# myshell-ai/OpenVoice

Measured on AMD Instinct MI355X. Metric: real_time_factor, higher is better.
Workload: dtype f32; 1 GPU; ToneColorConverter.convert path, 32 x 10 s @ 22.05 kHz per GPU (T=861 frames), fp32, calibrated random weights; batch_per_gpu=32, global_batch=32, parallelism=dp1 (utterance sharding, RCCL broadcast of src/tgt se)

## Files before the change

include/openvoice_amd.h:

```cpp
#ifndef OPENVOICE_AMD_H
#define OPENVOICE_AMD_H

#include <stddef.h>
#include <stdint.h>

#ifdef __cplusplus
extern "C" {
#endif

typedef void* ov_stream_t;

enum {
  OV_OK = 0,
  OV_E_BADARG = -1,
  OV_E_UNSUPPORTED = -2,
  OV_E_ALIGN = -3,
  OV_E_LAUNCH = -4
};

enum {
  OV_EPI_LINEAR = 0,
  OV_EPI_GATE = 1,
  OV_EPI_RESSKIP = 2,
  OV_EPI_COUPLE = 3,
  OV_EPI_POSTERIOR = 4,
  OV_EPI_CONVT = 5,
  OV_EPI_MAGNITUDE = 6
};

enum {
  OV_F_MASK_V = 1,
  OV_F_OUT2_INIT = 2,
  OV_F_CONVT_GROUPED = 4,
  OV_F_NO_XCD_MAP = 8
};

typedef struct ov_conv1d_params {
  const float* x;
  const float* w;
  const float* bias;
  const float* bias_b;
  float* out;
  const float* res;
  const float* add;
  float* out2;
  const float* mask;
  int64_t x_bstride;
  int64_t out_bstride;
  int64_t res_bstride;
  int64_t add_bstride;
  int64_t out2_bstride;
  int64_t bias_b_bstride;
  int64_t mask_bstride;
  int32_t B, Cin, L;
  int32_t x_ld;
  int32_t out_ld;
  int32_t M;
  int32_t Cout;
  int32_t K, dil;
  int32_t epi, flags, split, phase_s;
  int32_t tiles_per_wg;
  int32_t tile;
  int32_t loaders;
  int32_t chunk;
  float in_slope;
  float scale;
  const int32_t* col_limit;
  int32_t col_limit_scale;
  int32_t reserved0;
} ov_conv1d_params;


size_t ov_conv1d_pack_size(int Cout, int Cin, int K);
int ov_conv1d_pack_rows(int Cout);
int ov_conv1d_pack_f32(const float* w, int Cout, int Cin, int K, float* dst);


int ov_conv1d_f32(const ov_conv1d_params* p, ov_stream_t stream);

typedef struct ov_respair_params {
  const float* x;
  const float* w1;
  const float* b1;
  const float* w2;
  const float* b2;
  float* out;
  const float* add;
  int64_t x_bstride, out_bstride, add_bstride;
  int32_t B, C, L;
  int32_t ld;
  int32_t K, dil;
  int32_t nwg;
  float slope;
  float scale;
  unsigned long long* dbg;
  const int32_t* col_limit;
  int32_t col_limit_scale;
  int32_t reserved0;
} ov_respair_params;
int ov_resblock_pair_f32(const ov_respair_params* p, ov_stream_t stream);
int ov_resblock_pair_supported(int C, int K, int dil);

typedef struct ov_wn_layer_params {
  const float* x;
  float* out;
  float* skip;
  const float* w_in;
  const float* b_in;
  const float* cond;
  const float* w_rs;
  const float* b_rs;
  const float* mask;
  int64_t bstride;
  int64_t cond_bstride;
  int64_t mask_bstride;
  int32_t B, H, T;
  int32_t ld;
  int32_t K;
  int32_t first;
  int32_t last;
  int32_t width;
  int32_t ntile;
  int32_t row_split;
  unsigned long long* dbg;
  float* acts;
} ov_wn_layer_params;
int ov_wn_layer_f32(const ov_wn_layer_params* p, ov_stream_t stream);
int ov_wn_layer_supported(int H, int K);
size_t ov_wn_pack_size(int rows, int cin, int K);
int ov_wn_pack_f32(const float* w, int rows, int cin, int K, float* dst);
int ov_wn_layer_tile(int B, int T, int width);

int ov_wn_layer_wino_f32(const ov_wn_layer_params* p, ov_stream_t stream);
int ov_wn_layer_wino_tile(void);
size_t ov_wn_wino_pack_size(int rows, int cin, int K);
int ov_wn_wino_pack_f32(const float* w, int rows, int cin, int K, float* dst);

int ov_wn_layer_bf16(const ov_wn_layer_params* p, ov_stream_t stream);
int ov_wn_layer_bf16_supported(int H, int K);
size_t ov_wn_bf16_pack_size(int rows, int cin, int K);
int ov_wn_bf16_pack(const float* w, int rows, int cin, int K, uint16_t* dst);
int ov_wn_layer_bf16_tile(int B, int T, int width);

int ov_frame_hops_f32(const float* wave, float* hops, int B, int N, int hop, int pad, int U, int ld,
                      ov_stream_t stream);

int ov_frame_hops_windows_f32(const float* wave, int64_t n_samples, const int64_t* first_frame, int W, int hop, int pad,
                              int U, int ld, float* hops, ov_stream_t stream);
int ov_frame_hops_multi_f32(const float* pool, int64_t pool_len, const int64_t* records, int W, int hop, int pad, int U,
                            int ld, float* hops, ov_stream_t stream);
int ov_stitch_window_cores_f32(const float* o_hat, const int64_t* windows, int W, int Tw, int spf, float* out,
                               int64_t out_len, int64_t out_frame0, ov_stream_t stream);
int ov_carry_rows_f32(const int64_t* records, int n_records, const float* src_base, int64_t src_elems, float* dst_base,
                      int64_t dst_elems, ov_stream_t stream);
int ov_rows_f32_to_cl_bf16(const float* src, int64_t src_bs, int src_ld, uint16_t* dst, int B, int C, int L,
                           ov_stream_t stream);
int ov_cl_bf16_to_rows_f32(const uint16_t* src, float* dst, int64_t dst_bs, int dst_ld, int B, int C, int L,
                           ov_stream_t stream);

int ov_vad_frame_energy_f32(const float* pool, int64_t pool_len, const int64_t* records, int R, int H, int ldT,
                            float* energy, ov_stream_t stream);
int ov_vad_segments_i32(const float* energy, const int64_t* records, int R, int H, int ldT, float floor_lin,
                        float range_lin, int min_silence_frames, int min_speech_frames, int pad_frames, int32_t* mask,
                        int64_t* offsets, int64_t* n_active, ov_stream_t stream);
int ov_vad_compact_f32(const float* pool, int64_t pool_len, const int64_t* records, int R, int H, int ldT,
                       const int32_t* mask, const int64_t* offsets, const int64_t* out_bases, float* out,
                       int64_t out_len, ov_stream_t stream);

int ov_join_segments_f32(const float* src, int64_t src_elems, const int64_t* records, int R, float* dst,
                         int64_t dst_elems, int64_t max_span, ov_stream_t stream);

int ov_pack_groups_cl_bf16(const float* src, int64_t src_len, const int64_t* records, int n, int C, uint16_t* dst,
                           int64_t dst_len, ov_stream_t stream);
int ov_unpack_groups_f32(const float* src, int64_t src_len, const int64_t* records, int n, float* dst, int64_t dst_len,
                         ov_stream_t stream);

int ov_normal_philox_f32(const int64_t* records, int R, int C, float* dst, int64_t dst_elems, int64_t max_frames,
                         ov_stream_t stream);

int ov_polyphase_fir_f32(const float* x, const double* h, float* y, int64_t n_in, int64_t n_out, int P, int Q, int taps,
                         ov_stream_t stream);

int ov_polyphase_fir_rows_f32(const int64_t* records, int n_records, const float* src_base, int64_t src_elems,
                              const double* h_base, int64_t h_elems, float* dst_base, int64_t dst_elems, int64_t max_out,
                              ov_stream_t stream);

int ov_conv_post_tanh_f32(const float* x, const float* w, float* out, int B, int C, int L, int K,
                          float in_slope, ov_stream_t stream);
int ov_conv_post_tanh_limited_f32(const float* x, const float* w, float* out, int B, int C, int L, int K,
                                  float in_slope, const int32_t* col_limit, int col_limit_scale, ov_stream_t stream);
int ov_frame_limits_i32(const int64_t* lengths, int32_t* limits, int B, int T, int margin, ov_stream_t stream);

int ov_linear_f32(const float* x, const float* w, const float* bias, float* y, int B, int M, int Kdim,
                  ov_stream_t stream);

int ov_sequence_mask_f32(const int64_t* lengths, float* mask, int B, int T, int ld, ov_stream_t stream);
int ov_unpad_rows_f32(const float* src, float* dst, int rows, int T, int ld, ov_stream_t stream);


int ov_layernorm_freq_f32(const float* x, const float* gamma, const float* beta, float* y, int N, int F, int T,
                          float eps, ov_stream_t stream);

int ov_conv2d_s2_relu_f32(const float* x, const float* w, const float* bias, float* y, int N, int Cin, int Cout,
                          int Fi, int Ti, ov_stream_t stream);

int ov_gru_f32(const float* gi, const float* whh_t, const float* bhh, float* h_out, int N, int H, int T,
               ov_stream_t stream);


int ov_layernorm_freq_ragged_f32(const float* x, const float* gamma, const float* beta, const int32_t* lens, float* y,
                                 int N, int F, int ld, float eps, ov_stream_t stream);

int ov_conv2d_s2_relu_ragged_f32(const float* x, const float* w, const float* bias, const int32_t* lens_in, float* y,
                                 int N, int Cin, int Cout, int Fi, int ld_in, int ld_out, ov_stream_t stream);

int ov_gru_ragged_f32(const float* gi, const float* whh_t, const float* bhh, const int32_t* lens, float* h_out, int N,
                      int H, int ld, ov_stream_t stream);


int ov_embed_f32(const int64_t* tokens, const float* emb, const int64_t* lengths, float* out, int B, int T, int H,
                 int V, int ld, float scale, ov_stream_t stream);

enum {
  OV_LN_PRE_RELU = 1,
  OV_LN_POST_GELU = 2
};
int ov_layernorm_ch_f32(const float* x, const float* res, const float* gamma, const float* beta, const float* res2,
                        const float* mask, float* out, int B, int C, int T, int ld, float eps, int flags,
                        ov_stream_t stream);

int ov_rel_attention_f32(const float* q, const float* k, const float* v, const float* emb_k, const float* emb_v,
                         const float* mask, float* out, int64_t qkv_bstride, int64_t out_bstride, int B, int n_heads,
                         int dk, int T, int ld, int window, ov_stream_t stream);

int ov_dwconv1d_f32(const float* x, const float* w, const float* bias, const float* mask, float* out, int B, int C,
                    int T, int ld, int K, int dil, ov_stream_t stream);

int ov_expand1_f32(const float* x0, int64_t x0_bstride, const float* w, const float* bias, const float* g, float* out,
                   int B, int C, int T, int ld, ov_stream_t stream);

int ov_add_bias_mask_f32(const float* x, const float* bias_b, const float* mask, float* out, int B, int C, int T,
                         int ld, ov_stream_t stream);

int ov_rq_spline_inverse_f32(float* z, int64_t z_bstride, int c0, int c1, const float* h, int64_t h_bstride,
                             const float* mask, int B, int T, int ld, int num_bins, int filter_channels,
                             float tail_bound, ov_stream_t stream);

int ov_duration_f32(const float* z_sdp, int64_t z_bstride, float ea_m, float ea_logs, const float* dp,
                    int64_t dp_bstride, const float* mask, float* logw, int32_t* cum, int64_t* y_len, int B, int T,
                    int ld, float sdp_ratio, float length_scale, ov_stream_t stream);

int ov_expand_prior_f32(const float* m_tok, const float* logs_tok, int64_t tok_bstride, int ldx, const int32_t* cum,
                        const int64_t* x_len, const int64_t* y_len, const float* noise, int64_t noise_bstride, int ldn, float* z_p,
                        float* m_p, float* logs_p, float* attn, int B, int C, int Tx, int Ty, int ldy,
                        float noise_scale, ov_stream_t stream);

int ov_duration_items_f32(const float* z_sdp, int64_t z_bstride, float ea_m, float ea_logs, const float* dp,
                          int64_t dp_bstride, const float* mask, float* logw, int32_t* cum, int64_t* y_len, int B,
                          int T, int ld, const float* sdp_ratio_b, const float* length_scale_b, ov_stream_t stream);

int ov_expand_prior_items_f32(const float* m_tok, const float* logs_tok, int64_t tok_bstride, int ldx,
                              const int32_t* cum, const int64_t* x_len, const int64_t* y_len, const float* noise,
                              int64_t noise_bstride, int ldn, float* z_p, float* m_p, float* logs_p, float* attn,
                              int B, int C, int Tx, int Ty, int ldy, const float* noise_scale_b, ov_stream_t stream);

typedef struct ov_conv1d_bf16_params {
  const uint16_t* x;
  const uint16_t* w;
  const float* bias;
  uint16_t* out;
  const uint16_t* res;
  const uint16_t* add;
  int32_t B, L, Cin, Cout, K, dil;
  int32_t phase_s;
  int32_t bias_bstride;
  int32_t layout;
  float in_slope;
  float scale;
  float out_slope;
  unsigned long long* dbg;
} ov_conv1d_bf16_params;

size_t ov_conv1d_bf16_pack_size(int Cout, int Cin, int K);
int ov_conv1d_bf16_pack(const float* w, int Cout, int Cin, int K, uint16_t* dst);
int ov_conv1d_bf16cl(const ov_conv1d_bf16_params* p, ov_stream_t stream);
int ov_conv_post_tanh_bf16(const uint16_t* x, const float* w, float* out, int B, int C, int L, int K, float in_slope,
                           ov_stream_t stream);

typedef struct ov_respair_bf16_params {
  const uint16_t* x;
  const uint16_t* w1;
  const float* b1;
  const uint16_t* w2;
  const float* b2;
  uint16_t* out;
  const uint16_t* add;
  int32_t B, L, C, K, dil;
  int32_t nwg;
  float slope, scale;
  unsigned long long* dbg;
} ov_respair_bf16_params;
int ov_resblock_pair_bf16cl(const ov_respair_bf16_params* p, ov_stream_t stream);
int ov_resblock_pair_bf16_supported(int C, int K, int dil);

typedef struct ov_respair2_bf16_params {
  const uint16_t* x;
  const uint16_t* w1;
  const float* b1;
  const uint16_t* w2;
  const float* b2;
  uint16_t* out;
  const uint16_t* add;
  int32_t B, L, C, K, dil;
  int32_t nwg;
  float slope;
  float scale;
  float out_slope;
  int32_t exp_flags;
  unsigned long long* dbg;
} ov_respair2_bf16_params;
int ov_resblock_pair2_bf16cl(const ov_respair2_bf16_params* p, ov_stream_t stream);
int ov_conv1d_bf16_pack16(const float* w, int Cout, int Cin, int K, uint16_t* dst);
int ov_resblock_pair2_bf16_supported(int C, int K, int dil);

typedef struct ov_conv1d_split3_params {
  const uint16_t* x;
  const uint16_t* w;
  const float* bias;
  uint16_t* out;
  const uint16_t* res;
  int64_t x_plane, out_plane, res_plane;
  int32_t B, L, Cin, Cout, K, dil;
  int32_t nwg;
  int32_t products;
  float res_slope;
  float out_slope;
  float scale;
  int32_t col_limit_scale;
  unsigned long long* dbg;
  const int32_t* col_limit;
} ov_conv1d_split3_params;
int ov_conv1d_split3(const ov_conv1d_split3_params* p, ov_stream_t stream);
size_t ov_conv1d_split3_pack_size(int Cout, int Cin, int K);
int ov_conv1d_split3_pack(const float* w, int Cout, int Cin, int K, uint16_t* dst);
int ov_conv1d_split3_supported(int Cin, int Cout, int K, int dil);
int ov_split3_from_f32(const float* x, uint16_t* planes, int64_t plane_stride, int B, int C, int L, float slope,
                       ov_stream_t stream);
int ov_split3_to_f32(const uint16_t* a, const uint16_t* b, const uint16_t* c, int64_t plane_stride, float* out, int B,
                     int C, int L, float in_slope, float scale, ov_stream_t stream);

typedef struct ov_conv1d_wino_params {
  const float* x;
  const float* w;
  const float* bias;
  float* out;
  const float* res;
  const float* add;
  int64_t x_bstride, out_bstride, res_bstride, add_bstride;
  int32_t B, Cin, Cout, L;
  int32_t x_ld, out_ld;
  int32_t K, dil;
  int32_t nwg;
  int32_t frags;
  float in_slope;
  float scale;
  unsigned long long* dbg;
  const int32_t* col_limit;
  int32_t col_limit_scale;
  float out_slope;
} ov_conv1d_wino_params;
int ov_conv1d_wino_f32(const ov_conv1d_wino_params* p, ov_stream_t stream);
int ov_conv1d_wino_multi_f32(const ov_conv1d_wino_params* convs, int n, ov_stream_t stream);
int ov_conv1d_wino_supported(int Cin, int Cout, int K, int dil);
int ov_conv1d_wino_chunk(int K, int Cout);
size_t ov_conv1d_wino_pack_size(int Cout, int Cin, int K);
int ov_conv1d_wino_pack_f32(const float* w, int Cout, int Cin, int K, float* dst);

int ov_version(void);
#define OV_ABI_VERSION 212
int ov_build_experiment(void);

#ifdef __cplusplus
}
#endif
#endif
```

openvoice_amd/_lib.py:

```python
import ctypes
import os

_HERE = os.path.dirname(os.path.abspath(__file__))
LIB_PATH = os.environ.get("OPENVOICE_AMD_LIB") or os.path.join(_HERE, "libopenvoice_amd.so")

OV_OK = 0
MIN_VERSION = 212
OV_ERRORS = {-1: "OV_E_BADARG", -2: "OV_E_UNSUPPORTED", -3: "OV_E_ALIGN", -4: "OV_E_LAUNCH"}

EPI_LINEAR, EPI_GATE, EPI_RESSKIP, EPI_COUPLE, EPI_POSTERIOR, EPI_CONVT, EPI_MAGNITUDE = range(7)
F_MASK_V = 1
F_OUT2_INIT = 2
F_CONVT_GROUPED = 4
F_NO_XCD_MAP = 8

_fp = ctypes.c_void_p
_i = ctypes.c_int
_i64 = ctypes.c_int64
LN_PRE_RELU, LN_POST_GELU = 1, 2


class ConvParams(ctypes.Structure):
    _fields_ = [
        ("x", _fp), ("w", _fp), ("bias", _fp), ("bias_b", _fp), ("out", _fp), ("res", _fp),
        ("add", _fp), ("out2", _fp), ("mask", _fp),
        ("x_bstride", ctypes.c_int64), ("out_bstride", ctypes.c_int64), ("res_bstride", ctypes.c_int64),
        ("add_bstride", ctypes.c_int64), ("out2_bstride", ctypes.c_int64), ("bias_b_bstride", ctypes.c_int64),
        ("mask_bstride", ctypes.c_int64),
        ("B", ctypes.c_int32), ("Cin", ctypes.c_int32), ("L", ctypes.c_int32),
        ("x_ld", ctypes.c_int32), ("out_ld", ctypes.c_int32), ("M", ctypes.c_int32),
        ("Cout", ctypes.c_int32), ("K", ctypes.c_int32), ("dil", ctypes.c_int32), ("epi", ctypes.c_int32),
        ("flags", ctypes.c_int32), ("split", ctypes.c_int32), ("phase_s", ctypes.c_int32),
        ("tiles_per_wg", ctypes.c_int32), ("tile", ctypes.c_int32), ("loaders", ctypes.c_int32),
        ("chunk", ctypes.c_int32),
        ("in_slope", ctypes.c_float), ("scale", ctypes.c_float),
        ("col_limit", _fp), ("col_limit_scale", ctypes.c_int32), ("reserved0", ctypes.c_int32),
    ]


class ConvBf16Params(ctypes.Structure):
    _fields_ = [("x", _fp), ("w", _fp), ("bias", _fp), ("out", _fp), ("res", _fp), ("add", _fp),
                ("B", ctypes.c_int32), ("L", ctypes.c_int32), ("Cin", ctypes.c_int32), ("Cout", ctypes.c_int32),
                ("K", ctypes.c_int32), ("dil", ctypes.c_int32), ("phase_s", ctypes.c_int32), ("bias_bstride", ctypes.c_int32), ("layout", ctypes.c_int32),
                ("in_slope", ctypes.c_float), ("scale", ctypes.c_float), ("out_slope", ctypes.c_float), ("dbg", _fp)]


class RespairParams(ctypes.Structure):
    _fields_ = [("x", _fp), ("w1", _fp), ("b1", _fp), ("w2", _fp), ("b2", _fp), ("out", _fp), ("add", _fp),
                ("x_bstride", ctypes.c_int64), ("out_bstride", ctypes.c_int64), ("add_bstride", ctypes.c_int64),
                ("B", ctypes.c_int32), ("C", ctypes.c_int32), ("L", ctypes.c_int32), ("ld", ctypes.c_int32),
                ("K", ctypes.c_int32), ("dil", ctypes.c_int32), ("nwg", ctypes.c_int32),
                ("slope", ctypes.c_float), ("scale", ctypes.c_float), ("dbg", _fp),
                ("col_limit", _fp), ("col_limit_scale", ctypes.c_int32), ("reserved0", ctypes.c_int32)]


class RespairBf16Params(ctypes.Structure):
    _fields_ = [("x", _fp), ("w1", _fp), ("b1", _fp), ("w2", _fp), ("b2", _fp), ("out", _fp), ("add", _fp),
                ("B", ctypes.c_int32), ("L", ctypes.c_int32), ("C", ctypes.c_int32), ("K", ctypes.c_int32),
                ("dil", ctypes.c_int32), ("nwg", ctypes.c_int32), ("slope", ctypes.c_float), ("scale", ctypes.c_float),
                ("dbg", _fp)]


class Respair2Bf16Params(ctypes.Structure):
    _fields_ = [("x", _fp), ("w1", _fp), ("b1", _fp), ("w2", _fp), ("b2", _fp), ("out", _fp), ("add", _fp),
                ("B", ctypes.c_int32), ("L", ctypes.c_int32), ("C", ctypes.c_int32), ("K", ctypes.c_int32),
                ("dil", ctypes.c_int32), ("nwg", ctypes.c_int32), ("slope", ctypes.c_float), ("scale", ctypes.c_float),
                ("out_slope", ctypes.c_float), ("exp_flags", ctypes.c_int32), ("dbg", _fp)]


class ConvSplit3Params(ctypes.Structure):
    _fields_ = [("x", _fp), ("w", _fp), ("bias", _fp), ("out", _fp), ("res", _fp),
                ("x_plane", ctypes.c_int64), ("out_plane", ctypes.c_int64), ("res_plane", ctypes.c_int64),
                ("B", ctypes.c_int32), ("L", ctypes.c_int32), ("Cin", ctypes.c_int32), ("Cout", ctypes.c_int32),
                ("K", ctypes.c_int32), ("dil", ctypes.c_int32), ("nwg", ctypes.c_int32), ("products", ctypes.c_int32),
                ("res_slope", ctypes.c_float), ("out_slope", ctypes.c_float), ("scale", ctypes.c_float),
                ("col_limit_scale", ctypes.c_int32), ("dbg", _fp), ("col_limit", _fp)]


class ConvWinoParams(ctypes.Structure):
    _fields_ = [("x", _fp), ("w", _fp), ("bias", _fp), ("out", _fp), ("res", _fp), ("add", _fp),
                ("x_bstride", ctypes.c_int64), ("out_bstride", ctypes.c_int64), ("res_bstride", ctypes.c_int64),
                ("add_bstride", ctypes.c_int64),
                ("B", ctypes.c_int32), ("Cin", ctypes.c_int32), ("Cout", ctypes.c_int32), ("L", ctypes.c_int32),
                ("x_ld", ctypes.c_int32), ("out_ld", ctypes.c_int32), ("K", ctypes.c_int32), ("dil", ctypes.c_int32),
                ("nwg", ctypes.c_int32), ("frags", ctypes.c_int32),
                ("in_slope", ctypes.c_float), ("scale", ctypes.c_float), ("dbg", _fp),
                ("col_limit", _fp), ("col_limit_scale", ctypes.c_int32), ("out_slope", ctypes.c_float)]


class WnLayerParams(ctypes.Structure):
    _fields_ = [("x", _fp), ("out", _fp), ("skip", _fp), ("w_in", _fp), ("b_in", _fp), ("cond", _fp), ("w_rs", _fp),
                ("b_rs", _fp), ("mask", _fp),
                ("bstride", ctypes.c_int64), ("cond_bstride", ctypes.c_int64), ("mask_bstride", ctypes.c_int64),
                ("B", ctypes.c_int32), ("H", ctypes.c_int32), ("T", ctypes.c_int32), ("ld", ctypes.c_int32),
                ("K", ctypes.c_int32), ("first", ctypes.c_int32), ("last", ctypes.c_int32), ("width", ctypes.c_int32),
                ("ntile", ctypes.c_int32), ("row_split", ctypes.c_int32), ("dbg", _fp), ("acts", _fp)]


SIGNATURES = {
    "ov_version": (ctypes.c_int, []),
    "ov_build_experiment": (ctypes.c_int, []),
    "ov_conv1d_pack_size": (ctypes.c_size_t, [ctypes.c_int, ctypes.c_int, ctypes.c_int]),
    "ov_conv1d_pack_rows": (ctypes.c_int, [ctypes.c_int]),
    "ov_conv1d_pack_f32": (ctypes.c_int, [_fp, ctypes.c_int, ctypes.c_int, ctypes.c_int, _fp]),
    "ov_conv1d_f32": (ctypes.c_int, [ctypes.POINTER(ConvParams), _fp]),
    "ov_resblock_pair_f32": (ctypes.c_int, [ctypes.POINTER(RespairParams), _fp]),
    "ov_resblock_pair_supported": (ctypes.c_int, [_i, _i, _i]),
    "ov_wn_layer_f32": (ctypes.c_int, [ctypes.POINTER(WnLayerParams), _fp]),
    "ov_wn_layer_supported": (ctypes.c_int, [_i, _i]),
    "ov_wn_pack_size": (ctypes.c_size_t, [_i, _i, _i]),
    "ov_wn_pack_f32": (ctypes.c_int, [_fp, _i, _i, _i, _fp]),
    "ov_wn_layer_tile": (ctypes.c_int, [_i, _i, _i]),
    "ov_wn_layer_wino_f32": (ctypes.c_int, [ctypes.POINTER(WnLayerParams), _fp]),
    "ov_wn_layer_wino_tile": (ctypes.c_int, []),
    "ov_wn_wino_pack_size": (ctypes.c_size_t, [_i, _i, _i]),
    "ov_wn_wino_pack_f32": (ctypes.c_int, [_fp, _i, _i, _i, _fp]),
    "ov_wn_layer_bf16": (ctypes.c_int, [ctypes.POINTER(WnLayerParams), _fp]),
    "ov_wn_layer_bf16_supported": (ctypes.c_int, [_i, _i]),
    "ov_wn_bf16_pack_size": (ctypes.c_size_t, [_i, _i, _i]),
    "ov_wn_bf16_pack": (ctypes.c_int, [_fp, _i, _i, _i, _fp]),
    "ov_wn_layer_bf16_tile": (ctypes.c_int, [_i, _i, _i]),
    "ov_conv_post_tanh_f32": (ctypes.c_int, [_fp, _fp, _fp, ctypes.c_int, ctypes.c_int, ctypes.c_int,
                                             ctypes.c_int, ctypes.c_float, _fp]),
    "ov_conv_post_tanh_limited_f32": (ctypes.c_int, [_fp, _fp, _fp, ctypes.c_int, ctypes.c_int, ctypes.c_int,
                                                     ctypes.c_int, ctypes.c_float, _fp, ctypes.c_int, _fp]),
    "ov_frame_limits_i32": (ctypes.c_int, [_fp, _fp, _i, _i, _i, _fp]),
    "ov_linear_f32": (ctypes.c_int, [_fp, _fp, _fp, _fp, ctypes.c_int, ctypes.c_int, ctypes.c_int, _fp]),
    "ov_sequence_mask_f32": (ctypes.c_int, [_fp, _fp, ctypes.c_int, ctypes.c_int, ctypes.c_int, _fp]),
    "ov_unpad_rows_f32": (ctypes.c_int, [_fp, _fp, ctypes.c_int, ctypes.c_int, ctypes.c_int, _fp]),
    "ov_polyphase_fir_f32": (ctypes.c_int, [_fp, _fp, _fp, ctypes.c_int64, ctypes.c_int64, _i, _i, _i, _fp]),
    "ov_polyphase_fir_rows_f32": (ctypes.c_int, [_fp, _i, _fp, _i64, _fp, _i64, _fp, _i64, _i64, _fp]),
    "ov_layernorm_freq_f32": (ctypes.c_int, [_fp, _fp, _fp, _fp, ctypes.c_int, ctypes.c_int, ctypes.c_int,
                                             ctypes.c_float, _fp]),
    "ov_conv2d_s2_relu_f32": (ctypes.c_int, [_fp, _fp, _fp, _fp, ctypes.c_int, ctypes.c_int, ctypes.c_int,
                                             ctypes.c_int, ctypes.c_int, _fp]),
    "ov_gru_f32": (ctypes.c_int, [_fp, _fp, _fp, _fp, ctypes.c_int, ctypes.c_int, ctypes.c_int, _fp]),
    "ov_layernorm_freq_ragged_f32": (ctypes.c_int, [_fp, _fp, _fp, _fp, _fp, _i, _i, _i, ctypes.c_float, _fp]),
    "ov_conv2d_s2_relu_ragged_f32": (ctypes.c_int, [_fp, _fp, _fp, _fp, _fp, _i, _i, _i, _i, _i, _i, _fp]),
    "ov_gru_ragged_f32": (ctypes.c_int, [_fp, _fp, _fp, _fp, _fp, _i, _i, _i, _fp]),
    "ov_conv1d_bf16_pack_size": (ctypes.c_size_t, [_i, _i, _i]),
    "ov_conv1d_bf16_pack": (ctypes.c_int, [_fp, _i, _i, _i, _fp]),
    "ov_conv1d_bf16_pack16": (ctypes.c_int, [_fp, _i, _i, _i, _fp]),
    "ov_conv1d_bf16cl": (ctypes.c_int, [ctypes.POINTER(ConvBf16Params), _fp]),
    "ov_resblock_pair_bf16cl": (ctypes.c_int, [ctypes.POINTER(RespairBf16Params), _fp]),
    "ov_resblock_pair_bf16_supported": (ctypes.c_int, [_i, _i, _i]),
    "ov_resblock_pair2_bf16cl": (ctypes.c_int, [ctypes.POINTER(Respair2Bf16Params), _fp]),
    "ov_resblock_pair2_bf16_supported": (ctypes.c_int, [_i, _i, _i]),
    "ov_conv_post_tanh_bf16": (ctypes.c_int, [_fp, _fp, _fp, _i, _i, _i, _i, ctypes.c_float, _fp]),
    "ov_conv1d_split3": (ctypes.c_int, [ctypes.POINTER(ConvSplit3Params), _fp]),
    "ov_conv1d_split3_pack_size": (ctypes.c_size_t, [_i, _i, _i]),
    "ov_conv1d_split3_pack": (ctypes.c_int, [_fp, _i, _i, _i, _fp]),
    "ov_conv1d_split3_supported": (ctypes.c_int, [_i, _i, _i, _i]),
    "ov_split3_from_f32": (ctypes.c_int, [_fp, _fp, _i64, _i, _i, _i, ctypes.c_float, _fp]),
    "ov_split3_to_f32": (ctypes.c_int, [_fp, _fp, _fp, _i64, _fp, _i, _i, _i, ctypes.c_float, ctypes.c_float, _fp]),
    "ov_conv1d_wino_f32": (ctypes.c_int, [ctypes.POINTER(ConvWinoParams), _fp]),
    "ov_conv1d_wino_multi_f32": (ctypes.c_int, [ctypes.POINTER(ConvWinoParams), _i, _fp]),
    "ov_conv1d_wino_supported": (ctypes.c_int, [_i, _i, _i, _i]),
    "ov_conv1d_wino_chunk": (ctypes.c_int, [_i, _i]),
    "ov_conv1d_wino_pack_size": (ctypes.c_size_t, [_i, _i, _i]),
    "ov_conv1d_wino_pack_f32": (ctypes.c_int, [_fp, _i, _i, _i, _fp]),
    "ov_frame_hops_f32": (ctypes.c_int, [_fp, _fp, _i, _i, _i, _i, _i, _i, _fp]),
    "ov_frame_hops_windows_f32": (ctypes.c_int, [_fp, _i64, _fp, _i, _i, _i, _i, _i, _fp, _fp]),
    "ov_frame_hops_multi_f32": (ctypes.c_int, [_fp, _i64, _fp, _i, _i, _i, _i, _i, _fp, _fp]),
    "ov_stitch_window_cores_f32": (ctypes.c_int, [_fp, _fp, _i, _i, _i, _fp, _i64, _i64, _fp]),
    "ov_carry_rows_f32": (ctypes.c_int, [_fp, _i, _fp, _i64, _fp, _i64, _fp]),
    "ov_rows_f32_to_cl_bf16": (ctypes.c_int, [_fp, _i64, _i, _fp, _i, _i, _i, _fp]),
    "ov_cl_bf16_to_rows_f32": (ctypes.c_int, [_fp, _fp, _i64, _i, _i, _i, _i, _fp]),
    "ov_vad_frame_energy_f32": (ctypes.c_int, [_fp, _i64, _fp, _i, _i, _i, _fp, _fp]),
    "ov_vad_segments_i32": (ctypes.c_int, [_fp, _fp, _i, _i, _i, ctypes.c_float, ctypes.c_float, _i, _i, _i, _fp, _fp, _fp,
                                           _fp]),
    "ov_vad_compact_f32": (ctypes.c_int, [_fp, _i64, _fp, _i, _i, _i, _fp, _fp, _fp, _fp, _i64, _fp]),
    "ov_join_segments_f32": (ctypes.c_int, [_fp, _i64, _fp, _i, _fp, _i64, _i64, _fp]),
    "ov_pack_groups_cl_bf16": (ctypes.c_int, [_fp, _i64, _fp, _i, _i, _fp, _i64, _fp]),
    "ov_unpack_groups_f32": (ctypes.c_int, [_fp, _i64, _fp, _i, _fp, _i64, _fp]),
    "ov_normal_philox_f32": (ctypes.c_int, [_fp, _i, _i, _fp, _i64, _i64, _fp]),
    "ov_embed_f32": (ctypes.c_int, [_fp, _fp, _fp, _fp, _i, _i, _i, _i, _i, ctypes.c_float, _fp]),
    "ov_layernorm_ch_f32": (ctypes.c_int, [_fp, _fp, _fp, _fp, _fp, _fp, _fp, _i, _i, _i, _i, ctypes.c_float, _i, _fp]),
    "ov_rel_attention_f32": (ctypes.c_int, [_fp, _fp, _fp, _fp, _fp, _fp, _fp, _i64, _i64, _i, _i, _i, _i, _i, _i,
                                            _fp]),
    "ov_add_bias_mask_f32": (ctypes.c_int, [_fp, _fp, _fp, _fp, _i, _i, _i, _i, _fp]),
    "ov_dwconv1d_f32": (ctypes.c_int, [_fp, _fp, _fp, _fp, _fp, _i, _i, _i, _i, _i, _i, _fp]),
    "ov_expand1_f32": (ctypes.c_int, [_fp, _i64, _fp, _fp, _fp, _fp, _i, _i, _i, _i, _fp]),
    "ov_rq_spline_inverse_f32": (ctypes.c_int, [_fp, _i64, _i, _i, _fp, _i64, _fp, _i, _i, _i, _i, _i,
                                                ctypes.c_float, _fp]),
    "ov_duration_f32": (ctypes.c_int, [_fp, _i64, ctypes.c_float, ctypes.c_float, _fp, _i64, _fp, _fp, _fp, _fp,
                                       _i, _i, _i, ctypes.c_float, ctypes.c_float, _fp]),
    "ov_expand_prior_f32": (ctypes.c_int, [_fp, _fp, _i64, _i, _fp, _fp, _fp, _fp, _i64, _i, _fp, _fp, _fp, _fp,
                                           _i, _i, _i, _i, _i, ctypes.c_float, _fp]),
    "ov_duration_items_f32": (ctypes.c_int, [_fp, _i64, ctypes.c_float, ctypes.c_float, _fp, _i64, _fp, _fp, _fp, _fp,
                                             _i, _i, _i, _fp, _fp, _fp]),
    "ov_expand_prior_items_f32": (ctypes.c_int, [_fp, _fp, _i64, _i, _fp, _fp, _fp, _fp, _i64, _i, _fp, _fp, _fp, _fp,
                                                 _i, _i, _i, _i, _i, _fp, _fp]),
}

_lib = None


class OvError(RuntimeError):
    pass


GENERATORS = ("fp32", "bf16")


def check_generator(generator, optional=False):
    if generator is None and optional:
        return None
    if not isinstance(generator, str) or generator not in GENERATORS:
        raise OvError(f"generator must be 'fp32' or 'bf16'{' (or None)' if optional else ''}, got {generator!r}")
    return generator


def generator_kw(generator):
    return {} if generator is None else {"generator": generator}


WAVENETS = ("fp32", "bf16")


def check_wavenet(wavenet, optional=False):
    if wavenet is None and optional:
        return None
    if not isinstance(wavenet, str) or wavenet not in WAVENETS:
        raise OvError(f"wavenet must be 'fp32' or 'bf16'{' (or None)' if optional else ''}, got {wavenet!r}")
    return wavenet


def wavenet_kw(wavenet):
    return {} if wavenet is None else {"wavenet": wavenet}


def load():
    global _lib
    if _lib is None:
        if not os.path.exists(LIB_PATH):
            raise OvError(f"{LIB_PATH} not found: build the HIP extension first "
                          f"(python -c 'import __graft_entry__ as g; g.build()'); there is no CPU fallback")
        lib = ctypes.CDLL(LIB_PATH)
        lib.ov_version.restype, lib.ov_version.argtypes = ctypes.c_int, []
        if lib.ov_version() < MIN_VERSION:
            raise OvError(f"{LIB_PATH} is version {lib.ov_version()}, this package needs >= {MIN_VERSION}: rebuild it "
                          f"(make -C openvoice_amd/csrc)")
        for name, (restype, argtypes) in SIGNATURES.items():
            try:
                fn = getattr(lib, name)
            except AttributeError:
                raise OvError(f"{LIB_PATH} lacks {name}: it was built from older source, rebuild it "
                              f"(make -C openvoice_amd/csrc)") from None
            fn.restype = restype
            fn.argtypes = argtypes
        exp = lib.ov_build_experiment()
        if exp != 0 and os.environ.get("OPENVOICE_AMD_ALLOW_EXPERIMENT") != "1":
            raise OvError(f"{LIB_PATH} is a measurement build (OV_EXP={exp}: kernels with loads / barriers compiled "
                          f"out, results meaningless); rebuild with `make -C openvoice_amd/csrc clean all`")
        _lib = lib
    return _lib


def torch_op(name, *args):
    try:
        return getattr(torch_ops(), name)(*args)
    except RuntimeError as exc:
        if isinstance(exc, OvError):
            raise
        raise OvError(str(exc).split("\n")[0]) from None


def check(code, what):
    if code != OV_OK:
        raise OvError(f"{what} failed: {OV_ERRORS.get(code, code)}")


SHIM_PATH = os.path.join(_HERE, "libopenvoice_amd_torch.so")
_ops = None
VALUE_FUNCS = {"ov_version", "ov_build_experiment", "ov_conv1d_pack_size", "ov_conv1d_pack_rows", "ov_wn_pack_size",
               "ov_conv1d_bf16_pack_size", "ov_resblock_pair_supported", "ov_wn_layer_supported", "ov_wn_layer_tile",
               "ov_resblock_pair_bf16_supported", "ov_resblock_pair2_bf16_supported", "ov_conv1d_split3_pack_size",
               "ov_conv1d_split3_supported", "ov_conv1d_wino_supported", "ov_conv1d_wino_chunk", "ov_conv1d_wino_pack_size",
               "ov_wn_layer_wino_tile", "ov_wn_wino_pack_size", "ov_wn_layer_bf16_supported", "ov_wn_bf16_pack_size",
               "ov_wn_layer_bf16_tile"}


def binding():
    b = os.environ.get("OPENVOICE_AMD_BINDING", "ctypes" if os.environ.get("OPENVOICE_AMD_LIB") else "torch")
    if b not in ("torch", "ctypes"):
        raise OvError(f"OPENVOICE_AMD_BINDING={b!r}: expected 'torch' or 'ctypes'")
    return b


def use_torch_binding():
    return binding() == "torch"


def torch_ops():
    global _ops
    if _ops is None:
        import torch
        for path in (LIB_PATH, SHIM_PATH):
            if not os.path.exists(path):
                raise OvError(f"{path} not found: build the HIP extension first (python -c 'import __graft_entry__ "
                              f"as g; g.build()'); there is no CPU fallback (OPENVOICE_AMD_BINDING=ctypes needs only "
                              f"libopenvoice_amd.so)")
        torch.ops.load_library(SHIM_PATH)
        ops = torch.ops.openvoice_amd
        if ops.version() < MIN_VERSION:
            raise OvError(f"{LIB_PATH} is version {ops.version()}, this package needs >= {MIN_VERSION}: rebuild it "
                          f"(make -C openvoice_amd/csrc)")
        exp = ops.build_experiment()
        if exp != 0 and os.environ.get("OPENVOICE_AMD_ALLOW_EXPERIMENT") != "1":
            raise OvError(f"{LIB_PATH} is a measurement build (OV_EXP={exp}); rebuild with "
                          f"`make -C openvoice_amd/csrc clean all`")
        _ops = ops
    return _ops


def _flat_view(t, off):
    start = t.storage_offset() + off
    n = t.untyped_storage().nbytes() // t.element_size() - start
    return t.as_strided((n,), (1,), start)


def call(name, *args):
    if use_torch_binding():
        targs = [_flat_view(*a) if type(a) is tuple else a for a in args]
        try:
            return getattr(torch_ops(), name[3:])(*targs)
        except RuntimeError as exc:
            if isinstance(exc, OvError):
                raise
            raise OvError(str(exc).split("\n")[0]) from None
    import torch
    lib = load()
    fn = getattr(lib, name)
    cargs, dev = [], None
    for a in args:
        off = 0
        if type(a) is tuple:
            a, off = a
        if isinstance(a, torch.Tensor):
            if dev is None and a.is_cuda:
                dev = a.device
            a = ctypes.c_void_p(a.data_ptr() + off * a.element_size())
        cargs.append(a)
    if len(fn.argtypes) == len(cargs) + 1:
        if dev is None:
            raise OvError(f"{name}: no device tensor among the arguments")
        cargs.append(ctypes.c_void_p(torch.cuda.current_stream(dev).cuda_stream))
    rc = fn(*cargs)
    if name in VALUE_FUNCS:
        return rc
    check(rc, name)
```

openvoice_amd/csrc/conv1d_mfma.h:

```cpp
#pragma once
#include <hip/hip_runtime.h>

#include <atomic>

#include "openvoice_amd.h"

namespace ovk {

constexpr int EPI_CONVT_S8 = 16;
constexpr int EPI_CONVT_S2 = 17;
constexpr bool is_convt(int epi) { return epi == OV_EPI_CONVT || epi == EPI_CONVT_S8 || epi == EPI_CONVT_S2; }

typedef float f32x16 __attribute__((ext_vector_type(16)));
typedef float f32x4 __attribute__((ext_vector_type(4)));
typedef float f32x2 __attribute__((ext_vector_type(2)));

constexpr int UNIT = 8;
constexpr int REC = 256;
constexpr int LB_MAX = 12;
constexpr int LIMIT_MAX_BATCH = 256;

__host__ __device__ inline int packed_units(int cin) { return ((cin + UNIT - 1) / UNIT + 3) / 4 * 4; }

__device__ __forceinline__ float lrelu(float v, float slope) { return v > 0.f ? v : v * slope; }

template <int EPI, int WM, int WN>
__device__ __forceinline__ void conv_epilogue(const ov_conv1d_params& p, f32x16 (&acc)[WM][WN], int b, int tcol0,
                                              int mtile0, int q, int lane, bool preloaded) {
  const uint32_t L = (uint32_t)p.L;
  const uint32_t LD = (uint32_t)p.out_ld;
  const uint32_t half = (uint32_t)lane >> 5;
  const uint32_t Cout = (uint32_t)p.Cout;
  const float scale = p.scale;
  const float* mrow = p.mask ? p.mask + (int64_t)b * p.mask_bstride : nullptr;
  float* outb = p.out + (int64_t)b * p.out_bstride;
  const uint32_t col0 = (uint32_t)tcol0 + ((uint32_t)lane & 31u);

  if constexpr (EPI == EPI_CONVT_S8 || EPI == EPI_CONVT_S2) {
    static_assert(WM == 2, "grouped ConvTranspose pairs two 32-row tiles per wave");
    const uint32_t Lout = LD;
    if ((uint32_t)q * 64u >= Cout * (uint32_t)p.phase_s) return;
#pragma unroll
    for (int j = 0; j < WN; ++j) {
      const uint32_t col = col0 + 32u * j;
      if (col >= L) continue;
      if constexpr (EPI == EPI_CONVT_S8) {
#pragma unroll
        for (int i = 0; i < 2; ++i) {
          const f32x16 v = acc[i][j];
#pragma unroll
          for (int c = 0; c < 4; ++c) {
            f32x4 o = {v[4 * c], v[4 * c + 1], v[4 * c + 2], v[4 * c + 3]};
            *reinterpret_cast<f32x4*>(outb + (size_t)((uint32_t)q * 8u + 2u * c + half) * Lout +
                                      (8u * col + 4u * i)) = o;
          }
        }
      } else {
        const f32x16 v0 = acc[0][j], v1 = acc[1][j];
#pragma unroll
        for (int r = 0; r < 16; ++r) {
          const uint32_t co = (uint32_t)q * 32u + 4u * half + (r & 3) + 8 * (r >> 2);
          f32x2 o = {v0[r], v1[r]};
          *reinterpret_cast<f32x2*>(outb + (co * Lout + 2u * col)) = o;
        }
      }
    }
    return;
  } else if constexpr (EPI == OV_EPI_MAGNITUDE) {
    static_assert(WM == 2, "magnitude pairs two 32-row tiles per wave");
    if ((uint32_t)q * 32u >= Cout) return;
#pragma unroll
    for (int j = 0; j < WN; ++j) {
      const uint32_t col = col0 + 32u * j;
      if (col >= L) continue;
      const uint32_t rbase = (uint32_t)q * 32u + 4u * half;
      const uint32_t voff = rbase * LD + col;
#pragma unroll
      for (int r = 0; r < 16; ++r) {
        const uint32_t rr = (r & 3) + 8 * (r >> 2);
        const float re = acc[0][j][r], im = acc[1][j][r];
        if (rbase + rr < Cout) (outb + (size_t)rr * LD)[voff] = sqrtf(re * re + im * im + scale);
      }
    }
    return;
  } else if constexpr (EPI == OV_EPI_GATE || EPI == OV_EPI_POSTERIOR) {
    static_assert(WM == 2, "gate/posterior pair two 32-row tiles per wave");
    if ((uint32_t)q * 32u >= Cout) return;
    const float* resb = p.res ? p.res + (int64_t)b * p.res_bstride : nullptr;
#pragma unroll
    for (int j = 0; j < WN; ++j) {
      const uint32_t col = col0 + 32u * j;
      if (col >= L) continue;
      const float mk = mrow ? mrow[col] : 1.f;
      const uint32_t voff = ((uint32_t)q * 32u + 4u * half) * LD + col;
      const uint32_t rbase = (uint32_t)q * 64u + 4u * half;
      const f32x16 v0 = acc[0][j], v1 = acc[1][j];
      if constexpr (EPI == OV_EPI_GATE) {
#pragma unroll
        for (int r = 0; r < 16; ++r) {
          const uint32_t rr = (r & 3) + 8 * (r >> 2);
          (outb + (size_t)rr * LD)[voff] = tanhf(v0[r]) * (1.f / (1.f + expf(-v1[r])));
        }
      } else {
        f32x16 nz;
#pragma unroll
        for (int r = 0; r < 16; ++r) nz[r] = (resb + (size_t)((r & 3) + 8 * (r >> 2)) * LD)[voff];
#pragma unroll
        for (int r = 0; r < 16; ++r) {
          const uint32_t rr = (r & 3) + 8 * (r >> 2);
          (outb + (size_t)rr * LD)[voff] = (v0[r] * mk + nz[r] * scale * expf(v1[r] * mk)) * mk;
        }
      }
    }
    return;
  } else {
    if constexpr (EPI == OV_EPI_LINEAR) {
      if (!mrow && !(p.res && !preloaded) && !p.add) {
#pragma unroll
        for (int i = 0; i < WM; ++i) {
          const uint32_t mt = (uint32_t)(mtile0 + i);
          if (mt * 32u >= Cout) continue;
#pragma unroll
          for (int j = 0; j < WN; ++j) {
            const uint32_t col = col0 + 32u * j;
            if (col >= L) continue;
            const uint32_t voff = (mt * 32u + 4u * half) * LD + col;
#pragma unroll
            for (int r = 0; r < 16; ++r) (outb + (size_t)((r & 3) + 8 * (r >> 2)) * LD)[voff] = acc[i][j][r] * scale;
          }
        }
        return;
      }
    }
#pragma unroll
    for (int i = 0; i < WM; ++i) {
      const uint32_t mt = (uint32_t)(mtile0 + i);
      if (mt * 32u >= (is_convt(EPI) ? Cout * (uint32_t)p.phase_s : Cout)) continue;
#pragma unroll
      for (int j = 0; j < WN; ++j) {
        const uint32_t col = col0 + 32u * j;
        if (col >= L) continue;
        const float mk = mrow ? mrow[col] : 1.f;
        const uint32_t rbase = mt * 32u + 4u * half;
        f32x16 v = acc[i][j];
        if constexpr (is_convt(EPI)) {
          const uint32_t s = (uint32_t)p.phase_s;
          const uint32_t Lout = LD;
          {
#pragma unroll
            for (int r = 0; r < 16; ++r) {
              const uint32_t row = rbase + (r & 3) + 8 * (r >> 2);
              const uint32_t co = row / s, ph = row - co * s;
              outb[co * Lout + s * col + ph] = v[r];
            }
          }
        } else {
          const uint32_t voff = rbase * LD + col;
          if constexpr (EPI == OV_EPI_LINEAR) {
            const float* resb = (p.res && !preloaded) ? p.res + (int64_t)b * p.res_bstride : nullptr;
            const float* addb = p.add ? p.add + (int64_t)b * p.add_bstride : nullptr;
            const float mkv = (p.flags & OV_F_MASK_V) ? mk : 1.f;
#pragma unroll
            for (int r = 0; r < 16; ++r) v[r] *= mkv;
            if (resb) {
#pragma unroll
              for (int r = 0; r < 16; ++r) v[r] += (resb + (size_t)((r & 3) + 8 * (r >> 2)) * LD)[voff];
            }
            if (addb) {
#pragma unroll
              for (int r = 0; r < 16; ++r) v[r] += (addb + (size_t)((r & 3) + 8 * (r >> 2)) * LD)[voff];
            }
#pragma unroll
            for (int r = 0; r < 16; ++r) (outb + (size_t)((r & 3) + 8 * (r >> 2)) * LD)[voff] = v[r] * scale;
          } else if constexpr (EPI == OV_EPI_RESSKIP) {
            if (mt * 32u < (uint32_t)p.split) {
#pragma unroll
              for (int r = 0; r < 16; ++r) (outb + (size_t)((r & 3) + 8 * (r >> 2)) * LD)[voff] = v[r] * mk;
            } else {
              float* o2 = p.out2 + (int64_t)b * p.out2_bstride;
              const uint32_t voff2 = voff - (uint32_t)p.split * LD;
#pragma unroll
              for (int r = 0; r < 16; ++r) (o2 + (size_t)((r & 3) + 8 * (r >> 2)) * LD)[voff2] = v[r];
            }
          } else {
            const float sg = scale > 0.f ? mk : -mk;
#pragma unroll
            for (int r = 0; r < 16; ++r) (outb + (size_t)((r & 3) + 8 * (r >> 2)) * LD)[voff] = v[r] * sg;
          }
        }
      }
    }
  }
}

template <int EPI, int WM, int WN>
__device__ __forceinline__ bool conv_preload(const ov_conv1d_params& p, f32x16 (&acc)[WM][WN], int b, int tcol0,
                                             int mtile0, int lane) {
  const uint32_t half = (uint32_t)lane >> 5;
  const uint32_t L = (uint32_t)p.L, LD = (uint32_t)p.out_ld;
  const uint32_t col0 = (uint32_t)tcol0 + ((uint32_t)lane & 31u);
  constexpr bool kOperands = EPI == OV_EPI_LINEAR || EPI == OV_EPI_RESSKIP || EPI == OV_EPI_COUPLE;
  bool preloaded = false;
  if constexpr (kOperands) {
    const float* src = nullptr;
    int64_t src_bs = 0;
    if constexpr (EPI == OV_EPI_LINEAR) {
      if (p.res && !(p.flags & OV_F_MASK_V)) { src = p.res; src_bs = p.res_bstride; }
    } else if (EPI == OV_EPI_COUPLE && p.res) {
      src = p.res; src_bs = p.res_bstride;
    } else {
      src = p.out; src_bs = p.out_bstride;
    }
    preloaded = src != nullptr;
    if (preloaded) {
      const uint32_t nfrag = (uint32_t)p.Cout / 32u;
      const float* srcb = src + (int64_t)b * src_bs;
#pragma unroll
      for (int i = 0; i < WM; ++i) {
        const uint32_t mt = min((uint32_t)(mtile0 + i), nfrag - 1u);
        const float* rowb = srcb;
        uint32_t mrow = mt * 32u;
        bool zero = false;
        if constexpr (EPI == OV_EPI_RESSKIP) {
          if (mrow >= (uint32_t)p.split) {
            rowb = p.out2 + (int64_t)b * p.out2_bstride;
            mrow -= (uint32_t)p.split;
            zero = (p.flags & OV_F_OUT2_INIT) != 0;
          }
        }
#pragma unroll
        for (int j = 0; j < WN; ++j) {
          const uint32_t col = min(col0 + 32u * j, L - 1u);
          const uint32_t voff = (mrow + 4u * half) * LD + col;
#pragma unroll
          for (int r = 0; r < 16; ++r) acc[i][j][r] = (rowb + (size_t)((r & 3) + 8 * (r >> 2)) * LD)[voff];
          if constexpr (EPI == OV_EPI_RESSKIP) {
            if (zero) {
#pragma unroll
              for (int r = 0; r < 16; ++r) acc[i][j][r] = 0.f;
            }
          }
          if constexpr (EPI == OV_EPI_COUPLE) {
            if (!(p.scale > 0.f)) {
#pragma unroll
              for (int r = 0; r < 16; ++r) acc[i][j][r] = -acc[i][j][r];
            }
          }
        }
      }
    }
  }
  if (!preloaded) {
#pragma unroll
    for (int i = 0; i < WM; ++i)
#pragma unroll
      for (int j = 0; j < WN; ++j)
#pragma unroll
        for (int r = 0; r < 16; ++r) acc[i][j][r] = 0.f;
  }
  {
    const float* __restrict__ bias = p.bias;
    const float* __restrict__ bias_b = p.bias_b ? p.bias_b + (int64_t)b * p.bias_b_bstride : nullptr;
    const uint32_t row_limit = (EPI == OV_EPI_GATE || EPI == OV_EPI_POSTERIOR || EPI == OV_EPI_MAGNITUDE)
                                   ? 2u * (uint32_t)p.Cout
                                   : (is_convt(EPI) ? (uint32_t)p.Cout * (uint32_t)p.phase_s : (uint32_t)p.Cout);
#pragma unroll
    for (int i = 0; i < WM; ++i) {
      const uint32_t rbase = (uint32_t)(mtile0 + i) * 32u + 4u * half;
      if (EPI != OV_EPI_MAGNITUDE && (uint32_t)(mtile0 + i) * 32u < row_limit) {
        f32x16 bv;
#pragma unroll
        for (int r = 0; r < 16; ++r) bv[r] = bias[rbase + (r & 3) + 8 * (r >> 2)];
        if (bias_b) {
#pragma unroll
          for (int r = 0; r < 16; ++r) bv[r] += bias_b[rbase + (r & 3) + 8 * (r >> 2)];
        }
#pragma unroll
        for (int j = 0; j < WN; ++j) acc[i][j] += bv;
      }
    }
  }
  return preloaded;
}

constexpr int STAGE_SCALAR = 0;
constexpr int STAGE_VEC = 1;

template <int K, int DIL, int WM, int WN, int WVM, int WVN, int CHUNK, int VEC, int EPI, int NLD>
__global__ __launch_bounds__(64 * (4 + NLD), (EPI == OV_EPI_GATE || EPI == EPI_CONVT_S8 || EPI == EPI_CONVT_S2) ? 4 : 1) void conv1d_mfma_kernel(const ov_conv1d_params p) {
  static_assert(WVM * WVN == 4, "4 matrix waves per workgroup");
  static_assert(VEC == STAGE_SCALAR || VEC == STAGE_VEC, "staging kind");
  static_assert(CHUNK % UNIT == 0 && (CHUNK / UNIT == 2 || CHUNK / UNIT == 4), "chunk = 2 or 4 units");
  constexpr int UPC = CHUNK / UNIT;
  constexpr int N_BLK = 32 * WN * WVN;
  constexpr int PAD = (K % 2 == 1) ? (K - 1) * DIL / 2 : 0;
  constexpr int PADR = (K - 1) * DIL - PAD;
  constexpr int PADA = (PAD + 3) / 4 * 4;
  constexpr int XS = N_BLK + PADA + (PADR + 3) / 4 * 4;
  constexpr int XS4 = XS / 4;
  constexpr int NITEM = VEC ? CHUNK * XS4 : CHUNK * XS;
  constexpr int BUF = CHUNK * XS;
  constexpr int PER_LANE = (NITEM + 64 * NLD - 1) / (64 * NLD);
  constexpr int LB = PER_LANE < LB_MAX ? PER_LANE : LB_MAX;
  constexpr int NBATCH = (PER_LANE + LB - 1) / LB;
  static_assert(NLD == 1 || NLD == 2 || NLD == 4, "1, 2 or 4 loader waves");

  __shared__ __attribute__((aligned(16))) float xs[2 * BUF];

  const int tid = threadIdx.x;
  const int lane = tid & 63;
  const int wave = __builtin_amdgcn_readfirstlane(tid >> 6);
  const int L = p.L, Cin = p.Cin;
  const int nunits = packed_units(Cin);
  const int nchunks = nunits / UPC;
  const int ntiles = (L + N_BLK - 1) / N_BLK;
  const int mblocks = (p.M + 32 * WM * WVM - 1) / (32 * WM * WVM);
  int total = ntiles * mblocks * p.B;
  __shared__ int lim_pref[LIMIT_MAX_BATCH + 1];
  const bool limited = p.col_limit != nullptr;
  if (limited) {
    if (wave == 0) {
      int carry = 0;
      for (int base = 0; base < p.B; base += 64) {
        const int bb = base + lane;
        int n = 0;
        if (bb < p.B) {
          long long c = (long long)p.col_limit[bb] * p.col_limit_scale;
          c = c < 0 ? 0 : (c > L ? L : c);
          n = ((int)c + N_BLK - 1) / N_BLK;
        }
        int s = n;
#pragma unroll
        for (int d = 1; d < 64; d <<= 1) {
          const int v = __shfl_up(s, d, 64);
          if (lane >= d) s += v;
        }
        if (bb < p.B) lim_pref[bb + 1] = carry + s;
        carry += __shfl(s, 63, 64);
      }
      if (lane == 0) lim_pref[0] = 0;
    }
    __syncthreads();
    total = __builtin_amdgcn_readfirstlane(lim_pref[p.B]) * mblocks;
  }
  auto decode = [&](int w, int& ub, int& utile, int& umblk) {
    const int g = w / mblocks;
    umblk = w - g * mblocks;
    if (!limited) {
      ub = g / ntiles;
      utile = g - ub * ntiles;
      return;
    }
    int lo = 0, hi = p.B;
    while (hi - lo > 1) {
      const int mid = (lo + hi) >> 1;
      if (__builtin_amdgcn_readfirstlane(lim_pref[mid]) <= g) lo = mid; else hi = mid;
    }
    ub = lo;
    utile = g - __builtin_amdgcn_readfirstlane(lim_pref[lo]);
  };
  int wid0 = blockIdx.x, wend = total, wstride = gridDim.x;
  if (!(p.flags & OV_F_NO_XCD_MAP) && (gridDim.x & 7u) == 0) {
    const int xcd = blockIdx.x & 7;
    const int lo = (int)(((long long)xcd * total) >> 3);
    wend = (int)(((long long)(xcd + 1) * total) >> 3);
    wid0 = lo + (int)(blockIdx.x >> 3);
    wstride = gridDim.x >> 3;
  }
  if (wid0 >= wend) return;

  bool is_loader = false;
#pragma unroll
  for (int i = 0; i < NLD; ++i) is_loader |= (wave == 4 + i);
#ifndef OV_EXP
#define OV_EXP 0
#endif
  if (is_loader) {
    if (OV_EXP == 1) return;
    const float slope = p.in_slope;
    const uint32_t ldx = (uint32_t)p.x_ld;
    const int llane = (wave - 4) * 64 + lane;
    const int Lin = L + ((K % 2 == 1) ? 0 : (K - 1) * DIL);
    int it = 0;
    for (int wid = wid0; wid < wend; wid += wstride) {
      int lb, ltile, lmblk;
      decode(wid, lb, ltile, lmblk);
      const int t0 = ltile * N_BLK;
      const float* __restrict__ xb = p.x + (int64_t)lb * p.x_bstride;
      for (int chunk = 0; chunk < nchunks; ++chunk, ++it) {
        float* dst = xs + (it & 1) * BUF;
#pragma unroll 1
        for (int bt = 0; bt < (OV_EXP ? 0 : NBATCH); ++bt) {
          if constexpr (VEC) {
            f32x4 stg[LB];
            int nval[LB];
#pragma unroll
            for (int i = 0; i < LB; ++i) {
              const int idx = (bt * LB + i) * (64 * NLD) + llane;
              const int row = idx / XS4, c4 = idx - row * XS4;
              const int ci = chunk * CHUNK + row;
              const int t = t0 - PADA + 4 * c4;
              const bool ok = idx < NITEM && ci < Cin && t >= 0 && t < Lin;
              const uint32_t goff = ok ? (uint32_t)ci * ldx + (uint32_t)t : 0u;
              nval[i] = ok ? min(Lin - t, 4) : 0;
              stg[i] = *reinterpret_cast<const f32x4*>(xb + goff);
            }
#pragma unroll
            for (int i = 0; i < LB; ++i) {
              const int idx = (bt * LB + i) * (64 * NLD) + llane;
              if (idx < NITEM) {
                f32x4 v = stg[i];
                const int n = nval[i];
                v[0] = n > 0 ? lrelu(v[0], slope) : 0.f;
                v[1] = n > 1 ? lrelu(v[1], slope) : 0.f;
                v[2] = n > 2 ? lrelu(v[2], slope) : 0.f;
                v[3] = n > 3 ? lrelu(v[3], slope) : 0.f;
                *reinterpret_cast<f32x4*>(dst + 4 * idx) = v;
              }
            }
          } else {
            float stg[LB];
            int nval[LB];
#pragma unroll
            for (int i = 0; i < LB; ++i) {
              const int idx = (bt * LB + i) * (64 * NLD) + llane;
              const int row = idx / XS, c = idx - row * XS;
              const int ci = chunk * CHUNK + row;
              const int t = t0 - PADA + c;
              const bool ok = idx < NITEM && ci < Cin && t >= 0 && t < Lin;
              const uint32_t goff = ok ? (uint32_t)ci * ldx + (uint32_t)t : 0u;
              nval[i] = ok ? 1 : 0;
              stg[i] = xb[goff];
            }
#pragma unroll
            for (int i = 0; i < LB; ++i) {
              const int idx = (bt * LB + i) * (64 * NLD) + llane;
              if (idx < NITEM) dst[idx] = nval[i] ? lrelu(stg[i], slope) : 0.f;
            }
          }
        }
        __syncthreads();
      }
    }
    return;
  }

  const int wm = wave / WVN, wn = wave % WVN;
  const int recs_per_mtile = nunits * K + 1;
  int wid = wid0;
  int mblk, tile, b;
  decode(wid, b, tile, mblk);
  int mtile0 = (mblk * WVM + wm) * WM;

  const f32x4* __restrict__ wbase = reinterpret_cast<const f32x4*>(p.w);
  uint32_t widx[WM];
#pragma unroll
  for (int i = 0; i < WM; ++i) widx[i] = (uint32_t)(mtile0 + i) * (uint32_t)recs_per_mtile * 64u + (uint32_t)lane;

  const int xl_off = (lane >> 5) * XS + wn * (32 * WN) + (lane & 31) + (PADA - PAD);

  f32x4 a_cur[WM], a_nxt[WM];
#pragma unroll
  for (int i = 0; i < WM; ++i) a_cur[i] = wbase[widx[i]];

#if OV_EXP == 3
  unsigned long long tph[5] = {0, 0, 0, 0, 0};
  unsigned long long tlast = __builtin_readcyclecounter();
#define OV_MARK(q) { const unsigned long long now_ = __builtin_readcyclecounter(); tph[q] += now_ - tlast; tlast = now_; }
#else
#define OV_MARK(q)
#endif
  int it = 0;
  while (true) {
    f32x16 acc[WM][WN];
    const bool preloaded = conv_preload<EPI, WM, WN>(p, acc, b, tile * N_BLK + wn * (32 * WN), mtile0, lane);
    OV_MARK(0)

    int rec = 0;
    for (int chunk = 0; chunk < nchunks; ++chunk, ++it) {
      if (OV_EXP != 1) __syncthreads();
      OV_MARK(1)
      const float* xl = xs + (it & 1) * BUF + xl_off;
      constexpr int STEPS = UPC * 4 * K;
      float bcur[WN], bnxt[WN];
#pragma unroll
      for (int j = 0; j < WN; ++j) bcur[j] = xl[32 * j];
#pragma unroll
      for (int sa = 0; sa < STEPS; ++sa) {
        const int u = sa & 3;
        if (u == 0) {
          ++rec;
#pragma unroll
          for (int i = 0; i < WM; ++i) a_nxt[i] = (wbase + (size_t)rec * 64)[widx[i]];
        }
        if (sa + 1 < STEPS) {
          const int uu = (sa + 1) / (4 * K), sn = (sa + 1) - uu * (4 * K);
          const int pp = sn / K, tap = sn - pp * K;
#pragma unroll
          for (int j = 0; j < WN; ++j) bnxt[j] = xl[(uu * UNIT + 2 * pp) * XS + 32 * j + tap * DIL];
        }
        __builtin_amdgcn_sched_barrier(0);
        const int tap_now = (sa % (4 * K)) % K;
#pragma unroll
        for (int m = 0; m < WM * WN; ++m) {
          const int i = m / WN, j = m % WN;
          if ((EPI == EPI_CONVT_S8 || EPI == EPI_CONVT_S2) && tap_now == ((i & 1) ? 0 : K - 1)) continue;
          acc[i][j] = __builtin_amdgcn_mfma_f32_32x32x2f32(a_cur[i][u], bcur[j], acc[i][j], 0, 0, 0);
        }
        __builtin_amdgcn_sched_barrier(0);
        if (sa + 1 < STEPS) {
#pragma unroll
          for (int j = 0; j < WN; ++j) bcur[j] = bnxt[j];
        }
        if (u == 3) {
#pragma unroll
          for (int i = 0; i < WM; ++i) a_cur[i] = a_nxt[i];
        }
      }
      OV_MARK(2)
    }
    const int nwid = wid + wstride;
    const bool more = nwid < wend;
    int nmblk = 0, ntile = 0, nb = 0;
    if (more) decode(nwid, nb, ntile, nmblk);
    const int nmtile0 = (nmblk * WVM + wm) * WM;
    uint32_t nwidx[WM];
#pragma unroll
    for (int i = 0; i < WM; ++i) nwidx[i] = (uint32_t)(nmtile0 + i) * (uint32_t)recs_per_mtile * 64u + (uint32_t)lane;
    if (more) {
#pragma unroll
      for (int i = 0; i < WM; ++i) a_cur[i] = wbase[nwidx[i]];
    }
    conv_epilogue<EPI, WM, WN>(p, acc, b, tile * N_BLK + wn * (32 * WN), mtile0, mblk * WVM + wm, lane, preloaded);
    OV_MARK(3)
#if OV_EXP == 3
    ++tph[4];
    if (!more && EPI == OV_EPI_LINEAR && p.out2 && lane == 0) {
      unsigned long long* dbg = reinterpret_cast<unsigned long long*>(p.out2) + ((size_t)blockIdx.x * 4 + wave) * 8;
#pragma unroll
      for (int q = 0; q < 5; ++q) dbg[q] = tph[q];
    }
#endif
    if (!more) break;
    wid = nwid; tile = ntile; mblk = nmblk; b = nb; mtile0 = nmtile0;
#pragma unroll
    for (int i = 0; i < WM; ++i) widx[i] = nwidx[i];
  }
}

constexpr int OV_MAX_DEVICES = 16;
inline int resident_workgroups(const void* kernel, int block_threads, std::atomic<int>* cache) {
  int dev = 0;
  const bool known = hipGetDevice(&dev) == hipSuccess && dev >= 0 && dev < OV_MAX_DEVICES;
  if (known) {
    const int v = cache[dev].load(std::memory_order_relaxed);
    if (v > 0) return v;
  }
  int per_cu = 0, slots = 512;
  hipDeviceProp_t prop;
  if (hipGetDeviceProperties(&prop, dev) == hipSuccess &&
      hipOccupancyMaxActiveBlocksPerMultiprocessor(&per_cu, kernel, block_threads, 0) == hipSuccess && per_cu > 0)
    slots = per_cu * prop.multiProcessorCount;
  if (known) cache[dev].store(slots, std::memory_order_relaxed);
  return slots;
}

inline int compute_units() {
  static std::atomic<int> cache[OV_MAX_DEVICES];
  int dev = 0;
  const bool known = hipGetDevice(&dev) == hipSuccess && dev >= 0 && dev < OV_MAX_DEVICES;
  if (known) {
    const int v = cache[dev].load(std::memory_order_relaxed);
    if (v > 0) return v;
  }
  int cus = 256;
  hipDeviceProp_t prop;
  if (hipGetDeviceProperties(&prop, dev) == hipSuccess && prop.multiProcessorCount > 0) cus = prop.multiProcessorCount;
  if (known) cache[dev].store(cus, std::memory_order_relaxed);
  return cus;
}

typedef int (*conv_launch_fn)(const ov_conv1d_params*, hipStream_t);

template <int K, int DIL, int WM, int WN, int WVM, int WVN, int CHUNK, int VEC, int EPI, int NLD>
int conv1d_launch(const ov_conv1d_params* p, hipStream_t stream) {
  constexpr int M_BLK = 32 * WM * WVM, N_BLK = 32 * WN * WVN;
  const int ntiles = (p->L + N_BLK - 1) / N_BLK;
  const int mblocks = (p->M + M_BLK - 1) / M_BLK;
  const long total = (long)ntiles * mblocks * p->B;
  auto kernel = conv1d_mfma_kernel<K, DIL, WM, WN, WVM, WVN, CHUNK, VEC, EPI, NLD>;
  static std::atomic<int> slot_cache[OV_MAX_DEVICES];
  const int slots = resident_workgroups(reinterpret_cast<const void*>(kernel), 64 * (4 + NLD), slot_cache);
  const int tpw = p->tiles_per_wg > 0 ? p->tiles_per_wg : 1;
  const bool persistent = p->tiles_per_wg < 0 || (p->tiles_per_wg == 0 && p->res == nullptr && total >= 16L * slots);
  long nwg = persistent ? (long)slots : (total + tpw - 1) / tpw;
  if (nwg > total) nwg = total;
  if (!(p->flags & OV_F_NO_XCD_MAP) && nwg >= 8) nwg = (nwg + 7) / 8 * 8;
  hipLaunchKernelGGL(kernel, dim3((unsigned)nwg), dim3(64 * (4 + NLD)), 0, stream, *p);
  return hipGetLastError() == hipSuccess ? OV_OK : OV_E_LAUNCH;
}

enum { TILE_128x128 = 0, TILE_64x256 = 1, TILE_32x512 = 2, TILE_32x256 = 3 };

struct ConvVariant {
  int K, dil, tile, chunk, vec, epi, nld;
  conv_launch_fn fn;
};

#define OV_TILE_128x128 2, 2, 2, 2
#define OV_TILE_64x256 2, 2, 1, 4
#define OV_TILE_32x512 1, 4, 1, 4
#define OV_TILE_32x256 1, 2, 1, 4

#define OV_X_INST(K, DIL, TILE, CHUNK, VEC, EPI, NLD)                                                        \
  template __global__ void conv1d_mfma_kernel<K, DIL, OV_TILE_##TILE, CHUNK, VEC, EPI, NLD>(                  \
      const ov_conv1d_params);
#define OV_X_ROW(K, DIL, TILE, CHUNK, VEC, EPI, NLD)                                                         \
  {K, DIL, TILE_##TILE, CHUNK, VEC, EPI, NLD,                                                                \
   conv1d_launch<K, DIL, OV_TILE_##TILE, CHUNK, VEC, EPI, NLD>},
#if defined(__HIP_DEVICE_COMPILE__)
#define OV_DEFINE_VARIANTS(table, LIST) LIST(OV_X_INST)
#else
#define OV_DEFINE_VARIANTS(table, LIST)                   \
  LIST(OV_X_INST)                                         \
  const ConvVariant table[] = {LIST(OV_X_ROW)};           \
  const int table##Count = sizeof(table) / sizeof(table[0]);
#endif

#define OV_DECLARE_VARIANTS(table)  \
  extern const ConvVariant table[]; \
  extern const int table##Count;
OV_DECLARE_VARIANTS(kVariantsA)
OV_DECLARE_VARIANTS(kVariantsB)
OV_DECLARE_VARIANTS(kVariantsC)
OV_DECLARE_VARIANTS(kVariantsD)
OV_DECLARE_VARIANTS(kVariantsE)
OV_DECLARE_VARIANTS(kVariantsF)
OV_DECLARE_VARIANTS(kVariantsS)
OV_DECLARE_VARIANTS(kVariantsW)

}
```

openvoice_amd/csrc/torch_shim.cpp:

```cpp
#include <ATen/ATen.h>
#include <ATen/hip/impl/HIPGuardImplMasqueradingAsCUDA.h>
#include <c10/hip/HIPStream.h>
#include <torch/library.h>

#include <string>
#include <type_traits>

#include "openvoice_amd.h"

namespace {

const char* ov_strerror(int rc) {
  switch (rc) {
    case OV_E_BADARG: return "OV_E_BADARG";
    case OV_E_UNSUPPORTED: return "OV_E_UNSUPPORTED";
    case OV_E_ALIGN: return "OV_E_ALIGN";
    case OV_E_LAUNCH: return "OV_E_LAUNCH";
    default: return "unknown error";
  }
}

using OptTensor = c10::optional<at::Tensor>;

struct Ctx {
  const char* name;
  bool host;
  bool have_dev = false;
  c10::Device dev{c10::kCPU};
  void see(const at::Tensor& t, int index) {
    if (host) {
      TORCH_CHECK(t.device().is_cpu(), name, ": argument ", index, " must be a HOST (CPU) tensor");
      return;
    }
    TORCH_CHECK(t.is_cuda(), name, ": argument ", index, " must be on a ROCm device (there is no CPU path)");
    if (!have_dev) { dev = t.device(); have_dev = true; }
    TORCH_CHECK(t.device() == dev, name, ": argument ", index, " is on ", t.device(), ", expected ", dev);
  }
  ov_stream_t stream() const {
    TORCH_CHECK(have_dev, name, ": no device tensor among the arguments");
    return static_cast<ov_stream_t>(c10::hip::getCurrentHIPStream(dev.index()).stream());
  }
};

struct DeviceScope {
  c10::hip::OptionalHIPGuardMasqueradingAsCUDA guard;
  explicit DeviceScope(const Ctx& c) { if (c.have_dev) guard.set_device(c.dev); }
};

template <typename E> bool dtype_ok(at::ScalarType s);
template <> bool dtype_ok<float>(at::ScalarType s) { return s == at::kFloat; }
template <> bool dtype_ok<double>(at::ScalarType s) { return s == at::kDouble; }
template <> bool dtype_ok<int64_t>(at::ScalarType s) { return s == at::kLong; }
template <> bool dtype_ok<int32_t>(at::ScalarType s) { return s == at::kInt; }
template <> bool dtype_ok<uint16_t>(at::ScalarType s) { return s == at::kBFloat16 || s == at::kShort || s == at::kUInt16; }
template <> bool dtype_ok<unsigned long long>(at::ScalarType s) { return s == at::kLong || s == at::kUInt64; }
template <typename E> const char* dtype_name();
template <> const char* dtype_name<float>() { return "float32"; }
template <> const char* dtype_name<double>() { return "float64"; }
template <> const char* dtype_name<int64_t>() { return "int64"; }
template <> const char* dtype_name<int32_t>() { return "int32"; }
template <> const char* dtype_name<uint16_t>() { return "bfloat16 (or int16 bit patterns)"; }
template <> const char* dtype_name<unsigned long long>() { return "int64 (tick counters)"; }

template <typename E> E* tensor_ptr(const OptTensor& t, Ctx& c, int index) {
  if (!t.has_value() || !t->defined()) return nullptr;
  c.see(*t, index);
  TORCH_CHECK(dtype_ok<E>(t->scalar_type()), c.name, ": argument ", index, " must be ", dtype_name<E>(), ", got ",
              t->scalar_type());
  return static_cast<E*>(t->data_ptr());
}

template <typename C, typename = void> struct Arg;
template <typename E> struct Arg<const E*> {
  using torch_t = const OptTensor&;
  static std::string schema(int i) { return "Tensor? a" + std::to_string(i); }
  static const E* get(const OptTensor& t, Ctx& c, int i) { return tensor_ptr<E>(t, c, i); }
};
template <typename E> struct Arg<E*, std::enable_if_t<!std::is_const<E>::value>> {
  using torch_t = const OptTensor&;
  static std::string schema(int i) { return "Tensor(a" + std::to_string(i) + "!)? a" + std::to_string(i); }
  static E* get(const OptTensor& t, Ctx& c, int i) { return tensor_ptr<E>(t, c, i); }
};
template <> struct Arg<int> {
  using torch_t = int64_t;
  static std::string schema(int i) { return "int a" + std::to_string(i); }
  static int get(int64_t v, Ctx& c, int i) {
    TORCH_CHECK(v >= INT32_MIN && v <= INT32_MAX, c.name, ": argument ", i, " does not fit a 32-bit int");
    return static_cast<int>(v);
  }
};
template <> struct Arg<int64_t> {
  using torch_t = int64_t;
  static std::string schema(int i) { return "int a" + std::to_string(i); }
  static int64_t get(int64_t v, Ctx&, int) { return v; }
};
template <> struct Arg<float> {
  using torch_t = double;
  static std::string schema(int i) { return "float a" + std::to_string(i); }
  static float get(double v, Ctx&, int) { return static_cast<float>(v); }
};

template <typename... T> struct List {};
template <typename L, typename... Acc> struct DropLast;
template <typename T, typename... Acc> struct DropLast<List<T>, Acc...> { using type = List<Acc...>; using last = T; };
template <typename T, typename U, typename... R, typename... Acc>
struct DropLast<List<T, U, R...>, Acc...> : DropLast<List<U, R...>, Acc..., T> {};

template <typename... C> std::string schema_of(const char* name, bool returns_int) {
  std::string s = std::string(name) + "(";
  int i = 0;
  bool first = true;
  ((s += (first ? "" : ", ") + Arg<C>::schema(i++), first = false), ...);
  return s + (returns_int ? ") -> int" : ") -> ()");
}

template <int Kind, typename R, typename L> struct Wrap;
template <typename R, typename... C> struct Wrap<0, R, List<C...>> {
  template <R (*Fn)(C..., ov_stream_t)> struct On {
    static inline const char* name = "";
    static void call(typename Arg<C>::torch_t... a) {
      Ctx c{name, false};
      int i = 0;
      std::tuple<C...> v{Arg<C>::get(a, c, i++)...};
      DeviceScope scope(c);
      const int rc = std::apply([&](C... x) { return Fn(x..., c.stream()); }, v);
      TORCH_CHECK(rc == OV_OK, "ov_", name, " failed: ", ov_strerror(rc));
    }
    static void def(torch::Library& m, const char* n) { name = n; m.def(schema_of<C...>(n, false).c_str(), &call); }
  };
};
template <typename R, typename... C> struct Wrap<1, R, List<C...>> {
  template <R (*Fn)(C...)> struct On {
    static inline const char* name = "";
    static void call(typename Arg<C>::torch_t... a) {
      Ctx c{name, true};
      int i = 0;
      std::tuple<C...> v{Arg<C>::get(a, c, i++)...};
      const int rc = std::apply(Fn, v);
      TORCH_CHECK(rc == OV_OK, "ov_", name, " failed: ", ov_strerror(rc));
    }
    static void def(torch::Library& m, const char* n) { name = n; m.def(schema_of<C...>(n, false).c_str(), &call); }
  };
};
template <typename R, typename... C> struct Wrap<2, R, List<C...>> {
  template <R (*Fn)(C...)> struct On {
    static inline const char* name = "";
    static int64_t call(typename Arg<C>::torch_t... a) {
      Ctx c{name, true};
      int i = 0;
      std::tuple<C...> v{Arg<C>::get(a, c, i++)...};
      return static_cast<int64_t>(std::apply(Fn, v));
    }
    static void def(torch::Library& m, const char* n) { name = n; m.def(schema_of<C...>(n, true).c_str(), &call); }
  };
};

template <typename F> struct Sig;
template <typename R, typename... C> struct Sig<R (*)(C...)> { using ret = R; using args = List<C...>; };

template <auto Fn> void bind_device(torch::Library& m, const char* name) {
  using S = Sig<decltype(Fn)>;
  using D = DropLast<typename S::args>;
  static_assert(std::is_same<typename D::last, ov_stream_t>::value, "device entry points end with the stream");
  Wrap<0, typename S::ret, typename D::type>::template On<Fn>::def(m, name);
}
template <auto Fn> void bind_host(torch::Library& m, const char* name) {
  using S = Sig<decltype(Fn)>;
  Wrap<1, typename S::ret, typename S::args>::template On<Fn>::def(m, name);
}
template <auto Fn> void bind_value(torch::Library& m, const char* name) {
  using S = Sig<decltype(Fn)>;
  Wrap<2, typename S::ret, typename S::args>::template On<Fn>::def(m, name);
}

template <typename E> E* sptr(const OptTensor& t, Ctx& c, int index, int64_t off = 0) {
  E* p = tensor_ptr<E>(t, c, index);
  return p ? p + off : nullptr;
}
void finish(int rc, const char* what) { TORCH_CHECK(rc == OV_OK, what, " failed: ", ov_strerror(rc)); }

void conv1d_f32(const OptTensor& x, const OptTensor& w, const OptTensor& bias, const OptTensor& out, const OptTensor& res,
                const OptTensor& add, const OptTensor& out2, const OptTensor& mask, const OptTensor& bias_b,
                const OptTensor& col_limit, at::IntArrayRef ip, at::ArrayRef<double> fp) {
  TORCH_CHECK(ip.size() == 29 && fp.size() == 2, "openvoice_amd::conv1d_f32: 29 integer and 2 float parameters");
  Ctx c{"conv1d_f32", false};
  ov_conv1d_params p{};
  p.x = sptr<float>(x, c, 0, ip[24]);
  p.w = sptr<float>(w, c, 1);
  p.bias = sptr<float>(bias, c, 2);
  p.out = sptr<float>(out, c, 3, ip[25]);
  p.res = sptr<float>(res, c, 4, ip[26]);
  p.add = sptr<float>(add, c, 5);
  p.out2 = sptr<float>(out2, c, 6);
  p.mask = sptr<float>(mask, c, 7);
  p.bias_b = sptr<float>(bias_b, c, 8, ip[27]);
  p.col_limit = sptr<int32_t>(col_limit, c, 9);
  p.col_limit_scale = (int32_t)ip[28];
  p.B = (int32_t)ip[0]; p.Cin = (int32_t)ip[1]; p.L = (int32_t)ip[2]; p.x_ld = (int32_t)ip[3]; p.out_ld = (int32_t)ip[4];
  p.M = (int32_t)ip[5]; p.Cout = (int32_t)ip[6]; p.K = (int32_t)ip[7]; p.dil = (int32_t)ip[8]; p.epi = (int32_t)ip[9];
  p.flags = (int32_t)ip[10]; p.split = (int32_t)ip[11]; p.phase_s = (int32_t)ip[12]; p.tiles_per_wg = (int32_t)ip[13];
  p.tile = (int32_t)ip[14]; p.loaders = (int32_t)ip[15]; p.chunk = (int32_t)ip[16];
  p.x_bstride = ip[17]; p.out_bstride = ip[18]; p.res_bstride = ip[19]; p.add_bstride = ip[20];
  p.out2_bstride = ip[21]; p.bias_b_bstride = ip[22]; p.mask_bstride = ip[23];
  p.in_slope = (float)fp[0]; p.scale = (float)fp[1];
  DeviceScope scope(c);
  finish(ov_conv1d_f32(&p, c.stream()), "ov_conv1d_f32");
}

void resblock_pair_f32(const OptTensor& x, const OptTensor& w1, const OptTensor& b1, const OptTensor& w2,
                       const OptTensor& b2, const OptTensor& out, const OptTensor& add, const OptTensor& dbg,
                       const OptTensor& col_limit, at::IntArrayRef ip, at::ArrayRef<double> fp) {
  TORCH_CHECK(ip.size() == 11 && fp.size() == 2, "openvoice_amd::resblock_pair_f32: 11 integer and 2 float parameters");
  Ctx c{"resblock_pair_f32", false};
  ov_respair_params p{};
  p.x = sptr<float>(x, c, 0); p.w1 = sptr<float>(w1, c, 1); p.b1 = sptr<float>(b1, c, 2);
  p.w2 = sptr<float>(w2, c, 3); p.b2 = sptr<float>(b2, c, 4); p.out = sptr<float>(out, c, 5);
  p.add = sptr<float>(add, c, 6);
  p.dbg = sptr<unsigned long long>(dbg, c, 7);
  p.col_limit = sptr<int32_t>(col_limit, c, 8);
  p.B = (int32_t)ip[0]; p.C = (int32_t)ip[1]; p.L = (int32_t)ip[2]; p.ld = (int32_t)ip[3]; p.K = (int32_t)ip[4];
  p.dil = (int32_t)ip[5]; p.nwg = (int32_t)ip[6];
  p.x_bstride = ip[7]; p.out_bstride = ip[8]; p.add_bstride = ip[9]; p.col_limit_scale = (int32_t)ip[10];
  p.slope = (float)fp[0]; p.scale = (float)fp[1];
  DeviceScope scope(c);
  finish(ov_resblock_pair_f32(&p, c.stream()), "ov_resblock_pair_f32");
}

template <int (*FN)(const ov_wn_layer_params*, ov_stream_t)>
void wn_layer_any(const char* op, const char* entry, const OptTensor& x, const OptTensor& out, const OptTensor& skip,
                  const OptTensor& w_in, const OptTensor& b_in, const OptTensor& cond, const OptTensor& w_rs,
                  const OptTensor& b_rs, const OptTensor& mask, const OptTensor& dbg, const OptTensor& acts,
                  at::IntArrayRef ip) {
  TORCH_CHECK(ip.size() == 13, "openvoice_amd::", op, ": 13 integer parameters");
  Ctx c{op, false};
  ov_wn_layer_params p{};
  p.x = sptr<float>(x, c, 0); p.out = sptr<float>(out, c, 1); p.skip = sptr<float>(skip, c, 2);
  p.w_in = sptr<float>(w_in, c, 3); p.b_in = sptr<float>(b_in, c, 4); p.cond = sptr<float>(cond, c, 5, ip[11]);
  p.w_rs = sptr<float>(w_rs, c, 6); p.b_rs = sptr<float>(b_rs, c, 7); p.mask = sptr<float>(mask, c, 8);
  p.dbg = sptr<unsigned long long>(dbg, c, 9);
  p.acts = sptr<float>(acts, c, 10);
  p.B = (int32_t)ip[0]; p.H = (int32_t)ip[1]; p.T = (int32_t)ip[2]; p.ld = (int32_t)ip[3]; p.K = (int32_t)ip[4];
  p.first = (int32_t)ip[5]; p.last = (int32_t)ip[6]; p.width = (int32_t)ip[7];
  p.bstride = ip[8]; p.cond_bstride = ip[9]; p.mask_bstride = ip[10]; p.row_split = (int32_t)ip[12];
  DeviceScope scope(c);
  finish(FN(&p, c.stream()), entry);
}
void wn_layer_f32(const OptTensor& x, const OptTensor& out, const OptTensor& skip, const OptTensor& w_in,
                  const OptTensor& b_in, const OptTensor& cond, const OptTensor& w_rs, const OptTensor& b_rs,
                  const OptTensor& mask, const OptTensor& dbg, const OptTensor& acts, at::IntArrayRef ip) {
  wn_layer_any<&ov_wn_layer_f32>("wn_layer_f32", "ov_wn_layer_f32", x, out, skip, w_in, b_in, cond, w_rs, b_rs, mask, dbg, acts, ip);
}
void wn_layer_wino_f32(const OptTensor& x, const OptTensor& out, const OptTensor& skip, const OptTensor& w_in,
                       const OptTensor& b_in, const OptTensor& cond, const OptTensor& w_rs, const OptTensor& b_rs,
                       const OptTensor& mask, const OptTensor& dbg, const OptTensor& acts, at::IntArrayRef ip) {
  wn_layer_any<&ov_wn_layer_wino_f32>("wn_layer_wino_f32", "ov_wn_layer_wino_f32", x, out, skip, w_in, b_in, cond, w_rs, b_rs, mask, dbg,
                                      acts, ip);
}
void wn_layer_bf16(const OptTensor& x, const OptTensor& out, const OptTensor& skip, const OptTensor& w_in,
                   const OptTensor& b_in, const OptTensor& cond, const OptTensor& w_rs, const OptTensor& b_rs,
                   const OptTensor& mask, const OptTensor& dbg, const OptTensor& acts, at::IntArrayRef ip) {
  wn_layer_any<&ov_wn_layer_bf16>("wn_layer_bf16", "ov_wn_layer_bf16", x, out, skip, w_in, b_in, cond, w_rs, b_rs, mask, dbg, acts, ip);
}

void conv1d_bf16cl(const OptTensor& x, const OptTensor& w, const OptTensor& bias, const OptTensor& out,
                   const OptTensor& res, const OptTensor& add, const OptTensor& dbg, at::IntArrayRef ip,
                   at::ArrayRef<double> fp) {
  TORCH_CHECK(ip.size() == 9 && fp.size() == 3, "openvoice_amd::conv1d_bf16cl: 9 integer and 3 float parameters");
  Ctx c{"conv1d_bf16cl", false};
  ov_conv1d_bf16_params p{};
  p.x = sptr<uint16_t>(x, c, 0); p.w = sptr<uint16_t>(w, c, 1); p.bias = sptr<float>(bias, c, 2);
  p.out = sptr<uint16_t>(out, c, 3); p.res = sptr<uint16_t>(res, c, 4); p.add = sptr<uint16_t>(add, c, 5);
  p.dbg = sptr<unsigned long long>(dbg, c, 6);
  p.B = (int32_t)ip[0]; p.L = (int32_t)ip[1]; p.Cin = (int32_t)ip[2]; p.Cout = (int32_t)ip[3]; p.K = (int32_t)ip[4];
  p.dil = (int32_t)ip[5]; p.phase_s = (int32_t)ip[6]; p.bias_bstride = (int32_t)ip[7]; p.layout = (int32_t)ip[8];
  p.in_slope = (float)fp[0]; p.scale = (float)fp[1]; p.out_slope = (float)fp[2];
  DeviceScope scope(c);
  finish(ov_conv1d_bf16cl(&p, c.stream()), "ov_conv1d_bf16cl");
}

void resblock_pair_bf16cl(const OptTensor& x, const OptTensor& w1, const OptTensor& b1, const OptTensor& w2,
                          const OptTensor& b2, const OptTensor& out, const OptTensor& add, const OptTensor& dbg,
                          at::IntArrayRef ip, at::ArrayRef<double> fp) {
  TORCH_CHECK(ip.size() == 6 && fp.size() == 2, "openvoice_amd::resblock_pair_bf16cl: 6 integer and 2 float parameters");
  Ctx c{"resblock_pair_bf16cl", false};
  ov_respair_bf16_params p{};
  p.x = sptr<uint16_t>(x, c, 0); p.w1 = sptr<uint16_t>(w1, c, 1); p.b1 = sptr<float>(b1, c, 2);
  p.w2 = sptr<uint16_t>(w2, c, 3); p.b2 = sptr<float>(b2, c, 4); p.out = sptr<uint16_t>(out, c, 5);
  p.add = sptr<uint16_t>(add, c, 6);
  p.dbg = sptr<unsigned long long>(dbg, c, 7);
  p.B = (int32_t)ip[0]; p.L = (int32_t)ip[1]; p.C = (int32_t)ip[2]; p.K = (int32_t)ip[3]; p.dil = (int32_t)ip[4];
  p.nwg = (int32_t)ip[5];
  p.slope = (float)fp[0]; p.scale = (float)fp[1];
  DeviceScope scope(c);
  finish(ov_resblock_pair_bf16cl(&p, c.stream()), "ov_resblock_pair_bf16cl");
}

void resblock_pair2_bf16cl(const OptTensor& x, const OptTensor& w1, const OptTensor& b1, const OptTensor& w2,
                           const OptTensor& b2, const OptTensor& out, const OptTensor& add, const OptTensor& dbg,
                           at::IntArrayRef ip, at::ArrayRef<double> fp) {
  TORCH_CHECK(ip.size() == 7 && fp.size() == 3, "openvoice_amd::resblock_pair2_bf16cl: 7 integer and 3 float parameters");
  Ctx c{"resblock_pair2_bf16cl", false};
  ov_respair2_bf16_params p{};
  p.x = sptr<uint16_t>(x, c, 0); p.w1 = sptr<uint16_t>(w1, c, 1); p.b1 = sptr<float>(b1, c, 2);
  p.w2 = sptr<uint16_t>(w2, c, 3); p.b2 = sptr<float>(b2, c, 4); p.out = sptr<uint16_t>(out, c, 5);
  p.add = sptr<uint16_t>(add, c, 6);
  p.dbg = sptr<unsigned long long>(dbg, c, 7);
  p.B = (int32_t)ip[0]; p.L = (int32_t)ip[1]; p.C = (int32_t)ip[2]; p.K = (int32_t)ip[3]; p.dil = (int32_t)ip[4];
  p.nwg = (int32_t)ip[5]; p.exp_flags = (int32_t)ip[6];
  p.slope = (float)fp[0]; p.scale = (float)fp[1]; p.out_slope = (float)fp[2];
  DeviceScope scope(c);
  finish(ov_resblock_pair2_bf16cl(&p, c.stream()), "ov_resblock_pair2_bf16cl");
}

void conv1d_split3(const OptTensor& x, const OptTensor& w, const OptTensor& bias, const OptTensor& out, const OptTensor& res,
                   const OptTensor& dbg, const OptTensor& col_limit, at::IntArrayRef ip, at::ArrayRef<double> fp) {
  TORCH_CHECK(ip.size() == 12 && fp.size() == 3, "openvoice_amd::conv1d_split3: 12 integer and 3 float parameters");
  Ctx c{"conv1d_split3", false};
  ov_conv1d_split3_params p{};
  p.x = sptr<uint16_t>(x, c, 0); p.w = sptr<uint16_t>(w, c, 1); p.bias = sptr<float>(bias, c, 2);
  p.out = sptr<uint16_t>(out, c, 3); p.res = sptr<uint16_t>(res, c, 4);
  p.dbg = sptr<unsigned long long>(dbg, c, 5);
  p.col_limit = sptr<int32_t>(col_limit, c, 6);
  p.B = (int32_t)ip[0]; p.L = (int32_t)ip[1]; p.Cin = (int32_t)ip[2]; p.Cout = (int32_t)ip[3]; p.K = (int32_t)ip[4];
  p.dil = (int32_t)ip[5]; p.nwg = (int32_t)ip[6]; p.products = (int32_t)ip[7];
  p.x_plane = ip[8]; p.out_plane = ip[9]; p.res_plane = ip[10]; p.col_limit_scale = (int32_t)ip[11];
  p.res_slope = (float)fp[0]; p.out_slope = (float)fp[1]; p.scale = (float)fp[2];
  DeviceScope scope(c);
  finish(ov_conv1d_split3(&p, c.stream()), "ov_conv1d_split3");
}

void conv1d_wino_f32(const OptTensor& x, const OptTensor& w, const OptTensor& bias, const OptTensor& out, const OptTensor& res,
                     const OptTensor& add, const OptTensor& dbg, const OptTensor& col_limit, at::IntArrayRef ip,
                     at::ArrayRef<double> fp) {
  TORCH_CHECK(ip.size() == 15 && fp.size() == 3, "openvoice_amd::conv1d_wino_f32: 15 integer and 3 float parameters");
  Ctx c{"conv1d_wino_f32", false};
  ov_conv1d_wino_params p{};
  p.x = sptr<float>(x, c, 0); p.w = sptr<float>(w, c, 1); p.bias = sptr<float>(bias, c, 2);
  p.out = sptr<float>(out, c, 3); p.res = sptr<float>(res, c, 4); p.add = sptr<float>(add, c, 5);
  p.dbg = sptr<unsigned long long>(dbg, c, 6);
  p.col_limit = sptr<int32_t>(col_limit, c, 7); p.col_limit_scale = (int32_t)ip[14];
  p.B = (int32_t)ip[0]; p.Cin = (int32_t)ip[1]; p.Cout = (int32_t)ip[2]; p.L = (int32_t)ip[3];
  p.x_ld = (int32_t)ip[4]; p.out_ld = (int32_t)ip[5]; p.K = (int32_t)ip[6]; p.dil = (int32_t)ip[7]; p.nwg = (int32_t)ip[8];
  p.x_bstride = ip[9]; p.out_bstride = ip[10]; p.res_bstride = ip[11]; p.add_bstride = ip[12]; p.frags = (int32_t)ip[13];
  p.in_slope = (float)fp[0]; p.scale = (float)fp[1]; p.out_slope = (float)fp[2];
  DeviceScope scope(c);
  finish(ov_conv1d_wino_f32(&p, c.stream()), "ov_conv1d_wino_f32");
}

void conv1d_wino_multi_f32(const OptTensor& x0, const OptTensor& w0, const OptTensor& b0, const OptTensor& o0, const OptTensor& r0,
                           const OptTensor& a0, const OptTensor& x1, const OptTensor& w1, const OptTensor& b1, const OptTensor& o1,
                           const OptTensor& r1, const OptTensor& a1, const OptTensor& x2, const OptTensor& w2, const OptTensor& b2,
                           const OptTensor& o2, const OptTensor& r2, const OptTensor& a2, const OptTensor& col_limit, int64_t n,
                           at::IntArrayRef ip, at::ArrayRef<double> fp) {
  TORCH_CHECK(n >= 1 && n <= 3 && (int64_t)ip.size() == 15 * n && (int64_t)fp.size() == 3 * n,
              "openvoice_amd::conv1d_wino_multi_f32: 1 .. 3 convs, 15 integer and 3 float parameters each");
  Ctx c{"conv1d_wino_multi_f32", false};
  const OptTensor* t[3][6] = {{&x0, &w0, &b0, &o0, &r0, &a0}, {&x1, &w1, &b1, &o1, &r1, &a1}, {&x2, &w2, &b2, &o2, &r2, &a2}};
  ov_conv1d_wino_params ps[3] = {};
  const int32_t* lim = sptr<int32_t>(col_limit, c, 18);
  for (int64_t i = 0; i < n; ++i) {
    ov_conv1d_wino_params& p = ps[i];
    const int64_t* q = ip.data() + 15 * i;
    const int k = 6 * (int)i;
    p.x = sptr<float>(*t[i][0], c, k); p.w = sptr<float>(*t[i][1], c, k + 1); p.bias = sptr<float>(*t[i][2], c, k + 2);
    p.out = sptr<float>(*t[i][3], c, k + 3); p.res = sptr<float>(*t[i][4], c, k + 4); p.add = sptr<float>(*t[i][5], c, k + 5);
    p.col_limit = lim; p.col_limit_scale = (int32_t)q[14];
    p.B = (int32_t)q[0]; p.Cin = (int32_t)q[1]; p.Cout = (int32_t)q[2]; p.L = (int32_t)q[3];
    p.x_ld = (int32_t)q[4]; p.out_ld = (int32_t)q[5]; p.K = (int32_t)q[6]; p.dil = (int32_t)q[7]; p.nwg = (int32_t)q[8];
    p.x_bstride = q[9]; p.out_bstride = q[10]; p.res_bstride = q[11]; p.add_bstride = q[12]; p.frags = (int32_t)q[13];
    p.in_slope = (float)fp[3 * i]; p.scale = (float)fp[3 * i + 1]; p.out_slope = (float)fp[3 * i + 2];
  }
  DeviceScope scope(c);
  finish(ov_conv1d_wino_multi_f32(ps, (int)n, c.stream()), "ov_conv1d_wino_multi_f32");
}

}

TORCH_LIBRARY(openvoice_amd, m) {
  m.def("conv1d_f32(Tensor? x, Tensor? w, Tensor? bias, Tensor(a!)? out, Tensor? res, Tensor? add, Tensor(b!)? out2, "
        "Tensor? mask, Tensor? bias_b, Tensor? col_limit, int[] ip, float[] fp) -> ()", &conv1d_f32);
  m.def("resblock_pair_f32(Tensor? x, Tensor? w1, Tensor? b1, Tensor? w2, Tensor? b2, Tensor(a!)? out, Tensor? add, "
        "Tensor(b!)? dbg, Tensor? col_limit, int[] ip, float[] fp) -> ()", &resblock_pair_f32);
  m.def("wn_layer_f32(Tensor? x, Tensor(a!)? out, Tensor(b!)? skip, Tensor? w_in, Tensor? b_in, Tensor? cond, Tensor? w_rs, "
        "Tensor? b_rs, Tensor? mask, Tensor(c!)? dbg, Tensor(d!)? acts, int[] ip) -> ()", &wn_layer_f32);
  m.def("wn_layer_wino_f32(Tensor? x, Tensor(a!)? out, Tensor(b!)? skip, Tensor? w_in, Tensor? b_in, Tensor? cond, Tensor? w_rs, "
        "Tensor? b_rs, Tensor? mask, Tensor(c!)? dbg, Tensor(d!)? acts, int[] ip) -> ()", &wn_layer_wino_f32);
  m.def("wn_layer_bf16(Tensor? x, Tensor(a!)? out, Tensor(b!)? skip, Tensor? w_in, Tensor? b_in, Tensor? cond, Tensor? w_rs, "
        "Tensor? b_rs, Tensor? mask, Tensor(c!)? dbg, Tensor(d!)? acts, int[] ip) -> ()", &wn_layer_bf16);
  m.def("conv1d_bf16cl(Tensor? x, Tensor? w, Tensor? bias, Tensor(a!)? out, Tensor? res, Tensor? add, Tensor(b!)? dbg, "
        "int[] ip, float[] fp) -> ()", &conv1d_bf16cl);
  m.def("resblock_pair_bf16cl(Tensor? x, Tensor? w1, Tensor? b1, Tensor? w2, Tensor? b2, Tensor(a!)? out, Tensor? add, "
        "Tensor(b!)? dbg, int[] ip, float[] fp) -> ()", &resblock_pair_bf16cl);
  m.def("resblock_pair2_bf16cl(Tensor? x, Tensor? w1, Tensor? b1, Tensor? w2, Tensor? b2, Tensor(a!)? out, Tensor? add, "
        "Tensor(b!)? dbg, int[] ip, float[] fp) -> ()", &resblock_pair2_bf16cl);
  m.def("conv1d_split3(Tensor? x, Tensor? w, Tensor? bias, Tensor(a!)? out, Tensor? res, Tensor(b!)? dbg, "
        "Tensor? col_limit, int[] ip, float[] fp) -> ()", &conv1d_split3);
  m.def("conv1d_wino_f32(Tensor? x, Tensor? w, Tensor? bias, Tensor(a!)? out, Tensor? res, Tensor? add, Tensor(b!)? dbg, "
        "Tensor? col_limit, int[] ip, float[] fp) -> ()",
        &conv1d_wino_f32);
  m.def("conv1d_wino_multi_f32(Tensor? x0, Tensor? w0, Tensor? b0, Tensor(a!)? o0, Tensor? r0, Tensor? a0, Tensor? x1, Tensor? w1, "
        "Tensor? b1, Tensor(b!)? o1, Tensor? r1, Tensor? a1, Tensor? x2, Tensor? w2, Tensor? b2, Tensor(c!)? o2, Tensor? r2, "
        "Tensor? a2, Tensor? col_limit, int n, int[] ip, float[] fp) -> ()",
        &conv1d_wino_multi_f32);
  bind_device<&ov_frame_hops_f32>(m, "frame_hops_f32");
  bind_device<&ov_frame_hops_windows_f32>(m, "frame_hops_windows_f32");
  bind_device<&ov_frame_hops_multi_f32>(m, "frame_hops_multi_f32");
  bind_device<&ov_carry_rows_f32>(m, "carry_rows_f32");
  bind_device<&ov_rows_f32_to_cl_bf16>(m, "rows_f32_to_cl_bf16");
  bind_device<&ov_cl_bf16_to_rows_f32>(m, "cl_bf16_to_rows_f32");
  bind_device<&ov_vad_frame_energy_f32>(m, "vad_frame_energy_f32");
  bind_device<&ov_vad_segments_i32>(m, "vad_segments_i32");
  bind_device<&ov_vad_compact_f32>(m, "vad_compact_f32");
  bind_device<&ov_join_segments_f32>(m, "join_segments_f32");
  bind_device<&ov_pack_groups_cl_bf16>(m, "pack_groups_cl_bf16");
  bind_device<&ov_unpack_groups_f32>(m, "unpack_groups_f32");
  bind_device<&ov_normal_philox_f32>(m, "normal_philox_f32");
  bind_device<&ov_stitch_window_cores_f32>(m, "stitch_window_cores_f32");
  bind_device<&ov_conv_post_tanh_f32>(m, "conv_post_tanh_f32");
  bind_device<&ov_conv_post_tanh_limited_f32>(m, "conv_post_tanh_limited_f32");
  bind_device<&ov_frame_limits_i32>(m, "frame_limits_i32");
  bind_device<&ov_linear_f32>(m, "linear_f32");
  bind_device<&ov_sequence_mask_f32>(m, "sequence_mask_f32");
  bind_device<&ov_unpad_rows_f32>(m, "unpad_rows_f32");
  bind_device<&ov_polyphase_fir_f32>(m, "polyphase_fir_f32");
  bind_device<&ov_polyphase_fir_rows_f32>(m, "polyphase_fir_rows_f32");
  bind_device<&ov_layernorm_freq_f32>(m, "layernorm_freq_f32");
  bind_device<&ov_conv2d_s2_relu_f32>(m, "conv2d_s2_relu_f32");
  bind_device<&ov_gru_f32>(m, "gru_f32");
  bind_device<&ov_layernorm_freq_ragged_f32>(m, "layernorm_freq_ragged_f32");
  bind_device<&ov_conv2d_s2_relu_ragged_f32>(m, "conv2d_s2_relu_ragged_f32");
  bind_device<&ov_gru_ragged_f32>(m, "gru_ragged_f32");
  bind_device<&ov_embed_f32>(m, "embed_f32");
  bind_device<&ov_layernorm_ch_f32>(m, "layernorm_ch_f32");
  bind_device<&ov_rel_attention_f32>(m, "rel_attention_f32");
  bind_device<&ov_dwconv1d_f32>(m, "dwconv1d_f32");
  bind_device<&ov_expand1_f32>(m, "expand1_f32");
  bind_device<&ov_add_bias_mask_f32>(m, "add_bias_mask_f32");
  bind_device<&ov_rq_spline_inverse_f32>(m, "rq_spline_inverse_f32");
  bind_device<&ov_duration_f32>(m, "duration_f32");
  bind_device<&ov_expand_prior_f32>(m, "expand_prior_f32");
  bind_device<&ov_duration_items_f32>(m, "duration_items_f32");
  bind_device<&ov_expand_prior_items_f32>(m, "expand_prior_items_f32");
  bind_device<&ov_conv_post_tanh_bf16>(m, "conv_post_tanh_bf16");
  bind_device<&ov_split3_from_f32>(m, "split3_from_f32");
  bind_device<&ov_split3_to_f32>(m, "split3_to_f32");
  bind_host<&ov_conv1d_pack_f32>(m, "conv1d_pack_f32");
  bind_host<&ov_wn_pack_f32>(m, "wn_pack_f32");
  bind_host<&ov_wn_wino_pack_f32>(m, "wn_wino_pack_f32");
  bind_value<&ov_wn_wino_pack_size>(m, "wn_wino_pack_size");
  bind_value<&ov_wn_layer_wino_tile>(m, "wn_layer_wino_tile");
  bind_host<&ov_wn_bf16_pack>(m, "wn_bf16_pack");
  bind_value<&ov_wn_bf16_pack_size>(m, "wn_bf16_pack_size");
  bind_value<&ov_wn_layer_bf16_supported>(m, "wn_layer_bf16_supported");
  bind_value<&ov_wn_layer_bf16_tile>(m, "wn_layer_bf16_tile");
  bind_host<&ov_conv1d_bf16_pack>(m, "conv1d_bf16_pack");
  bind_host<&ov_conv1d_bf16_pack16>(m, "conv1d_bf16_pack16");
  bind_host<&ov_conv1d_split3_pack>(m, "conv1d_split3_pack");
  bind_value<&ov_conv1d_split3_pack_size>(m, "conv1d_split3_pack_size");
  bind_value<&ov_conv1d_split3_supported>(m, "conv1d_split3_supported");
  bind_host<&ov_conv1d_wino_pack_f32>(m, "conv1d_wino_pack_f32");
  bind_value<&ov_conv1d_wino_pack_size>(m, "conv1d_wino_pack_size");
  bind_value<&ov_conv1d_wino_supported>(m, "conv1d_wino_supported");
  bind_value<&ov_conv1d_wino_chunk>(m, "conv1d_wino_chunk");
  bind_value<&ov_conv1d_pack_size>(m, "conv1d_pack_size");
  bind_value<&ov_conv1d_pack_rows>(m, "conv1d_pack_rows");
  bind_value<&ov_wn_pack_size>(m, "wn_pack_size");
  bind_value<&ov_conv1d_bf16_pack_size>(m, "conv1d_bf16_pack_size");
  bind_value<&ov_resblock_pair_supported>(m, "resblock_pair_supported");
  bind_value<&ov_wn_layer_supported>(m, "wn_layer_supported");
  bind_value<&ov_wn_layer_tile>(m, "wn_layer_tile");
  bind_value<&ov_resblock_pair_bf16_supported>(m, "resblock_pair_bf16_supported");
  bind_value<&ov_resblock_pair2_bf16_supported>(m, "resblock_pair2_bf16_supported");
  bind_value<&ov_version>(m, "version");
  bind_value<&ov_build_experiment>(m, "build_experiment");
}
```

openvoice_amd/engine.py:

```python
import contextlib
import ctypes
import functools
import os

import torch

from . import _lib
from . import noise as noise_mod
from ._lib import (ConvParams, EPI_CONVT, EPI_COUPLE, EPI_GATE, EPI_LINEAR, EPI_POSTERIOR, EPI_RESSKIP,
                   F_CONVT_GROUPED, F_MASK_V, F_OUT2_INIT)
from .generator import (FINAL_LRELU_SLOPE, GENERATOR_MARGIN, LRELU_SLOPE, conv_transpose_as_conv,
                        generator_margin_frames, generator_stages, resblock_convs, samples_per_frame, scratch_per_frame)
from .params import ENC_Q_LAYERS, FLOW_LAYERS, N_FLOWS, REF_ENC_FILTERS, REF_ENC_GRU, effective_weight

LIMIT_MAX_BATCH = 256


SUPPORTED_RESBLOCK_KERNELS = (3, 7, 11)
SUPPORTED_RESBLOCK_DILATIONS = (1, 3, 5)


def validate_config(cfg):
    def bad(field, value, why):
        raise _lib.OvError(f"config field {field!r} = {value!r} is not supported by the MI355X kernels: {why}")

    rb = str(cfg.get("resblock", "1"))
    if rb != "1":
        bad("resblock", cfg.get("resblock"), "only ResBlock1 ('1') is built (ResBlock2 is not; reference "
            "openvoice/models.py:242, modules.py:312-357)")
    kernels, dils = list(cfg["resblock_kernel_sizes"]), [list(d) for d in cfg["resblock_dilation_sizes"]]
    if len(kernels) != len(dils) or not kernels:
        bad("resblock_dilation_sizes", cfg["resblock_dilation_sizes"], f"one dilation list per entry of "
            f"resblock_kernel_sizes ({len(kernels)}) is required")
    for k in kernels:
        if k not in SUPPORTED_RESBLOCK_KERNELS:
            bad("resblock_kernel_sizes", kernels, f"kernel size {k} has no conv instance (built: "
                f"{SUPPORTED_RESBLOCK_KERNELS})")
    for d in dils:
        for v in d:
            if v not in SUPPORTED_RESBLOCK_DILATIONS:
                bad("resblock_dilation_sizes", dils, f"dilation {v} has no conv instance (built: "
                    f"{SUPPORTED_RESBLOCK_DILATIONS})")
    rates, uk = list(cfg["upsample_rates"]), list(cfg["upsample_kernel_sizes"])
    if len(rates) != len(uk) or not rates:
        bad("upsample_kernel_sizes", uk, f"one kernel size per entry of upsample_rates ({len(rates)}) is required")
    for (i, cin, ch, u, *_), k in zip(generator_stages(cfg), uk):
        if k != 2 * u:
            bad("upsample_kernel_sizes", uk, f"stage {i}: the transposed conv is built as a 3-tap phase conv, which needs "
                f"kernel == 2 * stride (got kernel {k}, stride {u})")
        if u <= 0 or 32 % u != 0:
            bad("upsample_rates", rates, f"stage {i}: stride {u} must divide 32 (phases are interleaved inside one "
                f"32-row fragment)")
        if cin % 2 != 0 or ch % 32 != 0:
            bad("upsample_initial_channel", cfg["upsample_initial_channel"], f"stage {i} would have {ch} channels; "
                f"every stage needs a multiple of 32 (whole MFMA fragments)")
    if cfg["hidden_channels"] % 32 != 0:
        bad("hidden_channels", cfg["hidden_channels"], "must be a multiple of 32 (the WaveNet gate rows are paired in "
            "32-row MFMA fragments)")
    if cfg["inter_channels"] % 64 != 0:
        bad("inter_channels", cfg["inter_channels"], "must be a multiple of 64 (the couplings split the channels in halves "
            "of whole 32-row fragments)")


def on_own_device(method):
    import functools

    @functools.wraps(method)
    def wrapper(self, *args, **kwargs):
        dev = getattr(self, "device", None)
        if dev is None:
            dev = (getattr(self, "engine", None) or kwargs.get("engine") or args[0]).device
        with torch.cuda.device(dev):
            return method(self, *args, **kwargs)
    return wrapper


def wavenet_keyword(method):
    @functools.wraps(method)
    def wrapper(self, *args, wavenet=None, **kwargs):
        if _lib.check_wavenet(wavenet, optional=True) is None:
            return method(self, *args, **kwargs)
        with contextlib.ExitStack() as stack:
            for core in self._wavenet_cores():
                stack.enter_context(core.wavenet_scope(wavenet))
            return method(self, *args, **kwargs)
    wrapper.__doc__ = (method.__doc__ or "") + ("\n        ``wavenet`` (keyword only): None follows ``use_bf16_wavenet``; "
                                               "``\"fp32\"`` / ``\"bf16\"`` choose the WaveNet layers' kernels for this call "
                                               "(``engine.wavenet_keyword``).")
    return wrapper


def _ptr(t, offset_elems=0):
    return ctypes.c_void_p(t.data_ptr() + 4 * offset_elems)


class PackedConv:

    def __init__(self, w_dense, bias, device, K, dil=1, cout=None):
        w_dense = w_dense.detach().to(torch.float32).cpu().contiguous()
        rows, cin, k = w_dense.shape
        assert k == K
        self.rows = rows
        self.cout = rows if cout is None else cout
        self.cin, self.K, self.dil = cin, K, dil
        n = _lib.call("ov_conv1d_pack_size", rows, cin, K)
        packed = torch.empty(n, dtype=torch.float32)
        _lib.call("ov_conv1d_pack_f32", w_dense, rows, cin, K, packed)
        self.w = packed.to(device)
        pack_rows = _lib.call("ov_conv1d_pack_rows", rows)
        b = torch.zeros(pack_rows, dtype=torch.float32)
        if bias is not None:
            b[:rows] = bias.detach().float().cpu()
        self.has_bias = bias is not None
        self.bias = b.to(device)


def padded_frames(T):
    return (T + 3) // 4 * 4


def ref_enc_lengths(T, n_convs=len(REF_ENC_FILTERS)):
    T = int(T)
    if T < 1:
        raise ValueError(f"ref_enc_lengths: T must be >= 1, got {T}")
    out = [T]
    for _ in range(n_convs):
        out.append((out[-1] - 1) // 2 + 1)
    return out


def gate_row_order(hidden):
    assert hidden % 32 == 0
    idx = []
    for q in range(hidden // 32):
        idx += list(range(32 * q, 32 * q + 32)) + list(range(hidden + 32 * q, hidden + 32 * q + 32))
    return torch.tensor(idx, dtype=torch.long)


def convt_row_order(cout, stride):
    s = stride
    if s == 8 and cout % 8 == 0:
        per_tile = 8
    elif s == 2 and cout % 32 == 0:
        per_tile = 32
    else:
        return None
    idx = []
    for q in range(cout // per_tile):
        for grp in range(2):
            for c in range(per_tile):
                for ph in range(s // 2):
                    idx.append((q * per_tile + c) * s + grp * (s // 2) + ph)
    return torch.tensor(idx, dtype=torch.long)


_EXTRA_CONV_FLAGS = int(os.environ.get("OPENVOICE_AMD_CONV_FLAGS", "0"))
if _EXTRA_CONV_FLAGS & ~_lib.F_NO_XCD_MAP:
    raise _lib.OvError(f"OPENVOICE_AMD_CONV_FLAGS={_EXTRA_CONV_FLAGS}: only the measurement bit OV_F_NO_XCD_MAP "
                       f"({_lib.F_NO_XCD_MAP}) may be set from the environment")


def launch_conv(layer, x, x_off, x_bs, out, out_off, out_bs, B, L, epi=EPI_LINEAR, flags=0, in_slope=1.0,
                scale=1.0, res=None, res_off=0, res_bs=0, add=None, add_bs=0, out2=None, out2_bs=0, mask=None,
                bias_b=None, bias_b_off=0, bias_b_bs=0, split=0, phase_s=1, cin=None, rows=None, tiles_per_wg=0,
                x_ld=0, out_ld=0, mask_bs=0, tile=0, loaders=0, chunk=0, col_limit=None, col_limit_scale=1):
    flags |= _EXTRA_CONV_FLAGS
    if _lib.use_torch_binding():
        ip = [B, layer.cin if cin is None else cin, L, x_ld, out_ld, layer.rows if rows is None else rows, layer.cout,
              layer.K, layer.dil, epi, flags, split, phase_s, tiles_per_wg, tile, loaders, chunk,
              x_bs, out_bs, res_bs, add_bs, out2_bs, bias_b_bs, mask_bs, x_off, out_off, res_off, bias_b_off,
              col_limit_scale]
        _lib.torch_op("conv1d_f32", x, layer.w, layer.bias, out, res, add, out2, mask, bias_b, col_limit, ip,
                      [in_slope, scale])
        return
    p = ConvParams()
    p.x, p.w = _ptr(x, x_off), _ptr(layer.w)
    p.bias = _ptr(layer.bias)
    p.bias_b = _ptr(bias_b, bias_b_off) if bias_b is not None else None
    p.out = _ptr(out, out_off)
    p.res = _ptr(res, res_off) if res is not None else None
    p.add = _ptr(add) if add is not None else None
    p.out2 = _ptr(out2) if out2 is not None else None
    p.mask = _ptr(mask) if mask is not None else None
    p.x_bstride, p.out_bstride, p.res_bstride = x_bs, out_bs, res_bs
    p.add_bstride, p.out2_bstride, p.bias_b_bstride = add_bs, out2_bs, bias_b_bs
    p.B, p.Cin, p.L = B, layer.cin if cin is None else cin, L
    p.M = layer.rows if rows is None else rows
    p.Cout = layer.cout
    p.K, p.dil, p.epi, p.flags, p.split, p.phase_s = layer.K, layer.dil, epi, flags, split, phase_s
    p.in_slope, p.scale = in_slope, scale
    p.tiles_per_wg, p.tile, p.loaders, p.chunk = tiles_per_wg, tile, loaders, chunk
    p.x_ld, p.out_ld, p.mask_bstride = x_ld, out_ld, mask_bs
    p.col_limit = ctypes.c_void_p(col_limit.data_ptr()) if col_limit is not None else None
    p.col_limit_scale = col_limit_scale
    stream = ctypes.c_void_p(torch.cuda.current_stream(x.device).cuda_stream)
    _lib.check(_lib.load().ov_conv1d_f32(ctypes.byref(p), stream), "ov_conv1d_f32")


def launch_pair(c1, c2, x, x_bs, out, out_bs, B, L, add=None, add_bs=0, scale=1.0, slope=LRELU_SLOPE, ld=0, nwg=0,
                dbg=None, col_limit=None, col_limit_scale=1):
    if _lib.use_torch_binding():
        _lib.torch_op("resblock_pair_f32", x, c1.w, c1.bias, c2.w, c2.bias, out, add, dbg, col_limit,
                      [B, c1.cin, L, ld, c1.K, c1.dil, nwg, x_bs, out_bs, add_bs, col_limit_scale], [slope, scale])
        return
    p = _lib.RespairParams()
    p.x, p.w1, p.b1, p.w2, p.b2 = _ptr(x), _ptr(c1.w), _ptr(c1.bias), _ptr(c2.w), _ptr(c2.bias)
    p.out = _ptr(out)
    p.add = _ptr(add) if add is not None else None
    p.x_bstride, p.out_bstride, p.add_bstride = x_bs, out_bs, add_bs
    p.B, p.C, p.L, p.ld, p.K, p.dil, p.nwg = B, c1.cin, L, ld, c1.K, c1.dil, nwg
    p.slope, p.scale = slope, scale
    p.dbg = ctypes.c_void_p(dbg.data_ptr()) if dbg is not None else None
    p.col_limit = ctypes.c_void_p(col_limit.data_ptr()) if col_limit is not None else None
    p.col_limit_scale = col_limit_scale
    stream = ctypes.c_void_p(torch.cuda.current_stream(x.device).cuda_stream)
    _lib.check(_lib.load().ov_resblock_pair_f32(ctypes.byref(p), stream), "ov_resblock_pair_f32")


_pair_supported = {}


def pair_supported(C, K, dil):
    key = (C, K, dil)
    if key not in _pair_supported:
        _pair_supported[key] = bool(_lib.call("ov_resblock_pair_supported", C, K, dil))
    return _pair_supported[key]


PAIR_POLICY = {(32, 3), (32, 7)}


def wino_policy(C, K, dil):
    return C >= 64 or dil == 1


WINO_MIN_ITEMS = 136

USE_MULTI_LAUNCH = True

SPLIT_MIN_CHANNELS = 128


def _wino_mw(cout):
    return 4 if cout % 128 == 0 else (2 if cout % 64 == 0 else 1)


def wino_ncol(cout, dil):
    return (256 if dil == 1 else 4 * (64 // dil) * dil) * (4 // _wino_mw(cout))


def wino_items(cout, dil, B, L):
    ncol = wino_ncol(cout, dil)
    return B * ((L + ncol - 1) // ncol) * (cout // (32 * _wino_mw(cout)))


DIRECT_MIN_NCOL = 128


def conv_reach(family, K, dil=1):
    if family in ("direct", "pair", "split3"):
        r = (K - 1) // 2 * dil
        return r, r
    if family == "wino":
        from . import wino
        G = (K + 2) // 3
        pad = (K - 1) // 2 + wino.LEAD_TAPS[K]
        return (pad + 2) * dil, (3 * (G - 1) + 4 - pad) * dil
    raise ValueError(f"unknown conv family {family!r}")


def resblock_families(C, K, dils, B, L, use_winograd=True, fuse_pairs=True):
    from . import wino
    if fuse_pairs and L % 4 == 0 and all((C, K) in PAIR_POLICY and pair_supported(C, K, d) for d in dils):
        return [("pair", "pair")] * len(dils)
    fam = lambda d: ("wino" if use_winograd and L % 4 == 0 and wino.supported(C, C, K, d) and wino_policy(C, K, d)
                     and wino_items(C, d, B, L) >= WINO_MIN_ITEMS else "direct")
    return [(fam(d), fam(1)) for d in dils]


def limit_margin_frames(cfg, B, T, use_winograd=True, fuse_pairs=True):
    stages = generator_stages(cfg)

    def chain_reach(i, k, dils):
        C, L = stages[i].ch, T * stages[i].rate_out
        fams = resblock_families(C, k, dils, B, L, use_winograd, fuse_pairs)
        return sum(conv_reach(f1, k, d)[1] + conv_reach(f2, k, 1)[1] for (f1, f2), d in zip(fams, dils))

    return max(GENERATOR_MARGIN, generator_margin_frames(cfg), generator_margin_frames(cfg, chain_reach=chain_reach))


def wn_fused_row_order(hidden):
    assert hidden % 8 == 0
    idx = []
    for q in range(hidden // 8):
        for j in range(4):
            a, b = 8 * q + j, 8 * q + j + 4
            idx += [a, b, hidden + a, hidden + b]
    return torch.tensor(idx, dtype=torch.long)


def wn_pack(w_dense, device):
    w_dense = w_dense.detach().to(torch.float32).cpu().contiguous()
    rows, cin, k = w_dense.shape
    n = _lib.call("ov_wn_pack_size", rows, cin, k)
    assert n > 0, (rows, cin, k)
    packed = torch.empty(n, dtype=torch.float32)
    _lib.call("ov_wn_pack_f32", w_dense, rows, cin, k, packed)
    return packed.to(device)


def wn_bf16_pack(w_dense, device):
    w_dense = w_dense.detach().to(torch.float32).cpu().contiguous()
    rows, cin, k = w_dense.shape
    n = _lib.call("ov_wn_bf16_pack_size", rows, cin, k)
    assert n > 0 and n % 2 == 0, (rows, cin, k)
    packed = torch.empty(n, dtype=torch.bfloat16)
    _lib.call("ov_wn_bf16_pack", w_dense, rows, cin, k, packed)
    return packed.view(torch.float32).to(device)


WN_WINO_MIN_ITEMS = 168
WN_WINO_ROUND = 256


def wn_wino_items(B, T):
    return B * ((T + 127) // 128)


def wn_wino_policy(B, T):
    items = wn_wino_items(B, T)
    rounds = (items + WN_WINO_ROUND - 1) // WN_WINO_ROUND
    return items >= WN_WINO_MIN_ITEMS * rounds


def wn_wino_pack(w_dense, device):
    w_dense = w_dense.detach().to(torch.float32).cpu().contiguous()
    rows, cin, k = w_dense.shape
    n = _lib.call("ov_wn_wino_pack_size", rows, cin, k)
    assert n > 0, (rows, cin, k)
    packed = torch.empty(n, dtype=torch.float32)
    _lib.call("ov_wn_wino_pack_f32", w_dense, rows, cin, k, packed)
    return packed.to(device)


def launch_wn_layer(layer, x, out, skip, mask, B, T, ld, cond=None, cond_off=0, cond_bs=0, first=False, last=False,
                    width=0, mask_bs=0, dbg=None, acts=None, row_split=0, winograd=False, bf16=False):
    entry, w_in = ("wn_layer_wino_f32", layer["w_in_wino"]) if winograd else ("wn_layer_f32", layer["w_in"])
    w_rs = layer["w_rs"]
    if bf16:
        entry, w_in, w_rs, acts, row_split = "wn_layer_bf16", layer["w_in_bf16"], layer["w_rs_bf16"], None, 0
    if _lib.use_torch_binding():
        H = layer["hidden"]
        _lib.torch_op(entry, x, out, skip, w_in, layer["b_in"], cond, w_rs, layer["b_rs"],
                      mask, dbg, acts, [B, H, T, ld, layer["K"], int(first), int(last), width, H * ld, cond_bs, mask_bs,
                                        cond_off, row_split])
        return
    p = _lib.WnLayerParams()
    p.x, p.out, p.skip = _ptr(x), _ptr(out), _ptr(skip)
    p.w_in, p.b_in, p.w_rs, p.b_rs = _ptr(w_in), _ptr(layer["b_in"]), _ptr(w_rs), _ptr(layer["b_rs"])
    p.cond = _ptr(cond, cond_off) if cond is not None else None
    p.mask = _ptr(mask)
    H = layer["hidden"]
    p.bstride, p.cond_bstride, p.mask_bstride = H * ld, cond_bs, mask_bs
    p.B, p.H, p.T, p.ld, p.K = B, H, T, ld, layer["K"]
    p.first, p.last, p.width, p.row_split = int(first), int(last), width, row_split
    p.dbg = ctypes.c_void_p(dbg.data_ptr()) if dbg is not None else None
    p.acts = _ptr(acts) if acts is not None else None
    stream = ctypes.c_void_p(torch.cuda.current_stream(x.device).cuda_stream)
    _lib.check(getattr(_lib.load(), "ov_" + entry)(ctypes.byref(p), stream), "ov_" + entry)


class _WaveNet:

    def __init__(self, sd, prefix, n_layers, hidden, device):
        order = gate_row_order(hidden)
        self.hidden, self.n_layers = hidden, n_layers
        self.in_layers, self.rs_layers, self.fused_layers = [], [], []
        self.device, self._sd, self._prefix = device, sd, prefix
        K = sd[f"{prefix}.in_layers.0.weight_v"].shape[2] if f"{prefix}.in_layers.0.weight_v" in sd else \
            sd[f"{prefix}.in_layers.0.weight"].shape[2]
        self.fused = bool(_lib.call("ov_wn_layer_supported", hidden, K))
        forder = wn_fused_row_order(hidden) if self.fused else None
        for i in range(n_layers):
            w_in = effective_weight(sd, f"{prefix}.in_layers.{i}")
            b_in = sd[f"{prefix}.in_layers.{i}.bias"].float()
            self.in_layers.append(PackedConv(w_in[order], b_in[order], device, K=w_in.shape[2], cout=hidden))
            w_rs = effective_weight(sd, f"{prefix}.res_skip_layers.{i}")
            b_rs = sd[f"{prefix}.res_skip_layers.{i}.bias"].float()
            self.rs_layers.append(PackedConv(w_rs, b_rs, device, K=1))
            if self.fused:
                if w_rs.shape[0] == hidden:
                    w_rs = torch.cat([torch.zeros_like(w_rs), w_rs])
                    b_rs = torch.cat([torch.zeros_like(b_rs), b_rs])
                self.fused_layers.append(dict(hidden=hidden, K=w_in.shape[2], w_in=wn_pack(w_in[forder], device),
                                              w_in_wino=wn_wino_pack(w_in[forder], device),
                                              b_in=b_in[forder].contiguous().to(device), w_rs=wn_pack(w_rs, device),
                                              b_rs=b_rs.contiguous().to(device)))
        wc = effective_weight(sd, prefix + ".cond_layer")[:, :, 0]
        bc = sd[prefix + ".cond_layer.bias"].float()
        full = torch.cat([order + 2 * hidden * i for i in range(n_layers)])
        self.cond_w = wc[full].contiguous().to(device)
        self.cond_b = bc[full].contiguous().to(device)
        if self.fused:
            full = torch.cat([forder + 2 * hidden * i for i in range(n_layers)])
            self.cond_w_fused = wc[full].contiguous().to(device)
            self.cond_b_fused = bc[full].contiguous().to(device)

    def bf16_layers(self):
        if not (self.fused and _lib.call("ov_wn_layer_bf16_supported", self.hidden, self.fused_layers[0]["K"])):
            raise _lib.OvError(f"no bf16 WaveNet layer kernel for hidden = {self.hidden}: a missing kernel is an error")
        if "w_in_bf16" not in self.fused_layers[0]:
            forder = wn_fused_row_order(self.hidden)
            for i, layer in enumerate(self.fused_layers):
                w_rs = effective_weight(self._sd, f"{self._prefix}.res_skip_layers.{i}")
                if w_rs.shape[0] == self.hidden:
                    w_rs = torch.cat([torch.zeros_like(w_rs), w_rs])
                layer["w_in_bf16"] = wn_bf16_pack(effective_weight(self._sd, f"{self._prefix}.in_layers.{i}")[forder],
                                                  self.device)
                layer["w_rs_bf16"] = wn_bf16_pack(w_rs, self.device)
        return self.fused_layers


def multi_launch_scratch_buffers(cfg):
    return 2 * (len(cfg["resblock_kernel_sizes"]) - 1)


_DEC_BUFFERS = 5


def _workspace_elems(cfg, B, T):
    H, C, Tp = cfg["hidden_channels"], cfg["inter_channels"], padded_frames(T)
    frame_rate = Tp + 4 * H * Tp + C * Tp + 3 * C * Tp + generator_stages(cfg)[0].cin * Tp
    return B * frame_rate, B * T * scratch_per_frame(cfg)


def _resblock_tree(sd, cfg, make, keep=lambda stage: True):
    convs = list(resblock_convs(cfg))
    layer = lambda c, name, d: make(c, effective_weight(sd, name), sd[name + ".bias"], d)
    return [[[(layer(c, f"{c.prefix}.convs1.{c.n}", c.dil), layer(c, f"{c.prefix}.convs2.{c.n}", 1))
              for c in convs if (c.stage, c.j) == (i, j)]
             for j in range(len(cfg["resblock_kernel_sizes"]))] if keep(i) else None
            for i in range(len(cfg["upsample_rates"]))]


class ConverterEngine:

    def __init__(self, state_dict, model_cfg, spec_channels, device, zero_g=False):
        self.device = torch.device(device)
        if self.device.type != "cuda":
            raise _lib.OvError("ConverterEngine needs a ROCm device ('cuda:N'); there is no CPU path")
        sd = {k: v.detach().float().cpu() for k, v in state_dict.items()}
        cfg = dict(model_cfg.items()) if hasattr(model_cfg, "items") else dict(model_cfg)
        validate_config(cfg)
        self.cfg = cfg
        self.zero_g = bool(zero_g)
        self.inter = cfg["inter_channels"]
        self.hidden = cfg["hidden_channels"]
        self.gin = cfg.get("gin_channels", 256)
        self.spec_channels = spec_channels
        dev = self.device
        H, C = self.hidden, self.inter
        half = C // 2
        self.q_pre = PackedConv(sd["enc_q.pre.weight"], sd["enc_q.pre.bias"], dev, K=1)
        self.q_wn = _WaveNet(sd, "enc_q.enc", ENC_Q_LAYERS, H, dev)
        order = gate_row_order(C)
        self.q_proj = PackedConv(sd["enc_q.proj.weight"][order], sd["enc_q.proj.bias"][order], dev, K=1, cout=C)
        self.couplings = []
        for f in range(N_FLOWS):
            p = f"flow.flows.{2 * f}"
            flipped = f % 2 == 1
            w_pre, w_post, b_post = sd[p + ".pre.weight"], sd[p + ".post.weight"], sd[p + ".post.bias"]
            if flipped:
                w_pre = torch.flip(w_pre, [1])
                w_post, b_post = torch.flip(w_post, [0]), torch.flip(b_post, [0])
            self.couplings.append(dict(
                flipped=flipped,
                pre=PackedConv(w_pre, sd[p + ".pre.bias"], dev, K=1),
                wn=_WaveNet(sd, p + ".enc", FLOW_LAYERS, H, dev),
                post=PackedConv(w_post, b_post, dev, K=1)))
        self.half = half
        self.conv_pre = PackedConv(sd["dec.conv_pre.weight"], sd["dec.conv_pre.bias"], dev, K=7)
        self.dec_cond_w = sd["dec.cond.weight"][:, :, 0].contiguous().to(dev)
        self.dec_cond_b = sd["dec.cond.bias"].contiguous().to(dev)
        self.stages = generator_stages(cfg)
        self.ups = []
        for i, _, ch, u, *_ in self.stages:
            wc = conv_transpose_as_conv(effective_weight(sd, f"dec.ups.{i}"), u)
            bias = sd[f"dec.ups.{i}.bias"].repeat_interleave(u)
            order = convt_row_order(ch, u)
            if order is not None:
                wc, bias = wc[order], bias[order]
            self.ups.append(dict(conv=PackedConv(wc, bias, dev, K=3, cout=ch), stride=u,
                                 flags=F_CONVT_GROUPED if order is not None else 0))
        self.resblocks = _resblock_tree(sd, cfg, lambda c, w, b, d: PackedConv(w, b, dev, K=c.K, dil=d))
        from . import wino as _wino
        self.wino_resblocks = _resblock_tree(sd, cfg, lambda c, w, b, d: _wino.PackedConvWino(w, b, dev, dil=d)
                                             if _wino.supported(c.ch, c.ch, c.K, d) and wino_policy(c.ch, c.K, d) else None)
        self.final_channels = self.stages[-1].ch
        self.post_w = sd["dec.conv_post.weight"][0].contiguous().to(dev)
        self.total_upsample = samples_per_frame(cfg)
        self.ref_enc = None
        if "ref_enc.gru.weight_ih_l0" in sd:
            convs = [(effective_weight(sd, f"ref_enc.convs.{i}").contiguous().to(dev),
                      sd[f"ref_enc.convs.{i}.bias"].contiguous().to(dev)) for i in range(len(REF_ENC_FILTERS))]
            w_ih = sd["ref_enc.gru.weight_ih_l0"]
            self.ref_enc = dict(
                ln_w=sd["ref_enc.layernorm.weight"].contiguous().to(dev),
                ln_b=sd["ref_enc.layernorm.bias"].contiguous().to(dev),
                convs=convs,
                gru_in=PackedConv(w_ih.unsqueeze(-1), sd["ref_enc.gru.bias_ih_l0"], dev, K=1),
                whh_t=sd["ref_enc.gru.weight_hh_l0"].t().contiguous().to(dev),
                bhh=sd["ref_enc.gru.bias_hh_l0"].contiguous().to(dev),
                proj_w=sd["ref_enc.proj.weight"].contiguous().to(dev),
                proj_b=sd["ref_enc.proj.bias"].contiguous().to(dev))
        self._ws, self._graphs, self._limit_margins = {}, {}, {}
        self._live_ws, self._live_ws_bf16, self.live_ws_builds = {}, {}, 0
        self.resident_workspaces = 1
        self.profile = None
        self.chain_streams = 1
        self.chain_streams_max_batch = 8
        self._streams = []
        self._zeros = {}
        self.generator_margin = max(GENERATOR_MARGIN, generator_margin_frames(self.cfg))
        self.fuse_wn = True
        self.wn_row_split = 0
        self.fuse_pairs = True
        self.use_winograd = True
        self.use_multi_launch = USE_MULTI_LAUNCH
        self._cus = None
        self._state_dict_for_bf16 = sd
        self.generator_bf16 = None
        self._bf16_on = False
        self._wn_bf16_on, self._wn_choice = False, None
        self._split3_on = False
        self.split3_products = 6
        self.split_resblocks = None

    def _stream(self):
        return ctypes.c_void_p(torch.cuda.current_stream(self.device).cuda_stream)

    def _timed(self, tag, flops, fn, *extra):
        if self.profile is None:
            return fn()
        e0, e1 = torch.cuda.Event(enable_timing=True), torch.cuda.Event(enable_timing=True)
        e0.record()
        out = fn()
        e1.record()
        self.profile.append((tag, flops, e0, e1) + extra)
        return out

    def _conv(self, layer, x, x_off, x_bs, out, out_off, out_bs, B, L, tag="conv", alg_flops=None, **kwargs):
        if alg_flops is None:
            alg_flops = 2.0 * layer.rows * (kwargs.get("cin") or layer.cin) * layer.K * L * B
        self._timed(tag, alg_flops, lambda: launch_conv(layer, x, x_off, x_bs, out, out_off, out_bs, B, L, **kwargs))

    def _wino(self, layer, x, out, bs, B, L, res=None, add=None, scale=1.0, in_slope=LRELU_SLOPE, out_slope=1.0, **lim):
        from . import wino
        kw = dict(in_slope=in_slope, out_slope=out_slope, scale=scale, res=res, res_bs=bs if res is not None else 0, add=add,
                  add_bs=bs if add is not None else 0, **lim)
        alg = 2.0 * layer.cout * layer.cin * layer.K * L * B
        self._timed("mrf", alg, lambda: wino.launch_conv_wino(layer, x, bs, out, bs, B, L, **kw),
                    alg * wino.PRODUCTS_PER_TILE[layer.K] / (4.0 * layer.K))

    def _wino_multi(self, convs, B, L, **lim):
        from . import wino
        alg = [2.0 * c["layer"].cout * c["layer"].cin * c["layer"].K * L * B for c in convs]
        exe = sum(a * wino.PRODUCTS_PER_TILE[c["layer"].K] / (4.0 * c["layer"].K) for a, c in zip(alg, convs))
        self._timed("mrf", sum(alg), lambda: wino.launch_convs_wino(convs, B, L, **lim), exe)

    def _pair(self, c1, c2, x, out, bs, B, L, add, scale, **lim):
        self._timed("mrf", 2 * 2.0 * c1.rows * c1.cin * c1.K * L * B,
                    lambda: launch_pair(c1, c2, x, bs, out, bs, B, L, add=add, add_bs=bs, scale=scale, **lim))

    def _linear(self, x2d, w, b):
        Bg, Kd = x2d.shape
        M = w.shape[0]
        y = torch.empty(Bg, M, dtype=torch.float32, device=self.device)
        _lib.call("ov_linear_f32", x2d, w, b, y, Bg, M, Kd)
        return y

    def _wn_cond(self, wn, g):
        if self.fuse_wn and wn.fused:
            return self._linear(g, wn.cond_w_fused, wn.cond_b_fused)
        return self._linear(g, wn.cond_w, wn.cond_b)

    def _workspace(self, B, T):
        key = (B, T)
        ws = self._ws.pop(key, None)
        if ws is not None:
            self._ws[key] = ws
        else:
            while self._ws and len(self._ws) >= max(1, int(self.resident_workspaces)):
                self._ws.pop(next(iter(self._ws)))
            dev, H, C = self.device, self.hidden, self.inter
            Tp = padded_frames(T)
            f = lambda *shape: torch.zeros(*shape, dtype=torch.float32, device=dev)
            lat = f(3, B, C, Tp)
            ws = dict(Tp=Tp, mask=f(B, Tp), h=f(B, H, Tp), h2=f(B, H, Tp), acts=f(B, H, Tp), skip=f(B, H, Tp), noise=f(B, C, Tp),
                      lat=lat, z=lat[0], z_p=lat[1], z_hat=lat[2])
            ws["pre"] = f(B, self.stages[0].cin, Tp)
            dec = _workspace_elems(self.cfg, B, T)[1]
            ws["dec"] = [torch.empty(dec, dtype=torch.float32, device=dev) for _ in range(_DEC_BUFFERS)]
            self._chain_scratch(ws, self._multi_launch_scratch(B, T))
            self._ws[key] = ws
        return ws

    def workspace_bytes(self, B, T):
        frame_rate, dec = _workspace_elems(self.cfg, B, T)
        return 4 * (frame_rate + (_DEC_BUFFERS + self._multi_launch_scratch(B, T)) * dec)

    def _zeros_like_cached(self, t):
        key = tuple(t.shape)
        z = self._zeros.get(key)
        if z is None:
            z = self._zeros[key] = torch.zeros_like(t)
        return z

    def _side_streams(self, n):
        while len(self._streams) < n:
            self._streams.append(torch.cuda.Stream(self.device))
        return self._streams[:n]

    def _chain_scratch(self, ws, n):
        extra = ws.setdefault("dec_extra", [])
        while len(extra) < n:
            extra.append(torch.empty_like(ws["dec"][0]))
        return extra

    def _wavenet(self, wn, ws, B, T, cond, mask):
        H, Tp = wn.hidden, ws["Tp"]
        cbs = 0 if cond.shape[0] == 1 else cond.shape[1]
        if self.wavenet_bf16():
            if not self.fuse_wn:
                raise _lib.OvError("wavenet='bf16' runs the fused layer kernel: fuse_wn must be on")
            layers = wn.bf16_layers()
            src, dst = ws["h"], ws["h2"]
            for i in range(wn.n_layers):
                layer, last = layers[i], i == wn.n_layers - 1
                self._timed("wn_layer_bf16", 2.0 * (2 * H * H * layer["K"] + (H if last else 2 * H) * H) * T * B,
                            lambda: launch_wn_layer(layer, src, dst, ws["skip"], mask, B, T, Tp, cond=cond,
                                                    cond_off=2 * H * i, cond_bs=cbs, first=i == 0, last=last,
                                                    mask_bs=Tp, bf16=True))
                src, dst = dst, src
            return
        if self.fuse_wn and wn.fused:
            src, dst = ws["h"], ws["h2"]
            winograd = self.use_winograd and wn_wino_policy(B, T)
            for i in range(wn.n_layers):
                layer = wn.fused_layers[i]
                args = dict(cond=cond, cond_off=2 * H * i, cond_bs=cbs, first=i == 0, last=i == wn.n_layers - 1,
                            mask_bs=Tp, acts=ws["acts"], row_split=self.wn_row_split, winograd=winograd)
                rs_rows = H if args["last"] else 2 * H
                self._timed("wn_layer", 2.0 * (2 * H * H * layer["K"] + rs_rows * H) * T * B,
                            lambda: launch_wn_layer(layer, src, dst, ws["skip"], mask, B, T, Tp, **args))
                src, dst = dst, src
            return
        for i in range(wn.n_layers):
            self._conv(wn.in_layers[i], ws["h"], 0, H * Tp, ws["acts"], 0, H * Tp, B, T, epi=EPI_GATE,
                       bias_b=cond, bias_b_off=2 * H * i, bias_b_bs=cbs, rows=2 * H, x_ld=Tp, out_ld=Tp, tag="wn_in")
            last = i == wn.n_layers - 1
            self._conv(wn.rs_layers[i], ws["acts"], 0, H * Tp, ws["h"], 0, H * Tp, B, T, epi=EPI_RESSKIP,
                       flags=F_OUT2_INIT if i == 0 else 0, out2=ws["skip"], out2_bs=H * Tp, mask=mask, mask_bs=Tp,
                       split=0 if last else H, x_ld=Tp, out_ld=Tp, tag="wn_rs")

    def _flow(self, src, buf, ws, B, T, conds, mask, reverse):
        C, half, H, Tp = self.inter, self.half, self.hidden, ws["Tp"]
        order = range(N_FLOWS - 1, -1, -1) if reverse else range(N_FLOWS)
        for n, f in enumerate(order):
            cp = self.couplings[f]
            x0_off = half * Tp if cp["flipped"] else 0
            x1_off = 0 if cp["flipped"] else half * Tp
            self._conv(cp["pre"], src if n == 0 else buf, x0_off, C * Tp, ws["h"], 0, H * Tp, B, T, flags=F_MASK_V,
                       mask=mask, mask_bs=Tp, x_ld=Tp, out_ld=Tp, tag="cpl_pre")
            self._wavenet(cp["wn"], ws, B, T, conds[f], mask)
            self._conv(cp["post"], ws["skip"], 0, H * Tp, buf, x1_off, C * Tp, B, T, epi=EPI_COUPLE, mask=mask,
                       mask_bs=Tp, x_ld=Tp, out_ld=Tp, scale=-1.0 if reverse else 1.0, tag="cpl_post",
                       res=src if n < 2 else None, res_off=x1_off, res_bs=C * Tp)

    def _wavenet_cores(self):
        return (self,)

    @torch.no_grad()
    @on_own_device
    def voice_conversion(self, spec, spec_lengths, sid_src, sid_tgt, tau=1.0, noise=None, skip_padding=False, *,
                         seed=None, generator=None, wavenet=None):
        use_bf16 = self._bf16_on
        if _lib.check_generator(generator, optional=True) is not None:
            use_bf16 = generator == "bf16"
        with self.wavenet_scope(wavenet):
            return self._voice_conversion(spec, spec_lengths, sid_src, sid_tgt, tau, noise, skip_padding, seed, use_bf16)

    def _voice_conversion(self, spec, spec_lengths, sid_src, sid_tgt, tau, noise, skip_padding, seed, use_bf16):
        dev = self.device
        spec = spec.to(dev, torch.float32)
        B, F, T = spec.shape
        assert F == self.spec_channels
        if not (spec.stride(2) == 1 and spec.stride(1) >= T and spec.stride(0) >= F * spec.stride(1)):
            spec = spec.contiguous()
        C = self.inter
        lengths = spec_lengths.to(dev, torch.int64).contiguous()
        g_src = sid_src.to(dev, torch.float32).reshape(sid_src.shape[0], -1).contiguous()
        g_tgt = sid_tgt.to(dev, torch.float32).reshape(sid_tgt.shape[0], -1).contiguous()
        noise_mod.exclusive(seed, noise=noise)
        ws = self._workspace(B, T)
        Tp, mask = ws["Tp"], ws["mask"]
        if seed is not None:
            self.seed_noise(ws["noise"], seed, B, T, Tp)
        elif noise is None:
            ws["noise"][:, :, :T].normal_()
        else:
            ws["noise"][:, :, :T].copy_(noise.to(dev, torch.float32))
        _lib.call("ov_sequence_mask_f32", lengths, mask, B, T, Tp)
        conds = self._conds(g_src, g_tgt)
        self._frames(ws, 0, B, spec, conds, tau)
        z, z_p, z_hat = ws["z"], ws["z_p"], ws["z_hat"]
        if use_bf16:
            g_d = self._zeros_like_cached(g_tgt) if self.zero_g else g_tgt
            o_hat = self._timed("gen_bf16", 0.0, lambda: self.bf16_generator().decode(z_hat[:, :, :T], g_d.unsqueeze(-1)))
            if skip_padding:
                keep_samples = (lengths.clamp(max=T) * self.total_upsample).view(B, 1, 1)
                o_hat.masked_fill_(torch.arange(o_hat.shape[2], device=dev).view(1, 1, -1) >= keep_samples, 0.0)
        else:
            limits = self.frame_limits(lengths, T) if skip_padding else None
            o_hat = self.decode(z_hat, conds["d"], ws, T=T, limits=limits)
        dense = torch.empty(3, B, C, T, dtype=torch.float32, device=dev)
        _lib.call("ov_unpad_rows_f32", ws["lat"], dense, 3 * B * C, T, Tp)
        y_mask = torch.empty(B, 1, T, dtype=torch.float32, device=dev)
        _lib.call("ov_unpad_rows_f32", mask, y_mask, B, T, Tp)
        return o_hat, y_mask, (dense[0], dense[1], dense[2])

    def seed_noise(self, dst, seed, B, T, ld, purpose=noise_mod.PURPOSE_POSTERIOR):
        C = self.inter
        noise_mod.fill([(s, k, purpose, f0, T, b * C * ld, ld) for b, (s, k, f0) in enumerate(noise_mod.rows(seed, B))],
                       C, dst)

    def _frames(self, ws, b0, b1, spec, conds, tau):
        nb, T, Tp = b1 - b0, spec.shape[2], ws["Tp"]
        C, H = self.inter, self.hidden
        sub = {k: (v[b0:b1] if torch.is_tensor(v) else v) for k, v in ws.items() if k != "dec"}
        rows = lambda t: t if t.shape[0] == 1 else t[b0:b1]
        mask = sub["mask"]
        x = spec[b0:b1]
        self._conv(self.q_pre, x, 0, spec.stride(0), sub["h"], 0, H * Tp, nb, T, flags=F_MASK_V, mask=mask, mask_bs=Tp,
                   x_ld=spec.stride(1), out_ld=Tp, tag="q_pre")
        self._wavenet(self.q_wn, sub, nb, T, rows(conds["q"]), mask)
        z, z_p, z_hat = sub["z"], sub["z_p"], sub["z_hat"]
        self._conv(self.q_proj, sub["skip"], 0, H * Tp, z, 0, C * Tp, nb, T, epi=EPI_POSTERIOR, res=sub["noise"],
                   res_bs=C * Tp, scale=float(tau), mask=mask, mask_bs=Tp, rows=2 * C, x_ld=Tp, out_ld=Tp, tag="q_proj")
        self._flow(z, z_p, sub, nb, T, [rows(c) for c in conds["src"]], mask, reverse=False)
        self._flow(z_p, z_hat, sub, nb, T, [rows(c) for c in conds["tgt"]], mask, reverse=True)

    def graphed(self, B, T, tau, src_rows=1, tgt_rows=1, max_cached=4, skip_padding=False):
        key = (int(B), int(T), float(tau), int(src_rows), int(tgt_rows), self._bf16_on,
               bool(skip_padding), bool(self._split3_on), self.split3_products, self.wavenet_bf16())
        cache = self._graphs
        g = cache.pop(key, None)
        if g is None:
            g = GraphedConversion(self, B, T, tau, src_rows, tgt_rows, skip_padding=skip_padding,
                                  wavenet="bf16" if key[-1] else "fp32")
            while len(cache) >= max_cached:
                cache.pop(next(iter(cache)))
        cache[key] = g
        return g

    def use_bf16_wavenet(self, enable=True):
        self._wn_bf16_on = bool(enable)
        self._graphs.clear()
        return self

    def wavenet_bf16(self):
        return self._wn_bf16_on if self._wn_choice is None else self._wn_choice == "bf16"

    @contextlib.contextmanager
    def wavenet_scope(self, wavenet):
        if _lib.check_wavenet(wavenet, optional=True) is None:
            yield self
            return
        saved, self._wn_choice = self._wn_choice, wavenet
        try:
            yield self
        finally:
            self._wn_choice = saved

    def use_bf16_generator(self, enable=True):
        if enable:
            self.bf16_generator()
        self._bf16_on = bool(enable)
        return self

    def bf16_generator(self):
        if self.generator_bf16 is None:
            from .bf16 import GeneratorBf16
            self.generator_bf16 = GeneratorBf16(self._state_dict_for_bf16, self.cfg, self.device)
        return self.generator_bf16

    def use_split_bf16x3(self, enable=True, products=6):
        if products not in (6, 3):
            raise _lib.OvError(f"use_split_bf16x3: products must be 6 or 3, got {products!r}")
        if enable and self.split_resblocks is None:
            from . import split3
            convs = list(resblock_convs(self.cfg))
            keep = lambda i: all(c.ch >= SPLIT_MIN_CHANNELS and split3.supported(c.ch, c.ch, c.K, c.dil)
                                 and split3.supported(c.ch, c.ch, c.K, 1) for c in convs if c.stage == i)
            self.split_resblocks = _resblock_tree(self._state_dict_for_bf16, self.cfg, lambda c, w, b, d:
                                                  split3.PackedConvSplit3(w, b, self.device, dil=d), keep)
        self._split3_on = bool(enable)
        self.split3_products = products
        self._graphs.clear()
        return self

    def _split_buffers(self, ws, B, st, L):
        nk = len(self.cfg["resblock_kernel_sizes"])
        need = 3 * B * L * st.ch
        bufs = ws.get("split3")
        if bufs is None:
            if torch.cuda.is_current_stream_capturing():
                raise _lib.OvError("split-precision plane buffers must exist before graph capture: run one eager conversion "
                                   "of this (batch, frames) shape first")
            frames = L // st.rate_out
            largest = max([need] + [3 * B * frames * o.rate_out * o.ch for o in self.stages
                                    if self.split_resblocks[o.index] is not None])
            bufs = ws["split3"] = [torch.empty(largest, dtype=torch.bfloat16, device=self.device) for _ in range(4 + nk)]
        assert bufs[0].numel() >= need
        return [b[:need].view(3, B, L, st.ch) for b in bufs]

    def _mrf_split(self, st, u, acc, ws, B, L, limits=None):
        from . import split3
        stage, ch = self.split_resblocks[st.index], st.ch
        nk = len(stage)
        bufs = self._split_buffers(ws, B, st, L)
        xa, t, ping, pong, results = bufs[0], bufs[1], bufs[2], bufs[3], bufs[4:]
        prod = self.split3_products
        lim = dict(col_limit=limits, col_limit_scale=st.rate_out) if limits is not None else {}
        timed = self._timed
        uv = u[:B * ch * L].view(B, ch, L)
        timed("split_layout", 0.0, lambda: split3.to_planes(uv, LRELU_SLOPE, out=xa))
        for j, pairs in enumerate(stage):
            cur = xa
            for n, (c1, c2) in enumerate(pairs):
                last = n == len(pairs) - 1
                flops = 2.0 * ch * ch * c1.K * L * B
                timed("mrf_split", flops, lambda: split3.launch_conv_split3(c1, cur, t, out_slope=LRELU_SLOPE, products=prod, **lim))
                dst = results[j] if last else (pong if cur is ping else ping)
                timed("mrf_split", flops, lambda: split3.launch_conv_split3(c2, t, dst, res=cur, res_slope=LRELU_SLOPE,
                                                                             out_slope=1.0 if last else LRELU_SLOPE,
                                                                             products=prod, **lim))
                cur = dst
        ops = list(results[:nk]) + [None] * (3 - nk)
        if nk > 3:
            raise _lib.OvError("split-precision MRF: at most 3 ResBlocks per stage")
        av = acc[:B * ch * L].view(B, ch, L)
        timed("split_layout", 0.0, lambda: split3.from_planes(ops[0], ops[1], ops[2], in_slope=1.0, scale=1.0 / nk, out=av))

    def limit_margin(self, B, T):
        key = (int(B), int(T), bool(self.use_winograd), bool(self.fuse_pairs))
        cache = self._limit_margins
        if key not in cache:
            cache[key] = max(self.generator_margin, limit_margin_frames(self.cfg, *key))
        return cache[key]

    def frame_limits(self, lengths, T):
        B = lengths.shape[0]
        lim = torch.empty(2, B, dtype=torch.int32, device=self.device)
        _lib.call("ov_frame_limits_i32", lengths, lim[0], B, int(T), self.limit_margin(B, T))
        _lib.call("ov_frame_limits_i32", lengths, lim[1], B, int(T), 0)
        return lim

    def _upsample(self, i, x, x_ld, u, B, L, cin, ch, **lim):
        up = self.ups[i]
        s = up["stride"]
        self._conv(up["conv"], x, 0, cin * x_ld, u, 0, ch * L * s, B, L, epi=EPI_CONVT, in_slope=LRELU_SLOPE,
                   flags=up["flags"], phase_s=s, x_ld=x_ld, tag="ups", alg_flops=2.0 * cin * ch * 2 * s * L * B, **lim)

    def _mrf(self, i, u, t1, ra, acc, ws, B, ch, L, limits, rate):
        cfg = self.cfg
        nk = len(cfg["resblock_kernel_sizes"])
        lim = lambda scale: dict(col_limit=limits, col_limit_scale=scale) if limits is not None else {}
        bs = ch * L
        concurrent = (self.chain_streams > 1 and nk > 1 and B <= self.chain_streams_max_batch and self.profile is None
                      and not (torch.cuda.is_current_stream_capturing() and len(ws.get("dec_extra", [])) < 2 * (nk - 1)))
        scratch = [(t1, ra)]
        if concurrent:
            extra = self._chain_scratch(ws, 2 * (nk - 1))
            scratch += [(extra[2 * j], extra[2 * j + 1]) for j in range(nk - 1)]

        def chain(j, pairs):
            t1_, ra_ = scratch[j if concurrent else 0]
            cur = u
            fams = resblock_families(ch, pairs[0][0].K, [c1.dil for c1, _ in pairs], B, L, self.use_winograd,
                                     self.fuse_pairs)
            fused = fams[0][0] == "pair"
            wn = self.wino_resblocks[i][j]
            for n, (c1, c2) in enumerate(pairs):
                last = n == len(pairs) - 1
                if last and concurrent and j > 0:
                    torch.cuda.current_stream(self.device).wait_event(done[j - 1])
                add = acc if (last and j > 0) else None
                scale = 1.0 / nk if (last and j == nk - 1) else 1.0
                if fused:
                    dst = acc if last else (t1_ if cur is ra_ else ra_)
                    self._pair(c1, c2, cur, dst, bs, B, L, add, scale, **lim(rate))
                else:
                    w1, w2 = (w if f == "wino" else None for w, f in zip(wn[n], fams[n]))
                    if w1 is not None:
                        self._wino(w1, cur, t1_, bs, B, L, out_slope=LRELU_SLOPE, **lim(rate))
                    else:
                        self._conv(c1, cur, 0, bs, t1_, 0, bs, B, L, in_slope=LRELU_SLOPE, tag="mrf", **lim(rate))
                    c2_slope = 1.0 if w1 is not None else LRELU_SLOPE
                    dst = acc if last else ra_
                    if w2 is not None:
                        self._wino(w2, t1_, dst, bs, B, L, res=cur, add=add, scale=scale, in_slope=c2_slope, **lim(rate))
                    else:
                        self._conv(c2, t1_, 0, bs, dst, 0, bs, B, L, in_slope=c2_slope, res=cur, res_bs=bs,
                                   add=add, add_bs=bs, scale=scale, tag="mrf", **lim(rate))
                cur = dst

        if not concurrent and self._mrf_multi(i, u, t1, ra, acc, ws, B, ch, L, lim(rate)):
            return
        if not concurrent:
            for j, pairs in enumerate(self.resblocks[i]):
                chain(j, pairs)
        else:
            main = torch.cuda.current_stream(self.device)
            side = self._side_streams(nk)
            fork = torch.cuda.Event()
            fork.record(main)
            done = [None] * nk
            for j, pairs in enumerate(self.resblocks[i]):
                with torch.cuda.stream(side[j]):
                    side[j].wait_event(fork)
                    chain(j, pairs)
                    done[j] = torch.cuda.Event()
                    done[j].record(side[j])
            for j in range(nk):
                main.wait_event(done[j])

    def _multi_launch_stage(self, i, B, ch, L):
        blocks = self.resblocks[i]
        nk = len(blocks)
        ks = [pairs[0][0].K for pairs in blocks]
        dils = [[c1.dil for c1, _ in pairs] for pairs in blocks]
        if not (self.use_multi_launch and self.use_winograd and 2 <= nk <= 3 and len(set(ks)) == nk and set(ks) <= {3, 7, 11}
                and ch % 64 == 0 and all(d == dils[0] for d in dils)):
            return False
        if self._cus is None:
            self._cus = torch.cuda.get_device_properties(self.device).multi_processor_count
        if wino_items(ch, 1, B, L) <= self._cus:
            return False
        fams = [resblock_families(ch, k, d, B, L, self.use_winograd, self.fuse_pairs) for k, d in zip(ks, dils)]
        return all(f == ("wino", "wino") for fam in fams for f in fam)

    def _multi_launch_scratch(self, B, T):
        return (multi_launch_scratch_buffers(self.cfg)
                if any(self._multi_launch_stage(st.index, B, st.ch, T * st.rate_out) for st in self.stages) else 0)

    def _mrf_multi(self, i, u, t1, ra, acc, ws, B, ch, L, lim):
        cfg = self.cfg
        blocks, wn = self.resblocks[i], self.wino_resblocks[i]
        nk = len(blocks)
        dils = [[c1.dil for c1, _ in pairs] for pairs in blocks]
        if not self._multi_launch_stage(i, B, ch, L):
            return False
        need = multi_launch_scratch_buffers(cfg)
        if torch.cuda.is_current_stream_capturing() and len(ws.get("dec_extra", [])) < need:
            return False
        extra = self._chain_scratch(ws, need)
        ts, ras = [t1] + extra[0:need:2], [ra] + extra[1:need:2]
        bs, npairs = ch * L, len(dils[0])
        cur = [u] * nk
        for n in range(npairs):
            self._wino_multi([dict(layer=wn[j][n][0], x=cur[j], out=ts[j], bs=bs, in_slope=LRELU_SLOPE, out_slope=LRELU_SLOPE)
                              for j in range(nk)], B, L, **lim)
            if n < npairs - 1:
                self._wino_multi([dict(layer=wn[j][n][1], x=ts[j], out=ras[j], bs=bs, res=cur[j]) for j in range(nk)], B, L, **lim)
                cur = list(ras)
            else:
                for j in range(nk):
                    self._wino(wn[j][n][1], ts[j], acc, bs, B, L, res=cur[j], add=acc if j > 0 else None,
                               scale=1.0 / nk if j == nk - 1 else 1.0, in_slope=1.0, **lim)
        return True

    def _stage(self, st, x, x_ld, x_bs, bufs, out, ws, B, L, cond_d=None, limits=None, keep=None):
        lim = lambda scale: dict(col_limit=limits, col_limit_scale=scale) if limits is not None else {}
        if st.index == 0:
            Tp = ws["Tp"]
            self._conv(self.conv_pre, x, 0, x_bs, ws["pre"], 0, st.cin * Tp, B, L, bias_b=cond_d,
                       bias_b_bs=0 if cond_d.shape[0] == 1 else cond_d.shape[1], x_ld=x_ld, out_ld=Tp, tag="conv_pre",
                       **lim(1))
            x, x_ld = ws["pre"], Tp
        u, t1, ra, acc = bufs
        self._upsample(st.index, x, x_ld, u, B, L, st.cin, st.ch, **lim(st.rate_in))
        L *= st.stride
        if t1 is None:
            self._mrf_split(st, u, acc, ws, B, L, limits=limits)
        else:
            self._mrf(st.index, u, t1, ra, acc, ws, B, st.ch, L, limits, st.rate_out)
        if st.last and keep is not None:
            _lib.call("ov_conv_post_tanh_limited_f32", acc, self.post_w, out, B, st.ch, L, self.post_w.shape[1],
                      FINAL_LRELU_SLOPE, keep, st.rate_out)
        elif st.last:
            _lib.call("ov_conv_post_tanh_f32", acc, self.post_w, out, B, st.ch, L, self.post_w.shape[1], FINAL_LRELU_SLOPE)

    def decode(self, z_hat, cond_d, ws=None, T=None, limits=None):
        B, C, ld = z_hat.shape
        T = ld if T is None else T
        if ws is None:
            ws = self._workspace(B, T)
        keep = None
        if limits is not None:
            limits, keep = limits[0], limits[1]
            if B > LIMIT_MAX_BATCH:
                limits = None
        o_hat = torch.empty(B, 1, T * self.total_upsample, dtype=torch.float32, device=self.device)
        x, x_ld, x_bs = z_hat, ld, C * ld
        free = list(ws["dec"])
        for st in self.stages:
            u = free.pop()
            if st.index > 0:
                free.append(x)
            split = self._split3_on and self.split_resblocks[st.index] is not None
            t1, ra = (None, None) if split else (free.pop(), free.pop())
            acc = free.pop()
            self._stage(st, x, x_ld, x_bs, (u, t1, ra, acc), o_hat, ws, B, T * st.rate_in, cond_d, limits, keep)
            free += [u] if split else [u, t1, ra]
            x, x_ld = acc, T * st.rate_out
        return o_hat

    def live_workspace(self, key, B, width, stage=None):
        cache = self._live_ws
        ws = cache.get((key, B))
        if ws is not None:
            assert ws["width"] >= width, "live unit wider than its workspace"
            return ws
        self.live_ws_builds += 1
        dev, H = self.device, self.hidden
        z = lambda *shape: torch.zeros(*shape, dtype=torch.float32, device=dev)
        Tp = padded_frames(width)
        if stage is None:
            ws = dict(Tp=Tp, mask=z(B, Tp), mask_len=-1, h=z(B, H, Tp), h2=z(B, H, Tp), acts=z(B, H, Tp),
                      skip=z(B, H, Tp))
        else:
            st = self.stages[stage]
            n = B * st.ch * width * st.stride
            ws = dict(Tp=Tp, dec=[z(n) for _ in range(3)])
            if stage == 0:
                ws["pre"] = z(B, st.cin, Tp)
            if st.last:
                ws["acc"] = z(n)
        ws["width"] = width
        cache[(key, B)] = ws
        return ws

    def _conds(self, g_src, g_tgt):
        g_q = self._zeros_like_cached(g_src) if self.zero_g else g_src
        g_d = self._zeros_like_cached(g_tgt) if self.zero_g else g_tgt
        return dict(q=self._wn_cond(self.q_wn, g_q), src=[self._wn_cond(cp["wn"], g_src) for cp in self.couplings],
                    tgt=[self._wn_cond(cp["wn"], g_tgt) for cp in self.couplings],
                    d=self._linear(g_d, self.dec_cond_w, self.dec_cond_b))

    live_conds = _conds

    def _live_mask(self, ws, B, L):
        if ws["mask_len"] != L:
            lengths = torch.full((B,), L, dtype=torch.int64, device=self.device)
            _lib.call("ov_sequence_mask_f32", lengths, ws["mask"], B, L, ws["Tp"])
            ws["mask_len"] = L
        return ws["mask"]

    @torch.no_grad()
    @on_own_device
    def live_posterior(self, spec, spec_ld, spec_bs, noise, noise_bs, out, ld, bs, B, L, cond_q, tau, ws):
        H, C, Tp = self.hidden, self.inter, ws["Tp"]
        mask = self._live_mask(ws, B, L)
        self._conv(self.q_pre, spec, 0, spec_bs, ws["h"], 0, H * Tp, B, L, flags=F_MASK_V, mask=mask, mask_bs=Tp,
                   x_ld=spec_ld, out_ld=Tp, tag="q_pre")
        self._wavenet(self.q_wn, ws, B, L, cond_q, mask)
        self._conv(self.q_proj, ws["skip"], 0, H * Tp, out, 0, bs, B, L, epi=EPI_POSTERIOR, res=noise, res_bs=noise_bs,
                   scale=float(tau), mask=mask, mask_bs=Tp, rows=2 * C, x_ld=Tp, out_ld=ld, tag="q_proj")

    @torch.no_grad()
    @on_own_device
    def live_flow(self, src, dst, B, L, conds, reverse, ws):
        self._flow(src, dst, ws, B, L, conds, self._live_mask(ws, B, L), reverse)

    @torch.no_grad()
    @on_own_device
    def live_generator_stage(self, i, x, x_ld, x_bs, out, B, L, ws, cond_d=None):
        if self._bf16_on or self._split3_on:
            raise _lib.OvError("live streams run the fp32 generator only (use_bf16_generator / split_bf16x3 are off)")
        st = self.stages[i]
        u, t1, ra = ws["dec"]
        self._stage(st, x, x_ld, x_bs, (u, t1, ra, ws["acc"] if st.last else out), out, ws, B, L, cond_d)

    @torch.no_grad()
    @on_own_device
    def live_cond_bf16(self, g_tgt):
        g_d = self._zeros_like_cached(g_tgt) if self.zero_g else g_tgt
        return self.bf16_generator().cond_rows(g_d)

    def live_workspace_bf16(self, key, B, width, stage):
        cache = self._live_ws_bf16
        ws = cache.get((key, B))
        if ws is not None:
            assert ws["width"] >= width, "live unit wider than its workspace"
            return ws
        self.live_ws_builds += 1
        f = lambda n: torch.empty(n, dtype=torch.bfloat16, device=self.device)
        st = self.stages[stage]
        n = self.bf16_generator().stage_scratch_elems(stage, B, width)
        ws = dict(width=width, xin=f(B * width * (self.inter if stage == 0 else st.cin)), out=None if st.last else f(n),
                  bufs=[f(n) for _ in range(4 if st.last else 3)], pre=f(B * width * st.cin) if stage == 0 else None)
        cache[(key, B)] = ws
        return ws

    @torch.no_grad()
    @on_own_device
    def live_generator_stage_bf16(self, i, x, x_ld, x_bs, out, B, L, ws, cond_d=None):
        if self._bf16_on or self._split3_on:
            raise _lib.OvError("a live unit's generator is chosen by its pool (use_bf16_generator / split_bf16x3 are off)")
        gen, st = self.bf16_generator(), self.stages[i]
        cin, s = self.inter if i == 0 else st.cin, st.stride
        xin = ws["xin"][: B * L * cin].view(B, L, cin)
        _lib.call("ov_rows_f32_to_cl_bf16", x, x_bs, x_ld, xin, B, cin, L)
        bufs = list(ws["bufs"])
        if st.last:
            gen.stage(i, xin, out[: B * L * s].view(B, 1, L * s), B, L, cond=cond_d, bufs=bufs, pre=ws["pre"])
            return
        o = ws["out"][: B * L * s * st.ch].view(B, L * s, st.ch)
        gen.stage(i, xin, o, B, L, cond=cond_d, bufs=bufs, pre=ws["pre"])
        _lib.call("ov_cl_bf16_to_rows_f32", o, out, st.ch * L * s, L * s, B, st.ch, L * s)

    @torch.no_grad()
    @on_own_device
    def reference_encoder(self, spec_t):
        re = self.ref_enc
        if re is None:
            raise _lib.OvError("this checkpoint has no ref_enc.* weights")
        dev = self.device
        x = spec_t.to(dev, torch.float32).transpose(1, 2).contiguous()
        N, F, T = x.shape
        assert F == self.spec_channels
        cur = torch.empty_like(x)
        _lib.call("ov_layernorm_freq_f32", x, re["ln_w"], re["ln_b"], cur, N, F, T, 1e-5)
        cin = 1
        for w, b in re["convs"]:
            cout = w.shape[0]
            Fo, To = (F - 1) // 2 + 1, (T - 1) // 2 + 1
            nxt = torch.empty(N, cout, Fo, To, dtype=torch.float32, device=dev)
            _lib.call("ov_conv2d_s2_relu_f32", cur, w, b, nxt, N, cin, cout, F, T)
            cur, cin, F, T = nxt, cout, Fo, To
        feat = cin * F
        H = REF_ENC_GRU
        gi = torch.empty(N, 3 * H, T, dtype=torch.float32, device=dev)
        self._conv(re["gru_in"], cur, 0, feat * T, gi, 0, 3 * H * T, N, T, tag="gru_in")
        h = torch.empty(N, H, dtype=torch.float32, device=dev)
        _lib.call("ov_gru_f32", gi, re["whh_t"], re["bhh"], h, N, H, T)
        return self._linear(h, re["proj_w"], re["proj_b"])

    @torch.no_grad()
    @on_own_device
    def reference_encoder_ragged(self, spec, frames):
        re = self.ref_enc
        cur, steps, L = self._reference_encoder_ragged_stack(spec, frames)
        P, H = cur.shape[0], REF_ENC_GRU
        feat = cur.shape[1] * cur.shape[2]
        gi = torch.empty(P, 3 * H, L, dtype=torch.float32, device=self.device)
        self._conv(re["gru_in"], cur, 0, feat * L, gi, 0, 3 * H * L, P, L, tag="gru_in")
        h = torch.empty(P, H, dtype=torch.float32, device=self.device)
        _lib.call("ov_gru_ragged_f32", gi, re["whh_t"], re["bhh"], steps, h, P, H, L)
        return self._linear(h, re["proj_w"], re["proj_b"])

    @torch.no_grad()
    @on_own_device
    def _reference_encoder_ragged_stack(self, spec, frames):
        re = self.ref_enc
        if re is None:
            raise _lib.OvError("this checkpoint has no ref_enc.* weights")
        dev = self.device
        x = spec.to(dev, torch.float32)
        if x.dim() != 3:
            raise ValueError(f"reference_encoder_ragged: spec must be [P, n_freq, W], got {tuple(x.shape)}")
        P, F, W = x.shape
        assert F == self.spec_channels
        frames = [int(f) for f in frames]
        if len(frames) != P or P < 1:
            raise ValueError(f"reference_encoder_ragged: {len(frames)} lengths for {P} items")
        if min(frames) < 1 or max(frames) > W:
            raise ValueError(f"reference_encoder_ragged: every length must be in [1, {W}], got {frames}")
        ld = x.stride(1)
        if x.stride() != (F * ld, ld, 1) or ld < W:
            x = x.contiguous()
            ld = W
        n_convs = len(re["convs"])
        table = torch.tensor([list(col) for col in zip(*(ref_enc_lengths(f, n_convs) for f in frames))],
                             dtype=torch.int32).to(dev)
        lds = ref_enc_lengths(ld, n_convs)
        cur = torch.empty(P, F, ld, dtype=torch.float32, device=dev)
        _lib.call("ov_layernorm_freq_ragged_f32", x, re["ln_w"], re["ln_b"], table[0], cur, P, F, ld, 1e-5)
        cin = 1
        for k, (w, b) in enumerate(re["convs"]):
            cout = w.shape[0]
            Fo = (F - 1) // 2 + 1
            nxt = torch.empty(P, cout, Fo, lds[k + 1], dtype=torch.float32, device=dev)
            _lib.call("ov_conv2d_s2_relu_ragged_f32", cur, w, b, table[k], nxt, P, cin, cout, F, lds[k], lds[k + 1])
            cur, cin, F = nxt, cout, Fo
        return cur, table[n_convs], lds[-1]


class GraphedConversion:

    @on_own_device
    def __init__(self, engine, B, T, tau, src_rows=1, tgt_rows=1, skip_padding=False, wavenet=None):
        dev = engine.device
        self.engine, self.B, self.T, self.tau = engine, int(B), int(T), float(tau)
        f = lambda *shape: torch.zeros(*shape, dtype=torch.float32, device=dev)
        self.spec = f(B, engine.spec_channels, padded_frames(T))[:, :, :T]
        self.lengths = torch.full((B,), T, dtype=torch.int64, device=dev)
        self.g_src, self.g_tgt = f(src_rows, engine.gin, 1), f(tgt_rows, engine.gin, 1)
        self.noise = f(B, engine.inter, T)
        run = lambda: engine.voice_conversion(self.spec, self.lengths, self.g_src, self.g_tgt, tau=self.tau,
                                              noise=self.noise, skip_padding=skip_padding, **_lib.wavenet_kw(wavenet))
        saved, engine.profile = engine.profile, None
        try:
            side = torch.cuda.Stream(dev)
            side.wait_stream(torch.cuda.current_stream(dev))
            with torch.cuda.stream(side):
                run()
            torch.cuda.current_stream(dev).wait_stream(side)
            self.workspace = engine._workspace(B, T)
            self.graph = torch.cuda.CUDAGraph()
            with torch.cuda.graph(self.graph):
                self.out = run()
        finally:
            engine.profile = saved

    @torch.no_grad()
    @on_own_device
    def __call__(self, spec, spec_lengths, sid_src, sid_tgt, noise=None, *, seed=None):
        noise_mod.exclusive(seed, noise=noise)
        if tuple(spec.shape) != (self.B, self.engine.spec_channels, self.T):
            raise _lib.OvError(f"graph captured for spec {(self.B, self.engine.spec_channels, self.T)}, got {tuple(spec.shape)}")
        self.spec.copy_(spec)
        self.lengths.copy_(spec_lengths)
        self.g_src.copy_(sid_src.reshape(self.g_src.shape))
        self.g_tgt.copy_(sid_tgt.reshape(self.g_tgt.shape))
        if seed is not None:
            self.engine.seed_noise(self.noise, seed, self.B, self.T, self.T)
        elif noise is None:
            self.noise.normal_()
        else:
            self.noise.copy_(noise)
        self.graph.replay()
        return self.out
```

Baseline: 3169 x real-time (audio s / wall s).

## Add Winograd F(2,2) transposed-conv upsample kernel for grouped ConvT stages

```diff
diff --git a/include/openvoice_amd.h b/include/openvoice_amd.h
--- a/include/openvoice_amd.h
+++ b/include/openvoice_amd.h
@@ -376,6 +376,10 @@
 size_t ov_conv1d_wino_pack_size(int Cout, int Cin, int K);
 int ov_conv1d_wino_pack_f32(const float* w, int Cout, int Cin, int K, float* dst);
 
+int ov_convt_f22_f32(const ov_conv1d_params* p, int32_t kt, int32_t col_offset, ov_stream_t stream);
+int ov_convt_f22_supported(int kt, int stride);
+int ov_convt_f22_pack_f32(const float* w, int rows, int Cin, float* dst);
+
 int ov_version(void);
 #define OV_ABI_VERSION 212
 int ov_build_experiment(void);
diff --git a/openvoice_amd/_lib.py b/openvoice_amd/_lib.py
--- a/openvoice_amd/_lib.py
+++ b/openvoice_amd/_lib.py
@@ -159,6 +159,9 @@
     "ov_conv1d_wino_chunk": (ctypes.c_int, [_i, _i]),
     "ov_conv1d_wino_pack_size": (ctypes.c_size_t, [_i, _i, _i]),
     "ov_conv1d_wino_pack_f32": (ctypes.c_int, [_fp, _i, _i, _i, _fp]),
+    "ov_convt_f22_f32": (ctypes.c_int, [ctypes.POINTER(ConvParams), ctypes.c_int32, ctypes.c_int32, _fp]),
+    "ov_convt_f22_supported": (ctypes.c_int, [_i, _i]),
+    "ov_convt_f22_pack_f32": (ctypes.c_int, [_fp, _i, _i, _fp]),
     "ov_frame_hops_f32": (ctypes.c_int, [_fp, _fp, _i, _i, _i, _i, _i, _i, _fp]),
     "ov_frame_hops_windows_f32": (ctypes.c_int, [_fp, _i64, _fp, _i, _i, _i, _i, _i, _fp, _fp]),
     "ov_frame_hops_multi_f32": (ctypes.c_int, [_fp, _i64, _fp, _i, _i, _i, _i, _i, _fp, _fp]),
@@ -278,7 +281,7 @@
                "ov_resblock_pair_bf16_supported", "ov_resblock_pair2_bf16_supported", "ov_conv1d_split3_pack_size",
                "ov_conv1d_split3_supported", "ov_conv1d_wino_supported", "ov_conv1d_wino_chunk", "ov_conv1d_wino_pack_size",
                "ov_wn_layer_wino_tile", "ov_wn_wino_pack_size", "ov_wn_layer_bf16_supported", "ov_wn_bf16_pack_size",
-               "ov_wn_layer_bf16_tile"}
+               "ov_wn_layer_bf16_tile", "ov_convt_f22_supported"}
 
 
 def binding():
diff --git a/openvoice_amd/csrc/conv1d_mfma.h b/openvoice_amd/csrc/conv1d_mfma.h
--- a/openvoice_amd/csrc/conv1d_mfma.h
+++ b/openvoice_amd/csrc/conv1d_mfma.h
@@ -9,7 +9,13 @@
 
 constexpr int EPI_CONVT_S8 = 16;
 constexpr int EPI_CONVT_S2 = 17;
-constexpr bool is_convt(int epi) { return epi == OV_EPI_CONVT || epi == EPI_CONVT_S8 || epi == EPI_CONVT_S2; }
+constexpr int EPI_CONVT_F22_S8 = 18;
+constexpr int EPI_CONVT_F22_S2 = 19;
+constexpr bool is_f22(int epi) { return epi == EPI_CONVT_F22_S8 || epi == EPI_CONVT_F22_S2; }
+constexpr bool is_convt(int epi) {
+  return epi == OV_EPI_CONVT || epi == EPI_CONVT_S8 || epi == EPI_CONVT_S2 || is_f22(epi);
+}
+constexpr int conv_nblk(int epi, int wn, int wvn) { return (is_f22(epi) ? 64 : 32) * wn * wvn; }
 
 typedef float f32x16 __attribute__((ext_vector_type(16)));
 typedef float f32x4 __attribute__((ext_vector_type(4)));
@@ -188,6 +194,86 @@
             for (int r = 0; r < 16; ++r) (outb + (size_t)((r & 3) + 8 * (r >> 2)) * LD)[voff] = v[r] * sg;
           }
         }
+      }
+    }
+  }
+}
+
+template <int WM, int WN>
+__device__ __forceinline__ void f22_init(const ov_conv1d_params& p, f32x16 (&acc)[WM][3 * WN], int mtile0, int lane) {
+  const uint32_t half = (uint32_t)lane >> 5;
+  const uint32_t row_limit = (uint32_t)p.Cout * (uint32_t)p.phase_s;
+#pragma unroll
+  for (int i = 0; i < WM; ++i) {
+    const uint32_t rbase = min((uint32_t)(mtile0 + i) * 32u, row_limit - 32u) + 4u * half;
+    f32x16 bv;
+#pragma unroll
+    for (int r = 0; r < 16; ++r) bv[r] = p.bias[rbase + (r & 3) + 8 * (r >> 2)];
+#pragma unroll
+    for (int j = 0; j < WN; ++j) {
+      acc[i][3 * j] = bv;
+#pragma unroll
+      for (int r = 0; r < 16; ++r) acc[i][3 * j + 1][r] = acc[i][3 * j + 2][r] = 0.f;
+    }
+  }
+}
+
+template <int EPI, int WM, int WN>
+__device__ __forceinline__ void f22_epilogue(const ov_conv1d_params& p, f32x16 (&acc)[WM][3 * WN], int b, int tcol0,
+                                             int mtile0, int lane) {
+  const uint32_t L = (uint32_t)p.L, Lout = (uint32_t)p.out_ld;
+  const uint32_t half = (uint32_t)lane >> 5;
+  const uint32_t ntile = (uint32_t)p.Cout * (uint32_t)p.phase_s / 32u;
+  float* outb = p.out + (int64_t)b * p.out_bstride;
+#pragma unroll
+  for (int j = 0; j < WN; ++j) {
+    const uint32_t col = (uint32_t)tcol0 + 64u * j + 2u * ((uint32_t)lane & 31u);
+    if (col >= L) continue;
+    const bool second = col + 1u < L;
+    if constexpr (EPI == EPI_CONVT_F22_S8) {
+#pragma unroll
+      for (int i = 0; i < WM; ++i) {
+        const uint32_t mt = (uint32_t)(mtile0 + i);
+        if (mt >= ntile) continue;
+        const uint32_t q = mt >> 1, g = mt & 1u;
+        const f32x16 y0 = acc[i][3 * j], p1 = acc[i][3 * j + 1], p2 = acc[i][3 * j + 2];
+#pragma unroll
+        for (int c = 0; c < 4; ++c) {
+          float* o = outb + (size_t)(q * 8u + 2u * c + half) * Lout + (8u * col + 4u * g);
+          const f32x4 e = {y0[4 * c] + p1[4 * c], y0[4 * c + 1] + p1[4 * c + 1], y0[4 * c + 2] + p1[4 * c + 2],
+                           y0[4 * c + 3] + p1[4 * c + 3]};
+          *reinterpret_cast<f32x4*>(o) = e;
+          if (second) {
+            const f32x4 d = {y0[4 * c] + p2[4 * c], y0[4 * c + 1] + p2[4 * c + 1], y0[4 * c + 2] + p2[4 * c + 2],
+                             y0[4 * c + 3] + p2[4 * c + 3]};
+            *reinterpret_cast<f32x4*>(o + 8) = d;
+          }
+        }
+      }
+    } else if constexpr (WM == 2) {
+      const uint32_t q = (uint32_t)mtile0 >> 1;
+      if ((uint32_t)mtile0 >= ntile) continue;
+#pragma unroll
+      for (int r = 0; r < 16; ++r) {
+        float* o = outb + (size_t)(q * 32u + 4u * half + (r & 3) + 8 * (r >> 2)) * Lout + 2u * col;
+        const float e0 = acc[0][3 * j][r] + acc[0][3 * j + 1][r], e1 = acc[1][3 * j][r] + acc[1][3 * j + 1][r];
+        if (second) {
+          const f32x4 v = {e0, e1, acc[0][3 * j][r] + acc[0][3 * j + 2][r], acc[1][3 * j][r] + acc[1][3 * j + 2][r]};
+          *reinterpret_cast<f32x4*>(o) = v;
+        } else {
+          const f32x2 v = {e0, e1};
+          *reinterpret_cast<f32x2*>(o) = v;
+        }
+      }
+    } else {
+      const uint32_t mt = (uint32_t)mtile0;
+      if (mt >= ntile) continue;
+      const uint32_t q = mt >> 1, g = mt & 1u;
+#pragma unroll
+      for (int r = 0; r < 16; ++r) {
+        float* o = outb + (size_t)(q * 32u + 4u * half + (r & 3) + 8 * (r >> 2)) * Lout + (2u * col + g);
+        o[0] = acc[0][3 * j][r] + acc[0][3 * j + 1][r];
+        if (second) o[2] = acc[0][3 * j][r] + acc[0][3 * j + 2][r];
       }
     }
   }
@@ -287,12 +373,15 @@
 constexpr int STAGE_VEC = 1;
 
 template <int K, int DIL, int WM, int WN, int WVM, int WVN, int CHUNK, int VEC, int EPI, int NLD>
-__global__ __launch_bounds__(64 * (4 + NLD), (EPI == OV_EPI_GATE || EPI == EPI_CONVT_S8 || EPI == EPI_CONVT_S2) ? 4 : 1) void conv1d_mfma_kernel(const ov_conv1d_params p) {
+__global__ __launch_bounds__(64 * (4 + NLD), (EPI == OV_EPI_GATE || EPI == EPI_CONVT_S8 || EPI == EPI_CONVT_S2 || (is_f22(EPI) && WM == 1)) ? 4 : (is_f22(EPI) ? 2 : 1)) void conv1d_mfma_kernel(const ov_conv1d_params p) {
   static_assert(WVM * WVN == 4, "4 matrix waves per workgroup");
   static_assert(VEC == STAGE_SCALAR || VEC == STAGE_VEC, "staging kind");
   static_assert(CHUNK % UNIT == 0 && (CHUNK / UNIT == 2 || CHUNK / UNIT == 4), "chunk = 2 or 4 units");
   constexpr int UPC = CHUNK / UNIT;
-  constexpr int N_BLK = 32 * WN * WVN;
+  constexpr bool F22 = is_f22(EPI);
+  static_assert(!F22 || (K == 3 && DIL == 1 && WM <= 2), "F(2, 2): the 3-tap phase form, one tile or one tile pair per wave");
+  constexpr int N_BLK = conv_nblk(EPI, WN, WVN);
+  constexpr int WNA = F22 ? 3 * WN : WN;
   constexpr int PAD = (K % 2 == 1) ? (K - 1) * DIL / 2 : 0;
   constexpr int PADR = (K - 1) * DIL - PAD;
   constexpr int PADA = (PAD + 3) / 4 * 4;
@@ -457,7 +546,8 @@
 #pragma unroll
   for (int i = 0; i < WM; ++i) widx[i] = (uint32_t)(mtile0 + i) * (uint32_t)recs_per_mtile * 64u + (uint32_t)lane;
 
-  const int xl_off = (lane >> 5) * XS + wn * (32 * WN) + (lane & 31) + (PADA - PAD);
+  const int xl_off = F22 ? (lane >> 5) * XS + wn * (64 * WN) + 2 * (lane & 31) + (PADA - PAD)
+                         : (lane >> 5) * XS + wn * (32 * WN) + (lane & 31) + (PADA - PAD);
 
   f32x4 a_cur[WM], a_nxt[WM];
 #pragma unroll
@@ -472,16 +562,66 @@
 #endif
   int it = 0;
   while (true) {
-    f32x16 acc[WM][WN];
-    const bool preloaded = conv_preload<EPI, WM, WN>(p, acc, b, tile * N_BLK + wn * (32 * WN), mtile0, lane);
+    f32x16 acc[WM][WNA];
+    bool preloaded = false;
+    if constexpr (F22) f22_init<WM, WN>(p, acc, mtile0, lane);
+    else preloaded = conv_preload<EPI, WM, WN>(p, acc, b, tile * N_BLK + wn * (32 * WN), mtile0, lane);
     OV_MARK(0)
 
     int rec = 0;
     for (int chunk = 0; chunk < nchunks; ++chunk, ++it) {
       if (OV_EXP != 1) __syncthreads();
       OV_MARK(1)
-      const float* xl = xs + (it & 1) * BUF + xl_off;
+      const float* xl = xs + (it & 1) * BUF + xl_off + ((F22 && WM == 1) ? (mtile0 & 1) : 0);
       constexpr int STEPS = UPC * 4 * K;
+      if constexpr (F22) {
+        constexpr int DOFF[3] = {1, 0, 2};
+        float bcur[WM][WN], bnxt[WM][WN], bmid[WM][WN];
+#pragma unroll
+        for (int i = 0; i < WM; ++i)
+#pragma unroll
+          for (int j = 0; j < WN; ++j) bcur[i][j] = bmid[i][j] = xl[64 * j + i + DOFF[0]];
+#pragma unroll
+        for (int sa = 0; sa < STEPS; ++sa) {
+          const int u = sa & 3;
+          if (u == 0) {
+            ++rec;
+#pragma unroll
+            for (int i = 0; i < WM; ++i) a_nxt[i] = (wbase + (size_t)rec * 64)[widx[i]];
+          }
+          if (sa + 1 < STEPS) {
+            const int uu = (sa + 1) / (4 * K), sn = (sa + 1) - uu * (4 * K);
+            const int pp = sn / K, kk = sn - pp * K;
+#pragma unroll
+            for (int i = 0; i < WM; ++i)
+#pragma unroll
+              for (int j = 0; j < WN; ++j) bnxt[i][j] = xl[(uu * UNIT + 2 * pp) * XS + 64 * j + i + DOFF[kk]];
+          }
+          __builtin_amdgcn_sched_barrier(0);
+          const int k_now = (sa % (4 * K)) % K;
+#pragma unroll
+          for (int i = 0; i < WM; ++i)
+#pragma unroll
+            for (int j = 0; j < WN; ++j) {
+              float opnd;
+              if (k_now == 0) { opnd = bcur[i][j]; bmid[i][j] = bcur[i][j]; }
+              else if (k_now == 1) opnd = bcur[i][j] - bmid[i][j];
+              else opnd = bmid[i][j] - bcur[i][j];
+              acc[i][3 * j + k_now] = __builtin_amdgcn_mfma_f32_32x32x2f32(a_cur[i][u], opnd, acc[i][3 * j + k_now], 0, 0, 0);
+            }
+          __builtin_amdgcn_sched_barrier(0);
+          if (sa + 1 < STEPS) {
+#pragma unroll
+            for (int i = 0; i < WM; ++i)
+#pragma unroll
+              for (int j = 0; j < WN; ++j) bcur[i][j] = bnxt[i][j];
+          }
+          if (u == 3) {
+#pragma unroll
+            for (int i = 0; i < WM; ++i) a_cur[i] = a_nxt[i];
+          }
+        }
+      } else {
       float bcur[WN], bnxt[WN];
 #pragma unroll
       for (int j = 0; j < WN; ++j) bcur[j] = xl[32 * j];
@@ -516,6 +656,7 @@
 #pragma unroll
           for (int i = 0; i < WM; ++i) a_cur[i] = a_nxt[i];
         }
+      }
       }
       OV_MARK(2)
     }
@@ -531,7 +672,8 @@
 #pragma unroll
       for (int i = 0; i < WM; ++i) a_cur[i] = wbase[nwidx[i]];
     }
-    conv_epilogue<EPI, WM, WN>(p, acc, b, tile * N_BLK + wn * (32 * WN), mtile0, mblk * WVM + wm, lane, preloaded);
+    if constexpr (F22) f22_epilogue<EPI, WM, WN>(p, acc, b, tile * N_BLK + wn * (64 * WN), mtile0, lane);
+    else conv_epilogue<EPI, WM, WN>(p, acc, b, tile * N_BLK + wn * (32 * WN), mtile0, mblk * WVM + wm, lane, preloaded);
     OV_MARK(3)
 #if OV_EXP == 3
     ++tph[4];
@@ -584,7 +726,7 @@
 
 template <int K, int DIL, int WM, int WN, int WVM, int WVN, int CHUNK, int VEC, int EPI, int NLD>
 int conv1d_launch(const ov_conv1d_params* p, hipStream_t stream) {
-  constexpr int M_BLK = 32 * WM * WVM, N_BLK = 32 * WN * WVN;
+  constexpr int M_BLK = 32 * WM * WVM, N_BLK = conv_nblk(EPI, WN, WVN);
   const int ntiles = (p->L + N_BLK - 1) / N_BLK;
   const int mblocks = (p->M + M_BLK - 1) / M_BLK;
   const long total = (long)ntiles * mblocks * p->B;
@@ -600,7 +742,8 @@
   return hipGetLastError() == hipSuccess ? OV_OK : OV_E_LAUNCH;
 }
 
-enum { TILE_128x128 = 0, TILE_64x256 = 1, TILE_32x512 = 2, TILE_32x256 = 3 };
+enum { TILE_128x128 = 0, TILE_64x256 = 1, TILE_32x512 = 2, TILE_32x256 = 3,
+       TILE_F22_64x128 = 4, TILE_F22W_128x128 = 5, TILE_F22W_64x256 = 6, TILE_F22X_128x128 = 7, TILE_F22X_64x256 = 8 };
 
 struct ConvVariant {
   int K, dil, tile, chunk, vec, epi, nld;
@@ -611,6 +754,11 @@
 #define OV_TILE_64x256 2, 2, 1, 4
 #define OV_TILE_32x512 1, 4, 1, 4
 #define OV_TILE_32x256 1, 2, 1, 4
+#define OV_TILE_F22_64x128 1, 1, 2, 2
+#define OV_TILE_F22W_128x128 2, 1, 2, 2
+#define OV_TILE_F22W_64x256 2, 1, 1, 4
+#define OV_TILE_F22X_128x128 1, 2, 4, 1
+#define OV_TILE_F22X_64x256 1, 2, 2, 2
 
 #define OV_X_INST(K, DIL, TILE, CHUNK, VEC, EPI, NLD)                                                        \
   template __global__ void conv1d_mfma_kernel<K, DIL, OV_TILE_##TILE, CHUNK, VEC, EPI, NLD>(                  \
@@ -638,5 +786,6 @@
 OV_DECLARE_VARIANTS(kVariantsF)
 OV_DECLARE_VARIANTS(kVariantsS)
 OV_DECLARE_VARIANTS(kVariantsW)
-
-}
+OV_DECLARE_VARIANTS(kVariantsT)
+
+}
diff --git a/openvoice_amd/csrc/convt_f22.hip b/openvoice_amd/csrc/convt_f22.hip
--- /dev/null
+++ b/openvoice_amd/csrc/convt_f22.hip
@@ -0,0 +1,97 @@
+#include <hip/hip_runtime.h>
+
+#include <cstdint>
+#include <cstring>
+
+#include "conv1d_mfma.h"
+#include "openvoice_amd.h"
+
+namespace ovk {
+#define LIST(X) \
+  X(3, 1, F22X_128x128, 32, 1, EPI_CONVT_F22_S8, 4) \
+  X(3, 1, F22X_128x128, 32, 0, EPI_CONVT_F22_S8, 4) \
+  X(3, 1, F22_64x128, 32, 1, EPI_CONVT_F22_S8, 4) \
+  X(3, 1, F22_64x128, 32, 0, EPI_CONVT_F22_S8, 4) \
+  X(3, 1, F22X_128x128, 32, 1, EPI_CONVT_F22_S2, 4) \
+  X(3, 1, F22X_128x128, 32, 0, EPI_CONVT_F22_S2, 4) \
+  X(3, 1, F22W_128x128, 32, 1, EPI_CONVT_F22_S2, 4) \
+  X(3, 1, F22W_128x128, 32, 0, EPI_CONVT_F22_S2, 4) \
+  X(3, 1, F22W_64x256, 32, 1, EPI_CONVT_F22_S2, 4) \
+  X(3, 1, F22W_64x256, 32, 0, EPI_CONVT_F22_S2, 4) \
+  X(3, 1, F22X_64x256, 32, 1, EPI_CONVT_F22_S2, 4) \
+  X(3, 1, F22X_64x256, 32, 0, EPI_CONVT_F22_S2, 4)
+OV_DEFINE_VARIANTS(kVariantsT, LIST)
+}
+
+using namespace ovk;
+
+extern "C" {
+
+int ov_convt_f22_supported(int kt, int stride) { return (stride == 8 || stride == 2) && kt == 2 * stride; }
+
+int ov_convt_f22_pack_f32(const float* w, int rows, int Cin, float* dst) {
+  if (!w || !dst || rows <= 0 || Cin <= 0 || rows % 64 != 0) return OV_E_BADARG;
+  const int K = 3;
+  const int mtiles = ov_conv1d_pack_rows(rows) / 32;
+  const int nu = packed_units(Cin);
+  const size_t recs = (size_t)nu * K + 1;
+  for (int row = 0; row < rows; ++row)
+    for (int ci = 0; ci < Cin; ++ci)
+      if (w[((size_t)row * Cin + ci) * K + (((row / 32) & 1) ? 0 : 2)] != 0.f) return OV_E_BADARG;
+  std::memset(dst, 0, ov_conv1d_pack_size(rows, Cin, K) * sizeof(float));
+  for (int mt = 0; mt < mtiles; ++mt)
+    for (int U = 0; U < nu; ++U)
+      for (int g = 0; g < K; ++g) {
+        float* rec = dst + ((size_t)mt * recs + (size_t)U * K + g) * REC;
+        for (int lane = 0; lane < 64; ++lane)
+          for (int u = 0; u < 4; ++u) {
+            const int s = 4 * g + u, pp = s / K, k = s - pp * K;
+            const int ci = UNIT * U + 2 * pp + (lane >> 5);
+            const int row = 32 * mt + (lane & 31);
+            if (row >= rows || ci >= Cin) continue;
+            const float* t = w + ((size_t)row * Cin + ci) * K + (mt & 1);
+            const float g0 = t[0], g1 = t[1];
+            rec[lane * 4 + u] = k == 0 ? g0 + g1 : (k == 1 ? g0 : -g1);
+          }
+      }
+  return OV_OK;
+}
+
+int ov_convt_f22_f32(const ov_conv1d_params* pin, int32_t kt, int32_t col_offset, ov_stream_t stream) {
+  if (!pin || !pin->x || !pin->w || !pin->out || !pin->bias) return OV_E_BADARG;
+  ov_conv1d_params q = *pin;
+  ov_conv1d_params* p = &q;
+  if (p->B <= 0 || p->B > 65535 || p->Cin <= 0 || p->L <= 0 || p->M <= 0 || p->Cout <= 0) return OV_E_BADARG;
+  if (p->epi != OV_EPI_CONVT || !(p->flags & OV_F_CONVT_GROUPED) || p->K != 3 || p->dil != 1) return OV_E_BADARG;
+  if (!ov_convt_f22_supported(kt, p->phase_s)) return OV_E_BADARG;
+  if (col_offset < 0 || (col_offset & 1)) return OV_E_BADARG;
+  if (p->res || p->add || p->out2 || p->mask || p->bias_b) return OV_E_BADARG;
+  const int s = p->phase_s;
+  if (p->M % 64 != 0 || (int64_t)p->Cout * s != p->M) return OV_E_BADARG;
+  const int64_t lout = (int64_t)p->L * s;
+  if (lout > INT32_MAX) return OV_E_BADARG;
+  if (p->x_ld == 0) p->x_ld = p->L;
+  if (p->out_ld == 0) p->out_ld = (int32_t)lout;
+  if (p->x_ld < p->L || p->out_ld < lout) return OV_E_BADARG;
+  if ((int64_t)p->Cin * p->x_ld > UINT32_MAX || (int64_t)(p->M + 32) * p->out_ld > UINT32_MAX) return OV_E_BADARG;
+  if ((reinterpret_cast<uintptr_t>(p->out) & 15) || (p->out_bstride % 4) || (p->out_ld % 4)) return OV_E_ALIGN;
+  if ((reinterpret_cast<uintptr_t>(p->w) & 15)) return OV_E_ALIGN;
+  if (p->col_limit && (p->col_limit_scale <= 0 || (reinterpret_cast<uintptr_t>(p->col_limit) & 3))) return OV_E_BADARG;
+  if (p->col_limit && p->B > ovk::LIMIT_MAX_BATCH) p->col_limit = nullptr;
+  if (p->tile != 0 && (p->tile - 1 < TILE_F22_64x128 || p->tile - 1 > TILE_F22X_64x256)) return OV_E_BADARG;
+  int tile;
+  if (p->tile > 0) tile = p->tile - 1;
+  else if (p->M % 128 == 0) tile = TILE_F22X_128x128;
+  else tile = s == 8 ? TILE_F22_64x128 : TILE_F22W_64x256;
+  const bool can_vec = (p->x_ld % 4 == 0) && !(reinterpret_cast<uintptr_t>(p->x) & 15) && (p->x_bstride % 4 == 0);
+  const int epi = s == 8 ? EPI_CONVT_F22_S8 : EPI_CONVT_F22_S2;
+  conv_launch_fn fn = nullptr;
+  for (int i = 0; i < kVariantsTCount && !fn; ++i) {
+    const ConvVariant& v = kVariantsT[i];
+    if (v.tile == tile && v.vec == (can_vec ? 1 : 0) && v.epi == epi) fn = v.fn;
+  }
+  if (!fn) return OV_E_UNSUPPORTED;
+  return fn(p, static_cast<hipStream_t>(stream));
+}
+
+}
diff --git a/openvoice_amd/csrc/torch_shim.cpp b/openvoice_amd/csrc/torch_shim.cpp
--- a/openvoice_amd/csrc/torch_shim.cpp
+++ b/openvoice_amd/csrc/torch_shim.cpp
@@ -179,11 +179,12 @@
 }
 void finish(int rc, const char* what) { TORCH_CHECK(rc == OV_OK, what, " failed: ", ov_strerror(rc)); }
 
-void conv1d_f32(const OptTensor& x, const OptTensor& w, const OptTensor& bias, const OptTensor& out, const OptTensor& res,
-                const OptTensor& add, const OptTensor& out2, const OptTensor& mask, const OptTensor& bias_b,
-                const OptTensor& col_limit, at::IntArrayRef ip, at::ArrayRef<double> fp) {
-  TORCH_CHECK(ip.size() == 29 && fp.size() == 2, "openvoice_amd::conv1d_f32: 29 integer and 2 float parameters");
-  Ctx c{"conv1d_f32", false};
+void conv1d_launch_f32(bool f22, const OptTensor& x, const OptTensor& w, const OptTensor& bias, const OptTensor& out,
+                       const OptTensor& res, const OptTensor& add, const OptTensor& out2, const OptTensor& mask,
+                       const OptTensor& bias_b, const OptTensor& col_limit, at::IntArrayRef ip, at::ArrayRef<double> fp) {
+  TORCH_CHECK(ip.size() == (f22 ? 31u : 29u) && fp.size() == 2, "openvoice_amd::", f22 ? "convt_f22_f32: 31" : "conv1d_f32: 29",
+              " integer and 2 float parameters");
+  Ctx c{f22 ? "convt_f22_f32" : "conv1d_f32", false};
   ov_conv1d_params p{};
   p.x = sptr<float>(x, c, 0, ip[24]);
   p.w = sptr<float>(w, c, 1);
@@ -204,7 +205,18 @@
   p.out2_bstride = ip[21]; p.bias_b_bstride = ip[22]; p.mask_bstride = ip[23];
   p.in_slope = (float)fp[0]; p.scale = (float)fp[1];
   DeviceScope scope(c);
-  finish(ov_conv1d_f32(&p, c.stream()), "ov_conv1d_f32");
+  if (f22) finish(ov_convt_f22_f32(&p, (int32_t)ip[29], (int32_t)ip[30], c.stream()), "ov_convt_f22_f32");
+  else finish(ov_conv1d_f32(&p, c.stream()), "ov_conv1d_f32");
+}
+void conv1d_f32(const OptTensor& x, const OptTensor& w, const OptTensor& bias, const OptTensor& out, const OptTensor& res,
+                const OptTensor& add, const OptTensor& out2, const OptTensor& mask, const OptTensor& bias_b,
+                const OptTensor& col_limit, at::IntArrayRef ip, at::ArrayRef<double> fp) {
+  conv1d_launch_f32(false, x, w, bias, out, res, add, out2, mask, bias_b, col_limit, ip, fp);
+}
+void convt_f22_f32(const OptTensor& x, const OptTensor& w, const OptTensor& bias, const OptTensor& out, const OptTensor& res,
+                   const OptTensor& add, const OptTensor& out2, const OptTensor& mask, const OptTensor& bias_b,
+                   const OptTensor& col_limit, at::IntArrayRef ip, at::ArrayRef<double> fp) {
+  conv1d_launch_f32(true, x, w, bias, out, res, add, out2, mask, bias_b, col_limit, ip, fp);
 }
 
 void resblock_pair_f32(const OptTensor& x, const OptTensor& w1, const OptTensor& b1, const OptTensor& w2,
@@ -379,6 +391,8 @@
 TORCH_LIBRARY(openvoice_amd, m) {
   m.def("conv1d_f32(Tensor? x, Tensor? w, Tensor? bias, Tensor(a!)? out, Tensor? res, Tensor? add, Tensor(b!)? out2, "
         "Tensor? mask, Tensor? bias_b, Tensor? col_limit, int[] ip, float[] fp) -> ()", &conv1d_f32);
+  m.def("convt_f22_f32(Tensor? x, Tensor? w, Tensor? bias, Tensor(a!)? out, Tensor? res, Tensor? add, Tensor(b!)? out2, "
+        "Tensor? mask, Tensor? bias_b, Tensor? col_limit, int[] ip, float[] fp) -> ()", &convt_f22_f32);
   m.def("resblock_pair_f32(Tensor? x, Tensor? w1, Tensor? b1, Tensor? w2, Tensor? b2, Tensor(a!)? out, Tensor? add, "
         "Tensor(b!)? dbg, Tensor? col_limit, int[] ip, float[] fp) -> ()", &resblock_pair_f32);
   m.def("wn_layer_f32(Tensor? x, Tensor(a!)? out, Tensor(b!)? skip, Tensor? w_in, Tensor? b_in, Tensor? cond, Tensor? w_rs, "
@@ -445,6 +459,8 @@
   bind_device<&ov_split3_from_f32>(m, "split3_from_f32");
   bind_device<&ov_split3_to_f32>(m, "split3_to_f32");
   bind_host<&ov_conv1d_pack_f32>(m, "conv1d_pack_f32");
+  bind_host<&ov_convt_f22_pack_f32>(m, "convt_f22_pack_f32");
+  bind_value<&ov_convt_f22_supported>(m, "convt_f22_supported");
   bind_host<&ov_wn_pack_f32>(m, "wn_pack_f32");
   bind_host<&ov_wn_wino_pack_f32>(m, "wn_wino_pack_f32");
   bind_value<&ov_wn_wino_pack_size>(m, "wn_wino_pack_size");
diff --git a/openvoice_amd/engine.py b/openvoice_amd/engine.py
--- a/openvoice_amd/engine.py
+++ b/openvoice_amd/engine.py
@@ -115,6 +115,31 @@
         self.bias = b.to(device)
 
 
+class PackedConvtF22:
+
+    def __init__(self, w_dense, bias, device, cout, stride):
+        w_dense = w_dense.detach().to(torch.float32).cpu().contiguous()
+        rows, cin, k = w_dense.shape
+        assert k == 3 and rows == cout * stride
+        self.rows, self.cout, self.cin, self.K, self.dil = rows, cout, cin, 3, 1
+        self.stride, self.kt = stride, 2 * stride
+        packed = torch.empty(_lib.call("ov_conv1d_pack_size", rows, cin, 3), dtype=torch.float32)
+        _lib.call("ov_convt_f22_pack_f32", w_dense, rows, cin, packed)
+        self.w = packed.to(device)
+        b = torch.zeros(_lib.call("ov_conv1d_pack_rows", rows), dtype=torch.float32)
+        b[:rows] = bias.detach().float().cpu()
+        self.bias = b.to(device)
+
+
+def convt_f22_policy(cfg, i):
+    from . import live
+    st = generator_stages(cfg)[i]
+    unit = next(u for u in live.live_units(cfg) if u["stage"] == i)
+    kt = cfg["upsample_kernel_sizes"][i]
+    return (st.rate_in % 2 == 0 and unit["align"] % 2 == 0
+            and bool(_lib.call("ov_convt_f22_supported", kt, st.stride)))
+
+
 def padded_frames(T):
     return (T + 3) // 4 * 4
 
@@ -163,15 +188,15 @@
 def launch_conv(layer, x, x_off, x_bs, out, out_off, out_bs, B, L, epi=EPI_LINEAR, flags=0, in_slope=1.0,
                 scale=1.0, res=None, res_off=0, res_bs=0, add=None, add_bs=0, out2=None, out2_bs=0, mask=None,
                 bias_b=None, bias_b_off=0, bias_b_bs=0, split=0, phase_s=1, cin=None, rows=None, tiles_per_wg=0,
-                x_ld=0, out_ld=0, mask_bs=0, tile=0, loaders=0, chunk=0, col_limit=None, col_limit_scale=1):
+                x_ld=0, out_ld=0, mask_bs=0, tile=0, loaders=0, chunk=0, col_limit=None, col_limit_scale=1, f22=None):
     flags |= _EXTRA_CONV_FLAGS
     if _lib.use_torch_binding():
         ip = [B, layer.cin if cin is None else cin, L, x_ld, out_ld, layer.rows if rows is None else rows, layer.cout,
               layer.K, layer.dil, epi, flags, split, phase_s, tiles_per_wg, tile, loaders, chunk,
               x_bs, out_bs, res_bs, add_bs, out2_bs, bias_b_bs, mask_bs, x_off, out_off, res_off, bias_b_off,
               col_limit_scale]
-        _lib.torch_op("conv1d_f32", x, layer.w, layer.bias, out, res, add, out2, mask, bias_b, col_limit, ip,
-                      [in_slope, scale])
+        _lib.torch_op("conv1d_f32" if f22 is None else "convt_f22_f32", x, layer.w, layer.bias, out, res, add, out2, mask,
+                      bias_b, col_limit, ip + ([] if f22 is None else [int(f22[0]), int(f22[1])]), [in_slope, scale])
         return
     p = ConvParams()
     p.x, p.w = _ptr(x, x_off), _ptr(layer.w)
@@ -194,6 +219,9 @@
     p.col_limit = ctypes.c_void_p(col_limit.data_ptr()) if col_limit is not None else None
     p.col_limit_scale = col_limit_scale
     stream = ctypes.c_void_p(torch.cuda.current_stream(x.device).cuda_stream)
+    if f22 is not None:
+        _lib.check(_lib.load().ov_convt_f22_f32(ctypes.byref(p), int(f22[0]), int(f22[1]), stream), "ov_convt_f22_f32")
+        return
     _lib.check(_lib.load().ov_conv1d_f32(ctypes.byref(p), stream), "ov_conv1d_f32")
 
 
@@ -490,7 +518,10 @@
             order = convt_row_order(ch, u)
             if order is not None:
                 wc, bias = wc[order], bias[order]
-            self.ups.append(dict(conv=PackedConv(wc, bias, dev, K=3, cout=ch), stride=u,
+            f22 = None
+            if order is not None and convt_f22_policy(cfg, i):
+                f22 = PackedConvtF22(wc, bias, dev, ch, u)
+            self.ups.append(dict(conv=PackedConv(wc, bias, dev, K=3, cout=ch), stride=u, f22=f22,
                                  flags=F_CONVT_GROUPED if order is not None else 0))
         self.resblocks = _resblock_tree(sd, cfg, lambda c, w, b, d: PackedConv(w, b, dev, K=c.K, dil=d))
         from . import wino as _wino
@@ -526,6 +557,7 @@
         self.wn_row_split = 0
         self.fuse_pairs = True
         self.use_winograd = True
+        self.use_convt_f22 = None
         self.use_multi_launch = USE_MULTI_LAUNCH
         self._cus = None
         self._state_dict_for_bf16 = sd
@@ -869,8 +901,11 @@
     def _upsample(self, i, x, x_ld, u, B, L, cin, ch, **lim):
         up = self.ups[i]
         s = up["stride"]
-        self._conv(up["conv"], x, 0, cin * x_ld, u, 0, ch * L * s, B, L, epi=EPI_CONVT, in_slope=LRELU_SLOPE,
-                   flags=up["flags"], phase_s=s, x_ld=x_ld, tag="ups", alg_flops=2.0 * cin * ch * 2 * s * L * B, **lim)
+        on = self.use_winograd if self.use_convt_f22 is None else self.use_convt_f22
+        f22 = up["f22"] if on else None
+        self._conv(up["conv"] if f22 is None else f22, x, 0, cin * x_ld, u, 0, ch * L * s, B, L, epi=EPI_CONVT,
+                   in_slope=LRELU_SLOPE, flags=up["flags"], phase_s=s, x_ld=x_ld, tag="ups",
+                   alg_flops=2.0 * cin * ch * 2 * s * L * B, **(dict(f22=(f22.kt, 0)) if f22 is not None else {}), **lim)
 
     def _mrf(self, i, u, t1, ra, acc, ws, B, ch, L, limits, rate):
         cfg = self.cfg
```

New measurement: 3166 x real-time (audio s / wall s). About the same (-0.1%).
